# BauerLab/VARSCOT

Measured on AMD Instinct MI355X. Metric: guides/sec (candidate sites/sec alongside) at <=8 mismatches on a 3.0 Gbp reference, higher is better.
Workload: dtype u32

## Files before the change

### varscot_amd/csrc/vsc_api.cpp

```cpp
#include <algorithm>
#include <atomic>
#include <chrono>
#include <cstdlib>
#include <cmath>
#include <cstdio>
#include <cstring>
#include <memory>
#include <new>
#include <string>
#include <vector>

#include "vsc_enum.h"
#include "vsc_internal.h"
#include "vsc_objects.h"
#include "vsc_varmap.h"

using namespace vsc;

namespace {

struct HostTimer {
    bool on = vsc::host_timing_on();
    std::chrono::steady_clock::time_point t0 = std::chrono::steady_clock::now();
    void lap(const char *what)
    {
        if (!on) return;
        auto t1 = std::chrono::steady_clock::now();
        std::fprintf(stderr, "[vsc timing] %-28s %9.3f ms\n", what, std::chrono::duration<double, std::milli>(t1 - t0).count());
        t0 = t1;
    }
};

}

namespace vsc {
static std::atomic<int> g_host_timing{0};
bool host_timing_on() { return g_host_timing.load(std::memory_order_relaxed) != 0; }
}

namespace {

int fail(vsc_ctx *ctx, int code, const char *what, hipError_t e = hipSuccess)
{
    if (ctx) {
        char buf[512];
        if (e != hipSuccess)
            std::snprintf(buf, sizeof buf, "%s: %s", what, hipGetErrorString(e));
        else
            std::snprintf(buf, sizeof buf, "%s", what);
        ctx->err = buf;
    }
    return code;
}

int fail_in(vsc_ctx *ctx, int code, const char *who, const char *what) { return fail(ctx, code, (std::string(who) + ": " + what).c_str()); }

#define VSC_HIP(ctx, call)                                                 \
    do {                                                                   \
        hipError_t e_ = (call);                                            \
        if (e_ != hipSuccess) return fail((ctx), e_ == hipErrorOutOfMemory ? VSC_ERR_NOMEM : VSC_ERR_DEVICE, #call, e_); \
    } while (0)

hipError_t ensure_hl(vsc_ctx *ctx, const vsc_genome *genome)
{
    vsc_genome *g = const_cast<vsc_genome *>(genome);
    if (g->d_hl) return hipSuccess;
    hipError_t e = hipMalloc((void **)&g->d_hl, g->dev_words * sizeof(uint2));
    if (e != hipSuccess) return e;
    g->device_bytes += g->dev_words * sizeof(uint2);
    return launch_interleave(g->d_hi, g->d_lo, g->dev_words, g->d_hl, ctx->stream);
}

hipError_t take_records(vsc_ctx *ctx, vsc_hits *hits, uint64_t n)
{
    const size_t bytes = n * sizeof(vsc_hit);
    int best = -1;
    for (size_t i = 0; i < ctx->spare_records.size(); ++i)
        if (ctx->spare_records[i].cap >= bytes && (best < 0 || ctx->spare_records[i].cap < ctx->spare_records[best].cap))
            best = (int)i;
    if (best >= 0) {
        hits->storage = ctx->spare_records[best];
        ctx->spare_records.erase(ctx->spare_records.begin() + best);
    } else {
        for (auto &b : ctx->spare_records) b.release();
        ctx->spare_records.clear();
        hipError_t e = hits->storage.ensure(bytes);
        if (e != hipSuccess) return e;
    }
    hits->d_records = (vsc_hit *)hits->storage.p;
    return hipSuccess;
}

double hit_probability(unsigned m)
{
    double p = 0, c = 1;
    for (unsigned j = 0; j <= m && j <= 21; ++j) {
        if (j > 0) c = c * (21 - (j - 1)) / j;
        p += c * std::pow(0.75, (double)j) * std::pow(0.25, (double)(21 - j));
    }
    return p;
}

PamMasks pam_masks(int a, int b)
{
    PamMasks m;
    m.ah = (a & 2) ? 0xFFFFFFFFu : 0u;
    m.al = (a & 1) ? 0xFFFFFFFFu : 0u;
    m.bh = (b & 2) ? 0xFFFFFFFFu : 0u;
    m.bl = (b & 1) ? 0xFFFFFFFFu : 0u;
    return m;
}

int base_code(char c)
{
    switch (c) {
    case 'A': case 'a': return 0;
    case 'C': case 'c': return 1;
    case 'G': case 'g': return 2;
    case 'T': case 't': return 3;
    default: return 4;
    }
}

void guide_planes(uint64_t g, uint32_t *h, uint32_t *l)
{
    uint32_t hh = 0, ll = 0;
    for (int i = 0; i < VSC_READ_LEN; ++i) {
        const unsigned c = (unsigned)(g >> (2 * i)) & 3u;
        hh |= (c >> 1) << i;
        ll |= (c & 1u) << i;
    }
    *h = hh;
    *l = ll;
}

}

template <class F> int guarded(vsc_ctx *ctx, F &&body) noexcept
{
    try {
        return body();
    } catch (const std::bad_alloc &) {
        try {
            if (ctx) ctx->err = "out of host memory";
        } catch (...) {
        }
        return VSC_ERR_NOMEM;
    } catch (...) {
        try {
            if (ctx) ctx->err = "unexpected C++ exception";
        } catch (...) {
        }
        return VSC_ERR_DEVICE;
    }
}


extern "C" {

int vsc_abi_version(void) { return VSC_ABI_VERSION; }

int vsc_device_count(void)
{
    int n = 0;
    if (hipGetDeviceCount(&n) != hipSuccess) return 0;
    return n;
}

int vsc_ctx_create(int device_id, vsc_ctx **out) { return vsc_ctx_create_masked(device_id, nullptr, 0, out); }

int vsc_ctx_create_masked(int device_id, const uint32_t *cu_mask, uint32_t n_mask_words, vsc_ctx **out)
{
    if (!out) return VSC_ERR_INVALID;
    *out = nullptr;
    int n = 0;
    if (hipGetDeviceCount(&n) != hipSuccess || n <= 0) return VSC_ERR_NODEVICE;
    if (device_id < 0 || device_id >= n) return VSC_ERR_INVALID;
    vsc_ctx *ctx = new (std::nothrow) vsc_ctx();
    if (!ctx) return VSC_ERR_NOMEM;
    ctx->device = device_id;
    hipDeviceProp_t prop;
    if (hipSetDevice(device_id) != hipSuccess || hipGetDeviceProperties(&prop, device_id) != hipSuccess ||
        (cu_mask && n_mask_words ? hipExtStreamCreateWithCUMask(&ctx->stream, n_mask_words, cu_mask) : hipStreamCreate(&ctx->stream)) != hipSuccess) {
        delete ctx;
        return VSC_ERR_DEVICE;
    }
    ctx->own_stream = true;
    ctx->n_cus = prop.multiProcessorCount;
    for (auto &e : ctx->ev)
        if (hipEventCreate(&e) != hipSuccess) {
            vsc_ctx_destroy(ctx);
            return VSC_ERR_DEVICE;
        }
    *out = ctx;
    return VSC_OK;
}

int vsc_ctx_release_scratch(vsc_ctx *ctx)
{
    if (!ctx) return VSC_ERR_INVALID;
    (void)hipSetDevice(ctx->device);
    (void)hipStreamSynchronize(ctx->stream);
    for (DeviceBuf *b : {&ctx->counters, &ctx->guides, &ctx->score_guides, &ctx->keys_a, &ctx->keys_b, &ctx->vals_a, &ctx->vals_b, &ctx->votes_rows,
                         &ctx->score_mit, &ctx->score_flags, &ctx->score_feat, &ctx->score_sched, &ctx->sort_segs, &ctx->sort_tabs,
                         &ctx->sort_over, &ctx->seed_off,
                         &ctx->seed_poff, &ctx->seed_lrest, &ctx->sum_rows, &ctx->sum_excl, &ctx->sel_hist, &ctx->sel_tabs, &ctx->sel_keys,
                         &ctx->sel_masks, &ctx->sum_rows_in, &ctx->regions_buf, &ctx->enum_tabs, &ctx->locate_buf, &ctx->locate_out,
                         &ctx->varmap_buf, &ctx->var_state, &ctx->var_excl, &ctx->var_labels})
        b->release();
    ctx->regions_serial = 0;
    ctx->locate_serial = 0;
    ctx->varmap_serial = 0;
    for (auto &b : ctx->spare_records) b.release();
    ctx->spare_records.clear();
    ctx->forest.nodes.release();
    ctx->forest.ranks.release();
    ctx->forest.fingerprint = 0;
    return VSC_OK;
}

int vsc_ctx_destroy(vsc_ctx *ctx)
{
    if (!ctx) return VSC_OK;
    (void)vsc_ctx_release_scratch(ctx);
    for (auto &e : ctx->ev)
        if (e) (void)hipEventDestroy(e);
    if (ctx->own_stream && ctx->stream) (void)hipStreamDestroy(ctx->stream);
    delete ctx;
    return VSC_OK;
}

int vsc_ctx_set_stream(vsc_ctx *ctx, void *hip_stream)
{
    if (!ctx) return VSC_ERR_INVALID;
    if (ctx->own_stream && ctx->stream) {
        (void)hipStreamSynchronize(ctx->stream);
        (void)hipStreamDestroy(ctx->stream);
    }
    ctx->stream = (hipStream_t)hip_stream;
    ctx->own_stream = false;
    return VSC_OK;
}

const char *vsc_last_error(const vsc_ctx *ctx) { return ctx ? ctx->err.c_str() : "null context"; }

int vsc_ctx_set_debug_params(vsc_ctx *ctx, const vsc_debug_params *params)
{
    if (!ctx) return VSC_ERR_INVALID;
    ctx->dbg = params ? *params : default_debug_params();
    return VSC_OK;
}

int vsc_ctx_get_debug_params(const vsc_ctx *ctx, vsc_debug_params *out)
{
    if (!ctx || !out) return VSC_ERR_INVALID;
    *out = ctx->dbg;
    return VSC_OK;
}

void vsc_debug_set_host_timing(int on) { vsc::g_host_timing.store(on ? 1 : 0, std::memory_order_relaxed); }

int vsc_ctx_timing(const vsc_ctx *ctx, vsc_timing *out)
{
    if (!ctx || !out) return VSC_ERR_INVALID;
    *out = ctx->timing;
    return VSC_OK;
}

int vsc_genome_load(vsc_ctx *ctx, const uint32_t *hi, const uint32_t *lo, const uint32_t *nmask, uint64_t first_word,
                    uint64_t n_words, uint64_t own_words, const vsc_contig *contigs, uint32_t n_contigs,
                    vsc_genome **out)
{
    return guarded(ctx, [&]() -> int {
    if (!ctx || !out) return VSC_ERR_INVALID;
    *out = nullptr;
    ctx->err.clear();
    if (!hi || !lo || !nmask || !contigs || n_contigs == 0 || n_words == 0 || own_words == 0 || own_words > n_words)
        return fail(ctx, VSC_ERR_INVALID, "vsc_genome_load: null or empty argument");
    if (own_words < n_words && own_words % kTileWords != 0)
        return fail(ctx, VSC_ERR_INVALID, "vsc_genome_load: a shard followed by halo words must own a multiple of 64 words");
    const uint64_t n_tiles = (own_words + kTileWords - 1) / kTileWords;
    const uint64_t dev_words = std::max<uint64_t>(n_tiles * kTileWords, n_words) + kPadWords;
    if ((first_word + dev_words) * 32 >= (1ull << 32) - 4096)
        return fail(ctx, VSC_ERR_RANGE, "vsc_genome_load: genome exceeds the 32-bit position space (4 Gbases)");
    std::vector<uint32_t> off(n_contigs), end(n_contigs);
    for (uint32_t c = 0; c < n_contigs; ++c) {
        const uint64_t e = contigs[c].offset + contigs[c].length;
        if (e >= (1ull << 32) - 4096) return fail(ctx, VSC_ERR_RANGE, "vsc_genome_load: contig table exceeds 4 Gbases");
        if (c > 0 && contigs[c].offset < contigs[c - 1].offset + contigs[c - 1].length + 1)
            return fail(ctx, VSC_ERR_INVALID, "vsc_genome_load: contigs must be ascending and separated by >= 1 N position");
        off[c] = (uint32_t)contigs[c].offset;
        end[c] = (uint32_t)e;
    }
    VSC_HIP(ctx, hipSetDevice(ctx->device));
    vsc_genome *g = new (std::nothrow) vsc_genome();
    if (!g) return fail(ctx, VSC_ERR_NOMEM, "vsc_genome_load: out of host memory");
    g->ctx = ctx;
    g->first_word = first_word;
    g->own_words = own_words;
    g->dev_words = dev_words;
    g->n_tiles = (uint32_t)n_tiles;
    g->n_contigs = n_contigs;
    g->h_contig_off = off;
    g->h_contig_end = end;
    const size_t pb = dev_words * sizeof(uint32_t), cb = (size_t)n_contigs * sizeof(uint32_t);
    hipError_t e = hipSuccess;
    auto step = [&](hipError_t r) {
        if (e == hipSuccess) e = r;
    };
    step(hipMalloc((void **)&g->d_hi, pb));
    step(hipMalloc((void **)&g->d_lo, pb));
    step(hipMalloc((void **)&g->d_nm, pb));
    step(hipMalloc((void **)&g->d_contig_off, cb));
    step(hipMalloc((void **)&g->d_contig_end, cb));
    if (e == hipSuccess) {
        step(hipMemsetAsync(g->d_hi, 0, pb, ctx->stream));
        step(hipMemsetAsync(g->d_lo, 0, pb, ctx->stream));
        step(hipMemsetAsync(g->d_nm, 0xFF, pb, ctx->stream));
        step(hipMemcpyAsync(g->d_hi, hi, n_words * sizeof(uint32_t), hipMemcpyHostToDevice, ctx->stream));
        step(hipMemcpyAsync(g->d_lo, lo, n_words * sizeof(uint32_t), hipMemcpyHostToDevice, ctx->stream));
        step(hipMemcpyAsync(g->d_nm, nmask, n_words * sizeof(uint32_t), hipMemcpyHostToDevice, ctx->stream));
        step(hipMemcpyAsync(g->d_contig_off, off.data(), cb, hipMemcpyHostToDevice, ctx->stream));
        step(hipMemcpyAsync(g->d_contig_end, end.data(), cb, hipMemcpyHostToDevice, ctx->stream));
        step(hipStreamSynchronize(ctx->stream));
    }
    if (e != hipSuccess) {
        vsc_genome_free(g);
        return fail(ctx, e == hipErrorOutOfMemory ? VSC_ERR_NOMEM : VSC_ERR_DEVICE, "vsc_genome_load", e);
    }
    g->device_bytes = 3 * pb + 2 * cb;
    *out = g;
    return VSC_OK;
    });
}

}

int vsc::genome_table_only(vsc_ctx *ctx, const vsc_contig *contigs, uint32_t n_contigs, vsc_genome **out)
{
    if (!ctx || !out || !contigs || n_contigs == 0) return VSC_ERR_INVALID;
    *out = nullptr;
    std::vector<uint32_t> off(n_contigs), end(n_contigs);
    for (uint32_t c = 0; c < n_contigs; ++c) {
        off[c] = (uint32_t)contigs[c].offset;
        end[c] = (uint32_t)(contigs[c].offset + contigs[c].length);
    }
    VSC_HIP(ctx, hipSetDevice(ctx->device));
    vsc_genome *g = new (std::nothrow) vsc_genome();
    if (!g) return fail(ctx, VSC_ERR_NOMEM, "out of host memory");
    g->ctx = ctx;
    g->n_contigs = n_contigs;
    g->h_contig_off = off;
    g->h_contig_end = end;
    const size_t cb = (size_t)n_contigs * sizeof(uint32_t);
    hipError_t e = hipMalloc((void **)&g->d_contig_off, cb);
    if (e == hipSuccess) e = hipMalloc((void **)&g->d_contig_end, cb);
    if (e == hipSuccess) e = hipMemcpy(g->d_contig_off, off.data(), cb, hipMemcpyHostToDevice);
    if (e == hipSuccess) e = hipMemcpy(g->d_contig_end, end.data(), cb, hipMemcpyHostToDevice);
    if (e != hipSuccess) {
        vsc_genome_free(g);
        return fail(ctx, e == hipErrorOutOfMemory ? VSC_ERR_NOMEM : VSC_ERR_DEVICE, "contig table upload", e);
    }
    g->device_bytes = 2 * cb;
    *out = g;
    return VSC_OK;
}

extern "C" {

int vsc_genome_free(vsc_genome *g)
{
    if (!g) return VSC_OK;
    if (g->ctx) (void)hipSetDevice(g->ctx->device);
    for (void *p : {(void *)g->d_hi, (void *)g->d_lo, (void *)g->d_nm, (void *)g->d_contig_off, (void *)g->d_contig_end, (void *)g->d_hl,
                    (void *)g->d_ix_chunk_tab, (void *)g->d_ix_vert, (void *)g->d_ix_sites, (void *)g->d_ix_edge})
        if (p) (void)hipFree(p);
    delete g;
    return VSC_OK;
}

uint64_t vsc_genome_device_bytes(const vsc_genome *g) { return g ? g->device_bytes + g->index_bytes : 0; }

namespace {

#define VSC_TRY(call)                        \
    do {                                     \
        hipError_t e_ = (call);              \
        if (e_ != hipSuccess) return e_;     \
    } while (0)

void fill_pam(ScanArgs &a, const vsc_search_params *params)
{
    a.n_pam = 2;
    a.pam[0] = pam_masks(2, 2);
    a.pam[1] = pam_masks(2, 0);
    if (params && params->has_extra_pam) {
        const int p0 = base_code(params->extra_pam[0]), p1 = base_code(params->extra_pam[1]);
        if (p0 < 4 && p1 < 4) a.pam[a.n_pam++] = pam_masks(p0, p1);
    }
}

uint32_t pam_code_set(const ScanArgs &a)
{
    uint32_t codes = 0;
    for (uint32_t c = 0; c < a.n_pam; ++c)
        codes |= ((((a.pam[c].ah & 2u) | (a.pam[c].al & 1u)) << 2) | (a.pam[c].bh & 2u) | (a.pam[c].bl & 1u)) << (4 * c);
    return codes;
}

void fill_genome(ScanArgs &a, const vsc_ctx *ctx, const vsc_genome *genome)
{
    a.hi = genome->d_hi;
    a.lo = genome->d_lo;
    a.nm = genome->d_nm;
    a.first_pos = (uint32_t)(genome->first_word * 32);
    a.n_tiles = genome->n_tiles;
    a.contig_end = genome->d_contig_end;
    a.n_contigs = genome->n_contigs;
    a.counters = (unsigned long long *)ctx->counters.p;
}

int scan_groups(const vsc_ctx *ctx, uint32_t n_tiles)
{
    const uint32_t n_waves_max = (uint32_t)ctx->n_cus * 4 * kWavesPerGroup;
    const uint32_t n_chunks = (n_tiles + kChunkTiles - 1) / kChunkTiles;
    const uint32_t n_waves = std::max<uint32_t>(1, std::min<uint32_t>(n_waves_max, n_chunks));
    return (int)((n_waves + kWavesPerGroup - 1) / kWavesPerGroup);
}

bool index_matches(const vsc_genome *g, const vsc_search_params *p)
{
    if (!g->has_index) return false;
    const bool want = p && p->has_extra_pam && base_code(p->extra_pam[0]) < 4 && base_code(p->extra_pam[1]) < 4;
    if (want != (g->index_has_extra_pam != 0)) return false;
    return !want || (base_code(p->extra_pam[0]) == base_code(g->index_extra_pam[0]) &&
                     base_code(p->extra_pam[1]) == base_code(g->index_extra_pam[1]));
}

void free_index(vsc_genome *g)
{
    for (void **p : {(void **)&g->d_ix_chunk_tab, (void **)&g->d_ix_vert, (void **)&g->d_ix_sites, (void **)&g->d_ix_edge}) {
        if (*p) (void)hipFree(*p);
        *p = nullptr;
    }
    g->has_index = false;
    g->index_bytes = 0;
    g->ix_chunks = 0;
}

void class_counts(vsc_genome *g, const std::vector<uint32_t> &ctab);

hipError_t build_index(vsc_ctx *ctx, vsc_genome *g, const vsc_search_params *params, std::string *why)
{
    free_index(g);
    hipStream_t st = ctx->stream;
    ScanArgs a{};
    fill_pam(a, params);
    fill_genome(a, ctx, g);
    const int n_groups = scan_groups(ctx, a.n_tiles);
    VSC_TRY(ctx->counters.ensure(kCounterWords * sizeof(unsigned long long)));
    a.counters = (unsigned long long *)ctx->counters.p;
    unsigned long long cnt[kCntSlots];
    VSC_TRY(hipEventRecord(ctx->ev[kEvIndexStart], st));
    VSC_TRY(hipMemsetAsync(ctx->counters.p, 0, sizeof cnt, st));
    VSC_TRY(launch_scan(a, n_groups, true, st));
    VSC_TRY(hipMemcpyAsync(cnt, ctx->counters.p, sizeof cnt, hipMemcpyDeviceToHost, st));
    VSC_TRY(hipStreamSynchronize(st));
    const uint64_t S = cnt[kCntHits];
    if (3 * S >= (1ull << 32) - (1u << 20)) {
        *why = "too many PAM-valid sites for 32-bit table indices";
        return hipErrorInvalidValue;
    }
    DeviceBuf sx, sl, sp, full, rec16;
    auto release = [&]() {
        for (DeviceBuf *b : {&sx, &sl, &sp, &full, &rec16}) b->release();
    };
    hipError_t e = hipSuccess;
    auto step = [&](hipError_t r) {
        if (e == hipSuccess) e = r;
    };
    HostTimer ht;
    constexpr uint32_t kKeys = 8 * kBuckets;
    const uint32_t pam_codes = pam_code_set(a);
    const size_t n4 = std::max<uint64_t>(S, 1) * sizeof(uint32_t);
    for (DeviceBuf *b : {&sx, &sl, &sp}) step(b->ensure(n4));
    step(rec16.ensure(std::max<uint64_t>(S, 1) * sizeof(uint4)));
    const size_t edge_words = (size_t)((3 * S + 31) / 32 + 1);
    ht.lap("index: count pass + buffers");
    if (e == hipSuccess && S > 0) {
        a.site_x = (uint32_t *)sx.p;
        a.site_l = (uint32_t *)sl.p;
        a.site_pos = (uint32_t *)sp.p;
        a.hit_cap = S;
        step(hipMemsetAsync(ctx->counters.p, 0, sizeof cnt, st));
        step(launch_scan(a, n_groups, true, st));
        step(launch_seed_pack16((const uint32_t *)sx.p, (const uint32_t *)sl.p, (const uint32_t *)sp.p, S, (uint4 *)rec16.p, st));
        step(hipStreamSynchronize(st));
    }
    for (DeviceBuf *b : {&sx, &sl, &sp}) b->release();
    ht.lap("index: emit pass");
    constexpr unsigned kKeyBits = 2 * kSegBases + 3, kBits1 = 8, kBits2 = kKeyBits - kBits1;
    constexpr uint32_t kBins1 = 1u << kBits1, kBins2 = 1u << kBits2;
    step(ctx->keys_a.ensure(std::max<uint64_t>(S, 1) * sizeof(uint64_t)));
    step(ctx->keys_b.ensure(std::max<uint64_t>(S, 1) * sizeof(uint64_t)));
    step(full.ensure(std::max<uint64_t>(3 * S, 1) * sizeof(uint4)));
    step(ctx->sort_tabs.ensure(3 * (size_t)(kBins1 * kBins2) * sizeof(uint32_t)));
    const size_t seg_bytes = (kBins1 * sizeof(SortSeg) + 255) / 256 * 256;
    step(ctx->sort_segs.ensure(seg_bytes + (kBins1 + 1) * sizeof(uint32_t)));
// ... 154 lines not shown
    uint64_t sites;
    uint64_t own_words, vert_bytes, edge_words, fingerprint;
    uint32_t chunks, n_contigs;
    uint8_t has_extra_pam;
    char extra_pam[2];
    uint8_t layout;
    uint8_t pad[4];
};
static_assert(sizeof(IndexFileHeader) == 80, "index file header layout");
constexpr char kIndexMagic[8] = {'V', 'S', 'C', 'S', 'E', 'E', 'D', 0};
constexpr size_t kIndexIoChunk = 64u << 20;

hipError_t genome_fingerprint(vsc_ctx *ctx, const vsc_genome *g, uint64_t *out)
{
    VSC_TRY(ctx->counters.ensure(kCounterWords * sizeof(unsigned long long)));
    unsigned long long *d_sum = (unsigned long long *)ctx->counters.p;
    VSC_TRY(hipMemsetAsync(d_sum, 0, sizeof *d_sum, ctx->stream));
    const uint64_t words = std::min<uint64_t>(g->own_words + 1, g->dev_words);
    VSC_TRY(launch_plane_hash(g->d_hi, g->d_lo, g->d_nm, words, d_sum, ctx->stream));
    unsigned long long sum = 0;
    VSC_TRY(hipMemcpyAsync(&sum, d_sum, sizeof sum, hipMemcpyDeviceToHost, ctx->stream));
    std::vector<uint32_t> tab(2 * (size_t)g->n_contigs);
    if (g->n_contigs) {
        VSC_TRY(hipMemcpyAsync(tab.data(), g->d_contig_off, (size_t)g->n_contigs * sizeof(uint32_t), hipMemcpyDeviceToHost, ctx->stream));
        VSC_TRY(hipMemcpyAsync(tab.data() + g->n_contigs, g->d_contig_end, (size_t)g->n_contigs * sizeof(uint32_t), hipMemcpyDeviceToHost, ctx->stream));
    }
    VSC_TRY(hipStreamSynchronize(ctx->stream));
    uint64_t h = 0xcbf29ce484222325ull;
    auto eat = [&](uint64_t v) {
        for (int i = 0; i < 8; ++i) h = (h ^ ((v >> (8 * i)) & 0xFF)) * 0x100000001b3ull;
    };
    eat(sum);
    eat(g->own_words);
    eat(g->first_word);
    for (uint32_t w : tab) eat(w);
    *out = h;
    return hipSuccess;
}

bool chunk_table_ok(const std::vector<uint32_t> &ctab, uint64_t S, uint64_t vert_bytes, std::string *why)
{
    const uint64_t n_blocks = vert_bytes / (kVertWords * sizeof(uint32_t));
    uint64_t expect_site = 0, expect_block = 0;
    uint32_t last_group = 0;
    for (size_t c = 0; c * 4 < ctab.size(); ++c) {
        const uint64_t first = ctab[4 * c], count = ctab[4 * c + 1], vfirst = ctab[4 * c + 3];
        const uint32_t z = ctab[4 * c + 2], bucket = z & kChunkBucketMask, minus_from = (z >> kChunkMinusShift) & 0xFFFu;
        const uint32_t cls = z >> kChunkClassShift;
        const uint64_t blocks = (count + kSlicedSites - 1) / kSlicedSites;
        const char *bad = nullptr;
        if (count == 0 || count > (uint64_t)kSlicedChunk) bad = "site count";
        else if (first != expect_site || first + count > 3 * S) bad = "first site";
        else if (vfirst != expect_block || vfirst + blocks > n_blocks) bad = "first block";
        else if (bucket >= (uint32_t)kBuckets || cls >= (uint32_t)kSeedClasses || (bucket << 2 | cls) < last_group) bad = "bucket";
        else if (minus_from > count) bad = "strand boundary";
        if (bad) {
            *why = "chunk " + std::to_string(c) + ": bad " + bad;
            return false;
        }
        expect_site = first + count;
        expect_block = vfirst + blocks;
        last_group = bucket << 2 | cls;
    }
    if (expect_site != 3 * S) {
        *why = "the chunks do not cover the site table";
        return false;
    }
    return true;
}

void class_counts(vsc_genome *g, const std::vector<uint32_t> &ctab)
{
    for (int c = 0; c < 4; ++c) g->ix_class_sites[c] = g->ix_class_chunks[c] = 0;
    for (size_t c = 0; c * 4 < ctab.size(); ++c) {
        const uint32_t cls = ctab[4 * c + 2] >> kChunkClassShift;
        g->ix_class_sites[cls] += ctab[4 * c + 1];
        g->ix_class_chunks[cls] += 1;
    }
    for (int c = 0; c < 4; ++c) g->ix_class_sites[c] /= kSegments;
}

struct FileCloser {
    std::FILE *f;
    ~FileCloser() { if (f) std::fclose(f); }
};

hipError_t index_io(std::FILE *f, void *dev, uint64_t bytes, bool to_file, std::vector<char> &host, bool *io_ok)
{
    for (uint64_t off = 0; off < bytes; off += kIndexIoChunk) {
        const size_t n = (size_t)std::min<uint64_t>(kIndexIoChunk, bytes - off);
        if (to_file) {
            VSC_TRY(hipMemcpy(host.data(), (const char *)dev + off, n, hipMemcpyDeviceToHost));
            if (std::fwrite(host.data(), 1, n, f) != n) { *io_ok = false; return hipSuccess; }
        } else {
            if (std::fread(host.data(), 1, n, f) != n) { *io_ok = false; return hipSuccess; }
            VSC_TRY(hipMemcpy((char *)dev + off, host.data(), n, hipMemcpyHostToDevice));
        }
    }
    return hipSuccess;
}

}

int vsc_genome_build_index(vsc_ctx *ctx, vsc_genome *genome, const vsc_search_params *params)
{
    return guarded(ctx, [&]() -> int {
    if (!ctx || !genome || genome->ctx != ctx) return VSC_ERR_INVALID;
    ctx->err.clear();
    if (index_matches(genome, params)) return VSC_OK;
    VSC_HIP(ctx, hipSetDevice(ctx->device));
    std::string why;
    hipError_t e = build_index(ctx, genome, params, &why);
    if (e != hipSuccess) {
        if (!why.empty()) return fail(ctx, VSC_ERR_RANGE, ("vsc_genome_build_index: " + why).c_str());
        return fail(ctx, e == hipErrorOutOfMemory ? VSC_ERR_NOMEM : VSC_ERR_DEVICE, "vsc_genome_build_index", e);
    }
    ctx->timing.index_ms = genome->index_ms;
    return VSC_OK;
    });
}

int vsc_genome_index_save(vsc_ctx *ctx, const vsc_genome *genome, const char *path)
{
    return guarded(ctx, [&]() -> int {
    if (!ctx || !genome || genome->ctx != ctx || !path) return VSC_ERR_INVALID;
    ctx->err.clear();
    if (!genome->has_index) return fail(ctx, VSC_ERR_INVALID, "vsc_genome_index_save: the genome has no seed index (vsc_genome_build_index)");
    VSC_HIP(ctx, hipSetDevice(ctx->device));
    IndexFileHeader h{};
    std::memcpy(h.magic, kIndexMagic, sizeof h.magic);
    h.abi = VSC_ABI_VERSION;
    h.seg_bases = kSegBases;
    h.sliced_chunk = kSlicedChunk;
    h.sliced_sites = kSlicedSites;
    h.layout = (uint8_t)kIndexLayout;
    h.sites = genome->index_sites;
    h.own_words = genome->own_words;
    h.vert_bytes = genome->ix_vert_bytes;
    h.edge_words = genome->ix_edge_words;
    h.chunks = genome->ix_chunks;
    h.n_contigs = genome->n_contigs;
    h.has_extra_pam = genome->index_has_extra_pam;
    h.extra_pam[0] = genome->index_extra_pam[0];
    h.extra_pam[1] = genome->index_extra_pam[1];
    VSC_HIP(ctx, genome_fingerprint(ctx, genome, &h.fingerprint));
    FileCloser fc{std::fopen(path, "wb")};
    if (!fc.f) return fail(ctx, VSC_ERR_INVALID, (std::string("vsc_genome_index_save: cannot write ") + path).c_str());
    bool ok = std::fwrite(&h, sizeof h, 1, fc.f) == 1;
    std::vector<char> host(kIndexIoChunk);
    const uint64_t S = genome->index_sites;
    if (ok) VSC_HIP(ctx, index_io(fc.f, genome->d_ix_sites, 3 * S * sizeof(uint2), true, host, &ok));
    if (ok) VSC_HIP(ctx, index_io(fc.f, genome->d_ix_edge, h.edge_words * sizeof(uint32_t), true, host, &ok));
    if (ok) VSC_HIP(ctx, index_io(fc.f, genome->d_ix_chunk_tab, (uint64_t)h.chunks * sizeof(uint4), true, host, &ok));
    if (ok) VSC_HIP(ctx, index_io(fc.f, genome->d_ix_vert, h.vert_bytes, true, host, &ok));
    if (ok) ok = std::fflush(fc.f) == 0;
    if (!ok) return fail(ctx, VSC_ERR_DEVICE, (std::string("vsc_genome_index_save: write to ") + path + " failed").c_str());
    return VSC_OK;
    });
}

int vsc_genome_index_load(vsc_ctx *ctx, vsc_genome *genome, const char *path)
{
    return guarded(ctx, [&]() -> int {
    if (!ctx || !genome || genome->ctx != ctx || !path) return VSC_ERR_INVALID;
    ctx->err.clear();
    VSC_HIP(ctx, hipSetDevice(ctx->device));
    const auto t0 = std::chrono::steady_clock::now();
    FileCloser fc{std::fopen(path, "rb")};
    if (!fc.f) return fail(ctx, VSC_ERR_INVALID, (std::string("vsc_genome_index_load: cannot read ") + path).c_str());
    IndexFileHeader h{};
    if (std::fread(&h, sizeof h, 1, fc.f) != 1 || std::memcmp(h.magic, kIndexMagic, sizeof h.magic) != 0)
        return fail(ctx, VSC_ERR_INVALID, (std::string("vsc_genome_index_load: ") + path + " is not a seed index file").c_str());
    if (h.abi != VSC_ABI_VERSION || h.seg_bases != (uint32_t)kSegBases || h.sliced_chunk != (uint32_t)kSlicedChunk ||
        h.sliced_sites != (uint32_t)kSlicedSites || h.layout != (uint8_t)kIndexLayout)
        return fail(ctx, VSC_ERR_INVALID, "vsc_genome_index_load: the file was written by another version of the library");
    uint64_t fp = 0;
    VSC_HIP(ctx, genome_fingerprint(ctx, genome, &fp));
    if (h.own_words != genome->own_words || h.n_contigs != genome->n_contigs || h.fingerprint != fp)
        return fail(ctx, VSC_ERR_INVALID, "vsc_genome_index_load: the file belongs to another genome");
    const uint64_t S = h.sites;
    if (3 * S >= (1ull << 32) || h.edge_words != (3 * S + 31) / 32 + 1 || h.vert_bytes % (kVertWords * sizeof(uint32_t)) != 0)
        return fail(ctx, VSC_ERR_INVALID, "vsc_genome_index_load: inconsistent header");
    {
        const long at = std::ftell(fc.f);
        const uint64_t want = (uint64_t)sizeof h + 3 * S * sizeof(uint2) + h.edge_words * sizeof(uint32_t) +
                              (uint64_t)h.chunks * sizeof(uint4) + h.vert_bytes;
        if (at < 0 || std::fseek(fc.f, 0, SEEK_END) != 0) return fail(ctx, VSC_ERR_INVALID, "vsc_genome_index_load: cannot seek in the file");
        const long size = std::ftell(fc.f);
        if (size < 0 || (uint64_t)size != want || std::fseek(fc.f, at, SEEK_SET) != 0)
            return fail(ctx, VSC_ERR_INVALID, (std::string("vsc_genome_index_load: ") + path + " is truncated or does not match its header").c_str());
    }
    free_index(genome);
    hipError_t e = hipSuccess;
    auto step = [&](hipError_t r) {
        if (e == hipSuccess) e = r;
    };
    const uint64_t sb = std::max<uint64_t>(3 * S, 1) * sizeof(uint2), eb = h.edge_words * sizeof(uint32_t);
    const uint64_t cb = std::max<uint64_t>(h.chunks, 1) * sizeof(uint4), vb = std::max<uint64_t>(h.vert_bytes, kVertWords * sizeof(uint32_t));
    step(hipMalloc((void **)&genome->d_ix_sites, sb));
    step(hipMalloc((void **)&genome->d_ix_edge, eb));
    step(hipMalloc((void **)&genome->d_ix_chunk_tab, cb));
    step(hipMalloc((void **)&genome->d_ix_vert, vb));
    bool ok = true;
    std::vector<char> host(kIndexIoChunk);
    if (e == hipSuccess) step(index_io(fc.f, genome->d_ix_sites, 3 * S * sizeof(uint2), false, host, &ok));
    if (e == hipSuccess && ok) step(index_io(fc.f, genome->d_ix_edge, eb, false, host, &ok));
    if (e == hipSuccess && ok) step(index_io(fc.f, genome->d_ix_chunk_tab, (uint64_t)h.chunks * sizeof(uint4), false, host, &ok));
    if (e == hipSuccess && ok) step(index_io(fc.f, genome->d_ix_vert, h.vert_bytes, false, host, &ok));
    if (e != hipSuccess || !ok) {
        free_index(genome);
        if (e != hipSuccess) return fail(ctx, e == hipErrorOutOfMemory ? VSC_ERR_NOMEM : VSC_ERR_DEVICE, "vsc_genome_index_load", e);
        return fail(ctx, VSC_ERR_INVALID, (std::string("vsc_genome_index_load: ") + path + " is truncated").c_str());
    }
    {
        std::vector<uint32_t> ctab((size_t)h.chunks * 4);
        if (h.chunks) VSC_HIP(ctx, hipMemcpy(ctab.data(), genome->d_ix_chunk_tab, ctab.size() * sizeof(uint32_t), hipMemcpyDeviceToHost));
        std::string why;
        if (!chunk_table_ok(ctab, S, h.vert_bytes, &why)) {
            free_index(genome);
            return fail(ctx, VSC_ERR_INVALID, (std::string("vsc_genome_index_load: ") + path + " is damaged (" + why + ")").c_str());
        }
        class_counts(genome, ctab);
    }
    genome->ix_chunks = h.chunks;
    genome->ix_vert_bytes = vb;
    genome->ix_edge_words = h.edge_words;
    genome->index_sites = S;
    genome->sites = S;
    genome->has_index = true;
    genome->index_has_extra_pam = h.has_extra_pam;
    genome->index_extra_pam[0] = h.extra_pam[0];
    genome->index_extra_pam[1] = h.extra_pam[1];
    genome->index_bytes = sb + eb + cb + vb;
    genome->index_ms = std::chrono::duration<double, std::milli>(std::chrono::steady_clock::now() - t0).count();
    ctx->timing.index_ms = genome->index_ms;
    return VSC_OK;
    });
}

}

namespace {

unsigned ceil_log2(uint64_t x)
{
    unsigned b = 0;
    while (b < 63 && (1ull << b) < x) ++b;
    return b;
}

struct SortRows {
    uint32_t *side_src = nullptr;
    DeviceBuf *side_other = nullptr;
    const uint2 *guides = nullptr;
    uint32_t guide_first = 0;
    uint4 *rows = nullptr;
    uint64_t rows_first = 0;
};

struct SortInfo {
    unsigned levels = 0;
    unsigned bin_bits = 0;
    uint64_t bytes = 0;
    unsigned slot_fallbacks = 0;
};

hipError_t bin_sort(vsc_ctx *ctx, const vsc_genome *genome, std::vector<SortSeg> segs, uint64_t *src, uint64_t *other,
                    unsigned key_bits, unsigned pos_pad, uint32_t pos_base, vsc_hit *out, hipEvent_t ev_sorted, SortInfo *info,
                    DeviceBuf *other_buf = nullptr, bool *slots = nullptr, const SortRows *rows = nullptr)
{
    uint32_t *side_src = rows ? rows->side_src : nullptr, *side_other = nullptr;
    hipStream_t st = ctx->stream;
    unsigned rem = key_bits;
    bool sorted_marked = false;
    const vsc_debug_params &dbg = ctx->dbg;
    uint64_t sort_cap = kSortCap;
    unsigned max_bits = kSortMaxBinBits;
    if (dbg.sort_cap) sort_cap = std::min<uint64_t>(kSortCap, std::max<uint32_t>(16, dbg.sort_cap));
    if (dbg.sort_max_bits) max_bits = std::min<unsigned>(kSortMaxBinBits, std::max<uint32_t>(1, dbg.sort_max_bits));
    uint64_t slot_cap = dbg.sort_slot_cap ? dbg.sort_slot_cap : (sort_cap + sort_cap / 4 + 15) / 16 * 16;
    slot_cap = std::max<uint64_t>(slot_cap, 16);
    for (unsigned level = 1; !segs.empty(); ++level) {
        if (level > 48) return hipErrorUnknown;
        uint64_t n_max = 0, n_all = 0;
        for (const SortSeg &s : segs) {
            n_max = std::max<uint64_t>(n_max, s.n_in);
            n_all += s.n_in;
        }
        unsigned bits = 0;
        if (n_max > sort_cap) {
            if (rem == 0) return hipErrorUnknown;
            const uint64_t want = std::max<uint64_t>(1, sort_cap * 7 / 10);
            bits = std::min<unsigned>({std::max(1u, ceil_log2((n_max + want - 1) / want)), max_bits, rem});
            while (bits > 1 && ((uint64_t)segs.size() << bits) > (1ull << 22)) --bits;
        }
        const size_t n_segs = segs.size();
        const size_t n_bins = n_segs << bits;
        bool use_slots = level == 1 && bits && slots && other_buf && (dbg.sort_optimistic == 1 || (dbg.sort_optimistic != 0 && *slots));
        if (level == 1 && bits && other_buf) {
            uint64_t span = 1;
            for (const SortSeg &sg : segs) span = std::max<uint64_t>(span, sg.out_off + sg.n_in);
            const uint64_t slot_records = (uint64_t)n_bins * slot_cap;
            if (use_slots && dbg.sort_optimistic != 1) {
                size_t free_b = 0, total_b = 0;
                if (hipMemGetInfo(&free_b, &total_b) != hipSuccess) free_b = 0;
                const uint64_t room = (uint64_t)free_b + other_buf->cap;
                const uint64_t slot_bytes = slot_records * (sizeof(uint64_t) + (rows ? sizeof(uint32_t) : 0));
                if (slot_records > 4 * n_all + (1ull << 20) || slot_bytes + (1ull << 30) > room + (rows ? rows->side_other->cap : 0)) {
                    use_slots = false;
                    *slots = false;
                }
            }
            hipError_t ge = other_buf->ensure((size_t)(use_slots ? std::max(slot_records, span) : span) * sizeof(uint64_t));
            if (ge == hipErrorOutOfMemory && use_slots) {
                (void)hipGetLastError();
                use_slots = false;
                *slots = false;
                ge = other_buf->ensure((size_t)span * sizeof(uint64_t));
            }
            if (ge != hipSuccess) return ge;
            other = (uint64_t *)other_buf->p;
            if (rows) {
                VSC_TRY(rows->side_other->ensure(other_buf->cap / sizeof(uint64_t) * sizeof(uint32_t)));
                side_other = (uint32_t *)rows->side_other->p;
            }
        }
        std::vector<uint32_t> &tile0 = ctx->host_tile0;
        tile0.assign(n_segs + 1, 0);
        uint64_t tiles = 0;
        for (size_t i = 0; i < n_segs; ++i) {
            tile0[i] = (uint32_t)tiles;
            tiles += (segs[i].n_in + kSortTile - 1) / kSortTile;
        }
        if (tiles >= (1ull << 31)) return hipErrorInvalidValue;
        tile0[n_segs] = (uint32_t)tiles;
        const size_t seg_bytes = (n_segs * sizeof(SortSeg) + 255) / 256 * 256;
        VSC_TRY(ctx->sort_segs.ensure(seg_bytes + tile0.size() * sizeof(uint32_t)));
        SortSeg *d_segs = (SortSeg *)ctx->sort_segs.p;
        uint32_t *d_tile0 = (uint32_t *)((char *)ctx->sort_segs.p + seg_bytes);
        ctx->host_segs = segs;
        VSC_TRY(hipMemcpyAsync(d_segs, ctx->host_segs.data(), n_segs * sizeof(SortSeg), hipMemcpyHostToDevice, st));
        VSC_TRY(hipMemcpyAsync(d_tile0, tile0.data(), tile0.size() * sizeof(uint32_t), hipMemcpyHostToDevice, st));
        VSC_TRY(ctx->sort_over.ensure(256 + n_bins * sizeof(SortSeg)));
        uint32_t *d_n_over = (uint32_t *)ctx->sort_over.p;
        if (bits) VSC_TRY(ctx->sort_tabs.ensure(3 * n_bins * sizeof(uint32_t)));
        uint32_t flags[3] = {0, 0, 0};
        for (;;) {
            if (dbg.sort_debug)
                std::fprintf(stderr, "[vsc sort] level %u: %zu segments, %llu records, largest %llu, %u bits (of %u left), cap %llu%s\n", level,
                             n_segs, (unsigned long long)n_all, (unsigned long long)n_max, bits, rem, (unsigned long long)sort_cap,
                             use_slots ? ", slot mode" : "");
            VSC_TRY(hipMemsetAsync(d_n_over, 0, 3 * sizeof(uint32_t), st));
            FinArgs f{};
            f.segs = d_segs;
            f.n_segs = (uint32_t)n_segs;
            f.src = src;
            f.side_src = side_src;
            if (rows) {
                f.guides = rows->guides;
                f.guide_first = rows->guide_first;
                f.rows = rows->rows;
                f.rows_first = rows->rows_first;
            }
            if (bits) {
                SortArgs a{};
                a.segs = d_segs;
                a.seg_tile0 = d_tile0;
                a.n_segs = (uint32_t)n_segs;
                a.n_tiles = (uint32_t)tiles;
                a.in = src;
                a.out = other;
                a.side_in = rows ? side_src : nullptr;
                a.side_out = rows ? side_other : nullptr;
                a.hist = (uint32_t *)ctx->sort_tabs.p;
                a.cursor = a.hist + n_bins;
                a.bin_start = a.cursor + n_bins;
                a.bin_bits = bits;
                a.bin_shift = kRecPosShift + pos_pad + rem - bits;
                if (dbg.sort_xcd != 0 && tiles >= 64) a.xcd_tiles = (uint32_t)((tiles + 7) / 8);
                if (use_slots) {
                    a.hist = a.cursor;
                    a.slot_cap = (uint32_t)slot_cap;
                    a.overflow = d_n_over + 2;
                    VSC_TRY(hipMemsetAsync(a.cursor, 0, n_bins * sizeof(uint32_t), st));
                    VSC_TRY(launch_bin_partition(a, st));
                    VSC_TRY(launch_bin_scan(a, st));
                } else {
                    VSC_TRY(hipMemsetAsync(a.hist, 0, n_bins * sizeof(uint32_t), st));
                    VSC_TRY(launch_bin_hist(a, st));
                    VSC_TRY(launch_bin_scan(a, st));
                    if (dbg.sort_debug >= 2) {
                        std::vector<uint32_t> h(n_bins);
                        VSC_TRY(hipMemcpyAsync(h.data(), a.hist, n_bins * sizeof(uint32_t), hipMemcpyDeviceToHost, st));
                        VSC_TRY(hipStreamSynchronize(st));
                        for (size_t i = 0; i < n_segs; ++i) {
                            std::vector<uint64_t> recs(segs[i].n_in);
                            VSC_TRY(hipMemcpy(recs.data(), src + segs[i].in_off, recs.size() * sizeof(uint64_t), hipMemcpyDeviceToHost));
                            std::vector<uint32_t> want((size_t)1 << bits, 0);
                            for (uint64_t r : recs) {
                                if (r >> 63) continue;
                                want[(r >> a.bin_shift) & (((uint64_t)1 << bits) - 1)]++;
                            }
                            for (size_t b = 0; b < want.size(); ++b)
                                if (want[b] != h[(i << bits) + b])
                                    std::fprintf(stderr, "[vsc sort]   seg %zu (in_off %llu n %u) bin %zu: device %u host %u\n", i,
                                                 (unsigned long long)segs[i].in_off, segs[i].n_in, b, h[(i << bits) + b], want[b]);
                        }
                    }
                    VSC_TRY(launch_bin_partition(a, st));
                }
                f.src = other;
                f.side_src = side_other;
                f.hist = a.hist;
                f.bin_start = a.bin_start;
                f.bin_bits = bits;
                f.slot_cap = a.slot_cap;
                f.overflow = a.overflow;
            }
            if (!sorted_marked && ev_sorted) {
                VSC_TRY(hipEventRecord(ev_sorted, st));
                sorted_marked = true;
            }
            const unsigned rem_after = rem - bits;
            f.sub_bits = std::min<unsigned>(rows ? kSortSubBitsRows : kSortSubBits, rem_after);
            f.sub_shift = kRecPosShift + pos_pad + rem_after - f.sub_bits;
            f.pos_pad = pos_pad;
            f.pos_base = pos_base;
            f.low_bits = rem_after - f.sub_bits;
            f.over = (SortSeg *)((char *)ctx->sort_over.p + 256);
            f.over_cap = (uint32_t)std::min<size_t>(n_bins, 0xFFFFFFFFu);
            f.n_over = d_n_over;
            f.cursor = d_n_over + 1;
            f.cap = (uint32_t)sort_cap;
            f.contig_off = genome->d_contig_off;
            f.n_contigs = genome->n_contigs;
            f.out = out;
            VSC_TRY(launch_bin_finalize(f, 2 * ctx->n_cus, st));
            if (bits) {
                VSC_TRY(hipMemcpyAsync(flags, d_n_over, sizeof flags, hipMemcpyDeviceToHost, st));
                VSC_TRY(hipStreamSynchronize(st));
                if (use_slots && flags[2]) {
                    use_slots = false;
                    *slots = false;
                    if (info) {
                        info->slot_fallbacks++;
                        info->bytes += 16 * n_all;
                    }
                    continue;
                }
            }
            if (info && bits) {
                if (info->levels == 0) info->bin_bits = bits;
                info->levels++;
                info->bytes += (use_slots ? 16 : 24) * n_all;
            }
            if (info) info->bytes += 24 * n_all;
            if (info && rows) info->bytes += (bits ? 8 : 0) * n_all + (4 + 12 + 64) * n_all;
            break;
        }
        if (!bits) break;
        rem -= bits;
        const uint32_t n_over = flags[0];
        if (n_over == 0) break;
        segs.resize(n_over);
        VSC_TRY(hipMemcpyAsync(segs.data(), (char *)ctx->sort_over.p + 256, (size_t)n_over * sizeof(SortSeg), hipMemcpyDeviceToHost, st));
        VSC_TRY(hipStreamSynchronize(st));
        std::swap(src, other);
        std::swap(side_src, side_other);
        if (rows && !side_other) {
            uint64_t span = 1;
            for (const SortSeg &sg : segs) span = std::max<uint64_t>(span, sg.out_off + sg.n_in);
            VSC_TRY(rows->side_other->ensure(span * sizeof(uint32_t)));
            side_other = (uint32_t *)rows->side_other->p;
        }
    }
    return hipSuccess;
}

hipError_t result_room(vsc_ctx *ctx, vsc_hits *hits, uint64_t used, uint64_t n, uint64_t projected)
{
    const uint64_t need = used + n;
    if (hits->storage.p && hits->storage.cap >= need * sizeof(vsc_hit)) return hipSuccess;
    if (used == 0) {
        if (hits->storage.p) {
            ctx->spare_records.push_back(hits->storage);
            hits->storage = DeviceBuf{};
        }
        VSC_TRY(take_records(ctx, hits, std::max(need, projected)));
        return hipSuccess;
    }
    DeviceBuf bigger;
    VSC_TRY(bigger.ensure(std::max(need, projected) * sizeof(vsc_hit)));
    hipError_t e = hipMemcpyAsync(bigger.p, hits->storage.p, used * sizeof(vsc_hit), hipMemcpyDeviceToDevice, ctx->stream);
    if (e == hipSuccess) e = hipStreamSynchronize(ctx->stream);
    if (e != hipSuccess) {
        bigger.release();
        return e;
    }
    hits->storage.release();
    hits->storage = bigger;
    hits->d_records = (vsc_hit *)bigger.p;
    return hipSuccess;
}

struct PassFound {
    HostTimer ht;
    int algo = 0, n_parts = 0;
    uint32_t max_mm = 0, guide_base = 0;
    uint64_t cap = 0, n = 0;
    std::vector<SortSeg> segs;
    unsigned key_bits = 0, pos_pad = 0;
    uint32_t pos_base = 0;
    bool bases = false;
    bool selected = false;
    std::vector<uint64_t> sel_off;
    std::vector<SumSeg> sink_segs;
    std::vector<uint32_t> sink_tile0;
    SinkInput sink{};
    bool classified = false;
};

uint32_t neighbours(int k) { return k < 0 ? 0u : (k == 0 ? 1u : (k == 1 ? 22u : 211u)); }

SeedPlan seed_cut(const vsc_genome *genome, const uint32_t *gp, uint32_t n_guides, uint32_t m, int n_cus, const vsc_debug_params &dbg,
                  int *k2_max)
{
    SeedPlan plan{};
    plan.max_mm = m;
    ScanArgs pa{};
    vsc_search_params ip{};
    ip.has_extra_pam = genome->index_has_extra_pam;
    ip.extra_pam[0] = genome->index_extra_pam[0];
    ip.extra_pam[1] = genome->index_extra_pam[1];
    fill_pam(pa, &ip);
    plan.n_pam = pa.n_pam;
    plan.pam_codes = pam_code_set(pa);
    plan.tight = dbg.seed_tight != 0;
    if (!plan.tight) {
        plan.k0 = plan.k1 = m / kSegments;
        *k2_max = (int)plan.k0;
    } else {
        uint32_t left_reads[kSeedClasses][VSC_MAX_MISMATCHES + 1] = {};
        int left_max = -1;
        for (uint32_t i = 0; i < n_guides; ++i) {
            const uint32_t x = gp[2 * (size_t)i], l = gp[2 * (size_t)i + 1];
            const uint32_t mine = (((x >> 21) & 1u) << 3) | (((l >> 21) & 1u) << 2) | (((x >> 22) & 1u) << 1) | ((l >> 22) & 1u);
            for (uint32_t c = 0; c < plan.n_pam; ++c) {
                const uint32_t diff = mine ^ ((plan.pam_codes >> (4 * c)) & 15u);
                const uint32_t spent = ((diff & 12u) ? 1u : 0u) + ((diff & 3u) ? 1u : 0u);
                if (spent > m) continue;
                left_reads[c][m - spent]++;
                left_max = std::max(left_max, (int)(m - spent));
            }
        }
        double cost[9];
        double chunks_all = 0, sites_all = 0;
        uint64_t reads_any = 0;
        for (uint32_t c = 0; c < plan.n_pam; ++c) {
            chunks_all += (double)genome->ix_class_chunks[c] / kSegments;
            sites_all += (double)genome->ix_class_sites[c];
            uint64_t reads_c = 0;
            for (int left = 0; left <= (int)m; ++left) reads_c += left_reads[c][left];
            reads_any = std::max(reads_any, reads_c);
        }
        const double block_bytes = (double)kVertWords * 4 / kSlicedSites;
        for (int cut = 0; cut < 9; ++cut) {
            const int k0 = cut % 3, k1 = cut / 3;
            cost[cut] = -1;
            if (left_max - k0 - k1 - 2 > 2) continue;
            double bytes = 0, visits = 0;
            for (uint32_t c = 0; c < plan.n_pam; ++c) {
                double e2 = 0;
                for (int left = 0; left <= (int)m; ++left) e2 += (double)left_reads[c][left] * neighbours(left - k0 - k1 - 2);
                const double per_list = e2 / kBucketsPerSeg;
                bytes += (1.0 - std::exp(-per_list)) * (double)genome->ix_class_sites[c] * block_bytes;
                visits += per_list * (double)genome->ix_class_chunks[c] / kSegments;
            }
            for (int k : {k0, k1}) {
                const double per_list = (double)reads_any * neighbours(k) / kBucketsPerSeg;
                bytes += (1.0 - std::exp(-per_list)) * sites_all * block_bytes;
                visits += per_list * chunks_all;
            }
            cost[cut] = std::max(bytes / 4.2e12, visits * 215.0 / ((double)n_cus * 4 * 2.0e9));
        }
        int best = -1;
        for (int cut = 0; cut < 9; ++cut)
            if (cost[cut] >= 0 && (best < 0 || cost[cut] < cost[best])) best = cut;
        const int forced = dbg.seed_tight >= 1 ? dbg.seed_tight - 1 : -1;
        if (forced >= 0 && forced < 9 && cost[forced] >= 0) best = forced;
        if (best < 0) best = 4 * (int)(m ? (m - 1) / kSegments : 0u);
        plan.k0 = (uint32_t)(best % 3);
        plan.k1 = (uint32_t)(best / 3);
        *k2_max = std::min<int>(2, (int)m - (int)plan.k0 - (int)plan.k1 - 2);
    }
    plan.n_nbr = neighbours(std::max<int>(std::max<int>((int)plan.k0, (int)plan.k1), *k2_max));
    return plan;
}

hipError_t seed_plan(vsc_ctx *ctx, const vsc_genome *genome, const uint32_t *gp, uint32_t n_guides, const PassFound &f, SeedArgs &sa,
                     int *n_groups, bool *shared)
{
    int k2_max = 0;
    const SeedPlan plan = seed_cut(genome, gp, n_guides, f.max_mm, ctx->n_cus, ctx->dbg, &k2_max);
    const uint64_t n_pairs = (uint64_t)n_guides * (neighbours((int)plan.k0) + neighbours((int)plan.k1) + plan.n_pam * neighbours(k2_max));
    const uint64_t list_cap = n_pairs + (uint64_t)kLists * (kGuideUnroll - 1) + 2 * kGuideUnroll;
    VSC_TRY(ctx->seed_off.ensure((kLists + 1) * sizeof(uint32_t)));
    VSC_TRY(ctx->seed_poff.ensure((kLists + 1) * sizeof(uint32_t)));
    VSC_TRY(ctx->seed_lrest.ensure(list_cap * sizeof(uint2)));
    VSC_TRY(hipMemsetAsync(ctx->seed_lrest.p, 0xFF, list_cap * sizeof(uint2), ctx->stream));
    VSC_TRY(launch_seed_lists((const uint2 *)ctx->guides.p, n_guides, plan, (uint32_t *)ctx->seed_off.p, (uint32_t *)ctx->seed_poff.p,
                              (uint2 *)ctx->seed_lrest.p, ctx->stream));
    VSC_TRY(hipEventRecord(ctx->ev[kEvPrepEnd], ctx->stream));
    sa.chunk_tab = genome->d_ix_chunk_tab;
    sa.n_chunks = genome->ix_chunks;
    sa.vert = genome->d_ix_vert;
    sa.list_rest = (const uint2 *)ctx->seed_lrest.p;
    sa.sites = genome->d_ix_sites;
    sa.edge_bits = genome->d_ix_edge;
    sa.guides = (const uint2 *)ctx->guides.p;
    sa.poff = (const uint32_t *)ctx->seed_poff.p;
    sa.max_mm = f.max_mm;
    sa.k_half = f.max_mm / 2;
    sa.k_seg0 = plan.k0;
    sa.k_seg1 = plan.k1;
    sa.contig_end = genome->d_contig_end;
    sa.n_contigs = genome->n_contigs;
    sa.counters = (unsigned long long *)ctx->counters.p;
    sa.n_parts = (uint32_t)f.n_parts;
    uint32_t groups_per_cu = kSlicedWavesPerSimd;
    if (ctx->dbg.seed_groups_per_cu) groups_per_cu = ctx->dbg.seed_groups_per_cu;
    *shared = (uint64_t)n_guides * neighbours((int)std::max(plan.k0, plan.k1)) / kBucketsPerSeg >= 72;
    if (ctx->dbg.seed_shared >= 0) *shared = ctx->dbg.seed_shared == 1;
    const uint32_t n_grabs = (sa.n_chunks + kSlicedGrab - 1) / kSlicedGrab;
    const uint32_t n_waves_max = (uint32_t)ctx->n_cus * groups_per_cu * kWavesPerGroup;
    const uint32_t n_waves = std::max<uint32_t>(1, std::min<uint32_t>(n_waves_max, *shared ? n_grabs * kWavesPerGroup : n_grabs));
    *n_groups = (int)((n_waves + kWavesPerGroup - 1) / kWavesPerGroup);
    sa.group_out = *shared && ctx->dbg.seed_group_out != 0 ? 1u : 0u;
    const uint32_t owners = sa.group_out ? (uint32_t)*n_groups : (uint32_t)*n_groups * kWavesPerGroup;
    const uint64_t per_wave = f.cap / ((uint64_t)owners * 8 * f.n_parts);
    uint32_t want_reserve = (uint32_t)std::min<uint64_t>(f.n_parts > 8 ? (sa.group_out ? 1024 : 128) : 1024, std::max<uint64_t>(kWave, per_wave));
    if (ctx->dbg.seed_reserve) want_reserve = std::min<uint32_t>(1024, std::max<uint32_t>(kWave, ctx->dbg.seed_reserve));
    sa.reserve_log2 = 6;
    while ((2u << sa.reserve_log2) <= want_reserve) ++sa.reserve_log2;
    sa.reserve = 1u << sa.reserve_log2;
    sa.pos_pad = f.pos_pad;
    sa.pos_base = f.pos_base;
    uint64_t part_cap = f.cap / f.n_parts + f.cap / f.n_parts / 7 + 4096;
    part_cap = std::max<uint64_t>(part_cap, (uint64_t)(1.2 * genome->seen_rate[f.max_mm] * std::min<uint32_t>(n_guides, kRegionReads)) + 4096);
    sa.part_cap = part_cap + (uint64_t)owners * sa.reserve;
    return hipSuccess;
}

int find_pass(vsc_ctx *ctx, const vsc_genome *genome, const uint64_t *guides, uint32_t n_guides, uint32_t guide_base,
              const vsc_search_params *params, bool keep_bases, vsc_timing &t, PassFound &f)
{
    const int algo = (int)t.algorithm;
    const uint32_t m = params->max_mismatches;
    f.algo = algo;
    f.max_mm = m;
    f.guide_base = guide_base;
    f.bases = keep_bases;
    const uint32_t n_pad = (n_guides + kGuideUnroll - 1) / kGuideUnroll * kGuideUnroll;
    std::vector<uint32_t> gp((size_t)(n_pad + kGuideUnroll) * 2, 0xFFFFFFFFu);
    for (uint32_t i = 0; i < n_guides; ++i) guide_planes(guides[i], &gp[2 * (size_t)i], &gp[2 * (size_t)i + 1]);
    VSC_HIP(ctx, ctx->guides.ensure(gp.size() * sizeof(uint32_t)));
    VSC_HIP(ctx, ctx->counters.ensure(kCounterWords * sizeof(unsigned long long)));
    VSC_HIP(ctx, hipEventRecord(ctx->ev[kEvPassStart], ctx->stream));
    VSC_HIP(ctx, hipMemcpyAsync(ctx->guides.p, gp.data(), gp.size() * sizeof(uint32_t), hipMemcpyHostToDevice, ctx->stream));

    const double own_bases = (double)genome->n_tiles * kTileBases;
    const double sites_est = genome->sites ? (double)genome->sites : own_bases / 4;
    f.cap = (uint64_t)(1.5 * sites_est * n_guides * hit_probability(m)) + (1u << 20);
    const double seen_rate = genome->seen_rate[m];
    if (algo == VSC_ALGO_SCAN) f.cap = std::max<uint64_t>(f.cap, (uint64_t)(1.2 * seen_rate * n_guides) + 4096);
    unsigned long long cnt[kCntPart + 4 * kParts] = {};
    f.n_parts = (int)((n_guides + kRegionReads - 1) / kRegionReads);
    f.pos_base = (uint32_t)(genome->first_word * 32);
    const unsigned pos_bits = std::max(1u, ceil_log2((uint64_t)genome->dev_words * 32));
    f.pos_pad = pos_bits < 32 ? 32 - pos_bits : 0;
    f.key_bits = pos_bits + 1 + ceil_log2(std::min<uint32_t>(n_guides, kRegionReads));

    ScanArgs a{};
    SeedArgs sa{};
    int n_groups = 1;
    bool seed_shared = false;
    if (algo == VSC_ALGO_SCAN) {
        fill_pam(a, params);
        fill_genome(a, ctx, genome);
        a.guides = (const uint4 *)ctx->guides.p;
        a.n_guides_padded = n_pad;
        a.max_mm = m;
        a.k_half = m / 2;
        n_groups = scan_groups(ctx, a.n_tiles);
        t.genome_bytes += (uint64_t)genome->n_tiles * kTileWords * 3 * sizeof(uint32_t);
        VSC_HIP(ctx, hipEventRecord(ctx->ev[kEvPrepEnd], ctx->stream));
    } else {
        VSC_HIP(ctx, seed_plan(ctx, genome, gp.data(), n_guides, f, sa, &n_groups, &seed_shared));
        f.cap = sa.part_cap * f.n_parts;
    }

    f.ht.lap("prep enqueue");
    uint32_t list_total = 0;
    for (unsigned tries = 0;; ++tries) {
        if (algo == VSC_ALGO_SEED && (sa.part_cap >= (1ull << 32) - (1u << 20) || sa.part_cap >= ((uint64_t)sa.reserve << 20) - sa.reserve))
            return fail(ctx, VSC_ERR_RANGE, "vsc_search: more than 2^32 hits in a block of 64 reads");
        VSC_HIP(ctx, ctx->keys_a.ensure(f.cap * sizeof(uint64_t)));
        VSC_HIP(ctx, hipMemsetAsync(ctx->counters.p, 0, kCounterWords * sizeof(unsigned long long), ctx->stream));
        VSC_HIP(ctx, hipEventRecord(ctx->ev[kEvSearchStart], ctx->stream));
        if (algo == VSC_ALGO_SCAN) {
            VSC_HIP(ctx, ctx->vals_a.ensure(f.cap * sizeof(uint32_t)));
            a.hit_keys = (uint64_t *)ctx->keys_a.p;
            a.hit_vals = (uint32_t *)ctx->vals_a.p;
            a.hit_cap = f.cap;
            VSC_HIP(ctx, launch_scan(a, n_groups, false, ctx->stream));
        } else {
            sa.hit_recs = (uint64_t *)ctx->keys_a.p;
            if (keep_bases) {
                VSC_HIP(ctx, ctx->vals_a.ensure(f.cap * sizeof(uint32_t)));
                sa.hit_side = (uint32_t *)ctx->vals_a.p;
            }
            VSC_HIP(ctx, launch_seed_sliced(sa, n_groups, seed_shared, ctx->stream));
        }
        VSC_HIP(ctx, hipEventRecord(ctx->ev[kEvSearchEnd], ctx->stream));
        VSC_HIP(ctx, hipMemcpyAsync(cnt, ctx->counters.p, sizeof cnt, hipMemcpyDeviceToHost, ctx->stream));
        if (algo == VSC_ALGO_SEED)
            VSC_HIP(ctx, hipMemcpyAsync(&list_total, (const uint32_t *)ctx->seed_poff.p + kLists, sizeof list_total, hipMemcpyDeviceToHost, ctx->stream));
        VSC_HIP(ctx, hipStreamSynchronize(ctx->stream));
        f.ht.lap("search kernel + sync");
        t.passes++;
        if (!cnt[kCntOverflow]) break;
        if (tries >= 2) return fail(ctx, VSC_ERR_DEVICE, "vsc_search: hit buffer overflowed repeatedly");
        if (algo == VSC_ALGO_SEED) {
            uint64_t need = 0;
            for (int q = 0; q < f.n_parts; ++q) need = std::max<uint64_t>(need, cnt[kCntPart + 4 * q] + cnt[kCntPart + 4 * q + 2]);
            sa.part_cap = need + (need >> 6) + 4096 + (uint64_t)(sa.group_out ? n_groups : n_groups * kWavesPerGroup) * sa.reserve;
            f.cap = sa.part_cap * f.n_parts;
        } else {
            f.cap = cnt[kCntHits] + (cnt[kCntHits] >> 6) + 4096;
        }
    }
    float ms = 0;
    VSC_HIP(ctx, hipEventElapsedTime(&ms, ctx->ev[kEvPassStart], ctx->ev[kEvPrepEnd]));
    t.prep_ms += ms;
    VSC_HIP(ctx, hipEventElapsedTime(&ms, ctx->ev[kEvSearchStart], ctx->ev[kEvSearchEnd]));
    t.scan_ms += ms;

    if (algo == VSC_ALGO_SCAN) {
        genome->sites = cnt[kCntSites];
        t.sites = cnt[kCntSites];
        t.pairs += cnt[kCntSites] * n_guides;
        f.n = cnt[kCntHits];
        genome->seen_rate[m] = (double)f.n / n_guides;
        if (f.n >= (1ull << 32)) return fail(ctx, VSC_ERR_RANGE, "vsc_search: more than 2^32 hits in one scan pass (split the read set)");
        if (f.n > 0) f.segs.push_back(SortSeg{0, 0, 0, (uint32_t)f.n, guide_base});
    } else {
        t.list_entries = list_total;
        t.seed_cut = sa.k_seg0 | (sa.k_seg1 << 4);
        t.sites = genome->index_sites;
        t.pairs += cnt[kCntSites];
        t.genome_bytes += cnt[kCntVisited] * kVertWords * sizeof(uint32_t) / kSlicedSites;
        double fullest = 0;
        for (int q = 0; q < f.n_parts; ++q) {
            const uint64_t placed = cnt[kCntPart + 4 * q], real = placed - cnt[kCntPart + 4 * q + 1];
            fullest = std::max(fullest, (double)placed / std::min<uint32_t>(kRegionReads, n_guides - (uint32_t)q * kRegionReads));
            if (placed) f.segs.push_back(SortSeg{(uint64_t)q * sa.part_cap, (uint64_t)q * sa.part_cap, f.n, (uint32_t)placed,
                                                 guide_base + (uint32_t)q * kRegionReads});
            f.n += real;
        }
        genome->seen_rate[m] = fullest;
    }
    t.hits += f.n;
    return VSC_OK;
}

hipError_t sink_input(vsc_ctx *ctx, PassFound &f, bool excluded)
{
    if (f.sink.recs) return hipSuccess;
    f.sink_tile0.assign(1, 0);
    for (const SortSeg &sg : f.segs) {
        f.sink_segs.push_back(SumSeg{sg.in_off, sg.n_in, sg.guide_base - f.guide_base});
        f.sink_tile0.push_back(f.sink_tile0.back() + (sg.n_in + kSumTile - 1) / kSumTile);
    }
    const size_t seg_bytes = f.sink_segs.size() * sizeof(SumSeg), tile0_bytes = f.sink_tile0.size() * sizeof(uint32_t);
    const size_t tile0_at = (seg_bytes + 255) / 256 * 256;
    VSC_TRY(ctx->sort_segs.ensure(tile0_at + tile0_bytes));
    VSC_TRY(hipMemcpyAsync(ctx->sort_segs.p, f.sink_segs.data(), seg_bytes, hipMemcpyHostToDevice, ctx->stream));
    VSC_TRY(hipMemcpyAsync((char *)ctx->sort_segs.p + tile0_at, f.sink_tile0.data(), tile0_bytes, hipMemcpyHostToDevice, ctx->stream));
    SinkInput &a = f.sink;
    a.vals = f.algo == VSC_ALGO_SCAN ? (const uint32_t *)ctx->vals_a.p : nullptr;
    a.segs = (const SumSeg *)ctx->sort_segs.p;
    a.seg_tile0 = (const uint32_t *)((char *)ctx->sort_segs.p + tile0_at);
    a.n_segs = (uint32_t)f.sink_segs.size();
    a.n_tiles = f.sink_tile0.back();
    a.pos_pad = f.pos_pad;
    a.pos_base = f.pos_base;
    a.excl = excluded ? (const uint64_t *)ctx->sum_excl.p + f.guide_base : nullptr;
    a.recs = (const uint64_t *)ctx->keys_a.p;
    return hipSuccess;
}

hipError_t end_pass(vsc_ctx *ctx, PassFound &f, const char *lap, vsc_timing &t)
{
    VSC_TRY(hipEventRecord(ctx->ev[kEvSinkEnd], ctx->stream));
    VSC_TRY(hipStreamSynchronize(ctx->stream));
    f.ht.lap(lap);
    float ms = 0;
    VSC_TRY(hipEventElapsedTime(&ms, ctx->ev[kEvSinkStart], ctx->ev[kEvSinkEnd]));
    t.finalize_ms += ms;
    VSC_TRY(hipEventElapsedTime(&ms, ctx->ev[kEvPassStart], ctx->ev[kEvSinkEnd]));
    t.total_ms += ms;
    t.read_passes++;
    return hipSuccess;
}

int sort_pass(vsc_ctx *ctx, const vsc_genome *genome, PassFound &f, vsc_hits *hits, uint64_t used, uint64_t projected, vsc_timing &t)
{
    SortInfo info;
    if (f.n > 0) {
        uint64_t *src = (uint64_t *)ctx->keys_a.p, *other = nullptr;
        if (f.algo == VSC_ALGO_SCAN && !f.selected) {
            VSC_HIP(ctx, ctx->keys_b.ensure(f.cap * sizeof(uint64_t)));
            const unsigned bits0 = ceil_log2((uint64_t)f.n_parts);
            const size_t n_bins = (size_t)1 << bits0;
            VSC_HIP(ctx, ctx->sort_segs.ensure(512));
            VSC_HIP(ctx, ctx->sort_tabs.ensure(3 * n_bins * sizeof(uint32_t)));
            const uint32_t tile0[2] = {0u, (uint32_t)((f.n + kSortTile - 1) / kSortTile)};
            VSC_HIP(ctx, hipMemcpyAsync(ctx->sort_segs.p, f.segs.data(), sizeof(SortSeg), hipMemcpyHostToDevice, ctx->stream));
            VSC_HIP(ctx, hipMemcpyAsync((char *)ctx->sort_segs.p + 256, tile0, sizeof tile0, hipMemcpyHostToDevice, ctx->stream));
            SortArgs l0{};
            l0.segs = (const SortSeg *)ctx->sort_segs.p;
            l0.seg_tile0 = (const uint32_t *)((char *)ctx->sort_segs.p + 256);
            l0.n_segs = 1;
            l0.n_tiles = tile0[1];
            l0.pair_keys = (const uint64_t *)ctx->keys_a.p;
            l0.pair_vals = (const uint32_t *)ctx->vals_a.p;
            l0.out = (uint64_t *)ctx->keys_b.p;
            l0.hist = (uint32_t *)ctx->sort_tabs.p;
            l0.cursor = l0.hist + n_bins;
            l0.bin_start = l0.cursor + n_bins;
            l0.bin_bits = bits0;
            l0.bin_shift = kRecKeyBits;
            l0.pos_pad = f.pos_pad;
            l0.pos_base = f.pos_base;
            VSC_HIP(ctx, hipMemsetAsync(l0.hist, 0, n_bins * sizeof(uint32_t), ctx->stream));
            VSC_HIP(ctx, launch_bin_hist(l0, ctx->stream));
            VSC_HIP(ctx, launch_bin_scan(l0, ctx->stream));
            VSC_HIP(ctx, launch_bin_partition(l0, ctx->stream));
            std::vector<uint32_t> tabs(3 * n_bins);
            VSC_HIP(ctx, hipMemcpyAsync(tabs.data(), l0.hist, tabs.size() * sizeof(uint32_t), hipMemcpyDeviceToHost, ctx->stream));
            VSC_HIP(ctx, hipStreamSynchronize(ctx->stream));
            f.segs.clear();
            for (int q = 0; q < f.n_parts; ++q) {
                const uint32_t count = tabs[q], start = tabs[2 * n_bins + q];
                if (count) f.segs.push_back(SortSeg{start, start, start, count, f.guide_base + (uint32_t)q * kRegionReads});
            }
            src = (uint64_t *)ctx->keys_b.p;
            other = (uint64_t *)ctx->keys_a.p;
            info.bytes += 12 * f.n + 20 * f.n;
        }
        for (SortSeg &s : f.segs) s.final_off += used;
        f.ht.lap("sort buffers");
        VSC_HIP(ctx, result_room(ctx, hits, used, f.n, projected));
        f.ht.lap("record storage");
        bool *slots = f.algo == VSC_ALGO_SEED && !f.selected ? &genome->sort_slots_ok[f.max_mm] : nullptr;
        SortRows rows;
        if (f.bases) {
            if (ctx->score_feat.ensure(f.n * VSC_PACKED_FEATURE_BYTES) != hipSuccess) {
                (void)hipGetLastError();
                for (auto &b : ctx->spare_records) b.release();
                ctx->spare_records.clear();
                for (DeviceBuf *b : {&ctx->score_mit, &ctx->score_flags, &ctx->score_sched, &ctx->keys_b, &ctx->vals_b}) b->release();
                VSC_HIP(ctx, ctx->score_feat.ensure(f.n * VSC_PACKED_FEATURE_BYTES));
            }
            rows.side_src = (uint32_t *)ctx->vals_a.p;
            rows.side_other = &ctx->vals_b;
            rows.guides = (const uint2 *)ctx->guides.p;
            rows.guide_first = f.guide_base;
            rows.rows = (uint4 *)ctx->score_feat.p;
            rows.rows_first = used;
        }
        VSC_HIP(ctx, bin_sort(ctx, genome, std::move(f.segs), src, other, f.key_bits, f.pos_pad, f.pos_base, hits->d_records, ctx->ev[kEvSinkStart],
                              &info, f.algo == VSC_ALGO_SEED || f.selected ? &ctx->keys_b : nullptr, slots, f.bases ? &rows : nullptr));
    } else {
        VSC_HIP(ctx, hipEventRecord(ctx->ev[kEvSinkStart], ctx->stream));
    }
    VSC_HIP(ctx, end_pass(ctx, f, "sort + finalize + sync", t));
    float ms = 0;
    VSC_HIP(ctx, hipEventElapsedTime(&ms, ctx->ev[kEvSearchEnd], ctx->ev[kEvSinkStart]));
    t.sort_ms += ms;
    t.sort_levels = std::max(t.sort_levels, info.levels);
    t.sort_bin_bits = std::max(t.sort_bin_bits, info.bin_bits);
    t.sort_bytes += info.bytes;
    t.sort_fallbacks += info.slot_fallbacks;
    return VSC_OK;
}

int prepare_forest(vsc_ctx *ctx, const vsc_rf_model *model, const char *who);
void fill_forest(RfArgs &a, const vsc_ctx *ctx);
int resident_ranks(vsc_ctx *ctx, const double *guide_activity, uint32_t n_guides);

int classify_pass(vsc_ctx *ctx, const vsc_genome *genome, PassFound &f, uint32_t n_reads, bool excluded)
{
    if (f.segs.empty()) return VSC_OK;
    RfArgs a{};
    VSC_HIP(ctx, sink_input(ctx, f, excluded));
    fill_forest(a, ctx);
    a.in = f.sink;
    a.score.hl = genome->d_hl;
    a.score.first_pos = (uint32_t)(genome->first_word * 32);
    a.score.n_plane_words = genome->dev_words;
    a.score.guides = (const uint2 *)ctx->guides.p;
    a.act_rank = (const uint8_t *)ctx->forest.ranks.p + f.guide_base;
    a.n_reads = n_reads;
    a.n = (uint64_t)a.in.n_tiles * kSumTile;
// ... 1801 lines not shown
```

### varscot_amd/csrc/vsc_internal.h

```cpp
#pragma once

#include <hip/hip_runtime.h>
#include <stdint.h>

#include "varscot_hip.h"

namespace vsc {

constexpr int kWave = 64;
constexpr int kWavesPerGroup = 4;
constexpr int kSitesPerLane = 8;
constexpr int kBatch = kWave * kSitesPerLane;
constexpr int kQueueCap = kBatch + kWave;
constexpr int kHitCap = 128;
constexpr int kTileWords = kWave;
constexpr int kTileBases = kTileWords * 32;
constexpr int kChunkTiles = 8;
constexpr int kGuideUnroll = 4;
constexpr uint32_t kMask23 = 0x7FFFFFu;
constexpr int kSiteStrandBit = 23;
constexpr int kSiteEdgeBit = 24;
constexpr uint32_t kPadWords = 4;

constexpr int kSegments = 3;
constexpr int kSegBases = 7;
constexpr int kBucketsPerSeg = 1 << (2 * kSegBases);
constexpr int kBuckets = kSegments * kBucketsPerSeg;
constexpr int kSeedHitCap = 256;
constexpr int kSlicedSites = 32;
constexpr int kSlicedChunk = kWave * kSlicedSites;
constexpr int kRestBases = VSC_READ_LEN - kSegBases;
constexpr int kCmpBases = 2 * kSegBases;
constexpr int kVertWords = 2 * kCmpBases;
constexpr int kSeedClasses = 3;
constexpr int kLists = (kSegments - 1 + kSeedClasses) * kBucketsPerSeg;
constexpr int kListBudgetShift = 16;
constexpr uint32_t kListNoBudget = 15;
constexpr int kTokLaneShift = 26;
constexpr int kTokSlotShift = 14;
constexpr uint32_t kTokReadMask = (1u << kTokSlotShift) - 1u;
constexpr int kSlicedResolve = 3;
constexpr int kSlicedTokCap = 512;
constexpr uint32_t kChunkBucketMask = 0xFFFFu;
constexpr int kChunkMinusShift = 16;
constexpr int kChunkEdgeBit = 28;
constexpr int kChunkClassShift = 29;
constexpr uint32_t kIndexLayout = 2;
constexpr int kSlicedWavesPerSimd = 6;
constexpr int kSlicedGrab = 8;

enum { kCntHits = 0, kCntChunk = 1, kCntSites = 2, kCntOverflow = 3, kCntVisited = 4, kCntPad = 5, kCntLost = 6, kCntGroups = 7, kCntSlots = 8 };
constexpr int kRegionBits = 6;
constexpr int kRegionReads = 1 << kRegionBits;
constexpr int kParts = 256;
constexpr int kMaxPassReads = kParts * kRegionReads;
constexpr int kCntPart = 8;
constexpr int kCursors = 32;
constexpr int kCursorStride = 16;
constexpr int kCursorBase = kCntPart + 4 * kParts + 8;
constexpr int kCounterWords = kCursorBase + kCursors * kCursorStride;

constexpr int kRecPosShift = 23;
constexpr int kRecStrandShift = 55;
constexpr int kRecReadShift = 56;
constexpr int kRecKeyBits = 33 + kRegionBits;
constexpr uint64_t kRecSentinel = ~0ull;

constexpr int kSortThreads = 512;
constexpr int kSortItems = 16;
constexpr int kSortTile = kSortThreads * kSortItems;
constexpr int kFinThreads = 512;
constexpr int kFinItems = 16;
constexpr int kSortCap = kFinThreads * kFinItems - 128;
constexpr int kSortMaxBinBits = 11;
constexpr int kSortSubBits = 13;
constexpr int kSortSubBitsRows = 12;
constexpr int kHistTiles = 8;

struct PamMasks {
    uint32_t ah, al;
    uint32_t bh, bl;
};

struct ScanArgs {
    const uint32_t *hi, *lo, *nm;
    uint32_t first_pos;
    uint32_t n_tiles;
    const uint4 *guides;
    uint32_t n_guides_padded;
    uint32_t max_mm;
    uint32_t k_half;
    uint32_t n_pam;
    PamMasks pam[3];
    const uint32_t *contig_end;
    uint32_t n_contigs;
    uint64_t *hit_keys;
    uint32_t *hit_vals;
    unsigned long long hit_cap;
    unsigned long long *counters;
    uint32_t *site_x, *site_l, *site_pos;
};

struct SortSeg {
    uint64_t in_off;
    uint64_t out_off;
    uint64_t final_off;
    uint32_t n_in;
    uint32_t guide_base;
};

struct SortArgs {
    const SortSeg *segs;
    const uint32_t *seg_tile0;
    uint32_t n_segs, n_tiles;
    const uint64_t *in;
    const uint64_t *pair_keys;
    const uint32_t *pair_vals;
    uint64_t *out;
    const uint32_t *side_in;
    uint32_t *side_out;
    uint32_t *hist;
    uint32_t *cursor;
    uint32_t *bin_start;
    uint32_t bin_bits, bin_shift;
    uint32_t pos_pad;
    uint32_t pos_base;
    uint32_t xcd_tiles;
    uint32_t slot_cap;
    uint32_t *overflow;
};

struct FinArgs {
    const SortSeg *segs;
    uint32_t n_segs;
    const uint64_t *src;
    const uint32_t *hist;
    const uint32_t *bin_start;
    uint32_t bin_bits;
    uint32_t sub_shift, sub_bits;
    uint32_t low_bits;
    uint32_t pos_pad;
    uint32_t pos_base;
    SortSeg *over;
    uint32_t over_cap;
    uint32_t cap;
    uint32_t *n_over;
    uint32_t *cursor;
    const uint32_t *contig_off;
    uint32_t n_contigs;
    vsc_hit *out;
    uint32_t slot_cap;
    const uint32_t *overflow;
    const uint32_t *side_src;
    const uint2 *guides;
    uint32_t guide_first;
    uint4 *rows;
    uint64_t rows_first;
};

struct ScoreArgs {
    const vsc_hit *hits;
    uint64_t n;
    const uint2 *hl;
    uint32_t first_pos;
    uint64_t n_plane_words;
    const uint32_t *contig_off;
    const uint2 *guides;
    double *mit;
    uint8_t *mit_flags;
    uint8_t *features;
    const uint64_t *seg_prefix;
    const uint64_t *seg_start;
    uint32_t n_segs;
};

struct SeedPlan {
    uint32_t max_mm, k0, k1, tight;
    uint32_t n_nbr;
    uint32_t n_pam;
    uint32_t pam_codes;
};

struct SeedArgs {
    const uint4 *chunk_tab;
    const uint32_t *vert;
    const uint2 *list_rest;
    const uint2 *sites;
    const uint32_t *edge_bits;
    const uint2 *guides;
    uint32_t n_chunks;
    const uint32_t *poff;
    uint32_t max_mm, k_half;
    uint32_t k_seg0, k_seg1;
    const uint32_t *contig_end;
    uint32_t n_contigs;
    uint64_t *hit_recs;
    uint32_t *hit_side;
    uint32_t group_out;
    uint32_t reserve;
    uint32_t reserve_log2;
    uint32_t pos_pad;
    uint32_t pos_base;
    uint32_t n_parts;
    unsigned long long part_cap;
    unsigned long long *counters;
};

constexpr int kSumThreads = 256;
constexpr int kSumItems = 8;
constexpr int kSumTile = kSumThreads * kSumItems;
constexpr int kSumTilesPerBlock = 8;

struct SumSeg {
    uint64_t in_off;
    uint32_t n;
    uint32_t first_read;
};

struct SinkInput {
    const uint64_t *recs;
    const uint32_t *vals;
    const SumSeg *segs;
    const uint32_t *seg_tile0;
    uint32_t n_segs, n_tiles;
    uint32_t pos_pad, pos_base;
    const uint64_t *excl;
};

constexpr int kRfRows = 512;
constexpr int kRfMaxTests = 1024;
constexpr int kRfMaxNodes = 1024;
constexpr int kRfTileBytes = 26624;
constexpr int kRfPairFirstBit = 3;
constexpr int kRfPairMaxTests = 8 * (32 - kRfPairFirstBit);
constexpr int kRfPairBitsBytes = 16384;
constexpr int kRfPairTileBytes = 24512;
constexpr int kRfChains = 2;
constexpr int kRfRowWords = 20;
struct RfTest {
    uint8_t word, shift, width, thr;
    uint16_t dense_col;
    uint16_t pad;
};

struct RfArgs {
    const uint32_t *nodes;
    const uint8_t *depth;
    uint32_t n_trees, n_nodes;
    uint32_t compact;
    const RfTest *tests;
    const uint32_t *test_begin;
    uint32_t n_tests;
    const uint8_t *dense;
    const uint4 *packed;
    const uint8_t *act_rank;
    uint64_t n;
    uint32_t *votes;
    uint16_t *votes16;
    uint32_t tree_splits;
    ScoreArgs score;
    SinkInput in;
    uint32_t n_reads;
    uint32_t *slot_votes;
};

constexpr int kSumWords = 12;
constexpr int kSumCounts = 11;
constexpr int kSumCountBits = 7;

struct SummaryArgs : SinkInput {
    unsigned long long *out;
};

struct VotesSummaryArgs : SummaryArgs {
    const uint32_t *votes;
    uint32_t n_trees, n_reads;
};

constexpr int kSelBins = 128;
constexpr int kSelThreads = 256;
constexpr int kSelMaxTilesPerBlock = 128;
constexpr int kSelMinTilesPerBlock = 8;
constexpr uint32_t kSelDropped = ~0u;
constexpr int kSelKeyPosBits = 33;

struct SelectArgs : SinkInput {
    uint32_t min_score;
    uint32_t vote_trees;
    uint32_t top_k;
    uint32_t n_reads;
    uint32_t tiles_per_block;
    uint32_t *score;
    uint32_t *hist;
    uint32_t *thr;
    uint32_t *thr_region;
    uint32_t *count;
    uint32_t *cursor;
    const uint64_t *cand_off;
    const uint64_t *surv_off;
    uint64_t *cand_key;
    uint32_t *cand_mask;
    uint64_t *out;
};

constexpr uint32_t kRegOut = 0, kRegIn = 1, kRegMixed = 2;
constexpr uint32_t kRegMinBlockShift = 5;
constexpr uint32_t kRegMaxBlocks = 1u << 23;

struct RegionsView {
    const uint32_t *start;
    const uint32_t *end_max;
    const uint32_t *cls;
    uint32_t n;
    uint32_t n_blocks;
    uint32_t block_shift;
    uint32_t rule;
};

__host__ __device__ inline bool regions_search(const RegionsView &v, uint32_t pos, uint32_t len)
{
    const bool inside = v.rule == VSC_REGION_INSIDE;
    const uint32_t bound = inside ? pos + 1u : pos + len;
    uint32_t lo = 0, hi = v.n;
    while (lo < hi) {
        const uint32_t mid = (lo + hi) >> 1;
        if (v.start[mid] < bound) lo = mid + 1; else hi = mid;
    }
    if (lo == 0) return false;
    const uint32_t e = v.end_max[lo - 1];
    return inside ? e >= pos + (uint32_t)VSC_READ_LEN : e > pos;
}

__host__ __device__ inline bool regions_contains(const RegionsView &v, uint32_t pos, uint32_t len = VSC_READ_LEN)
{
    if (len != (uint32_t)VSC_READ_LEN) return len != 0 && regions_search(v, pos, len);
    const uint32_t b = pos >> v.block_shift;
    if (b >= v.n_blocks) return false;
    const uint32_t c = (v.cls[b >> 4] >> (2u * (b & 15u))) & 3u;
    return c == kRegMixed ? regions_search(v, pos, len) : c == kRegIn;
}

struct SummaryRegionArgs : SummaryArgs {
    RegionsView reg;
    unsigned long long *out_in;
};

struct SelectRegionArgs : SelectArgs {
    RegionsView reg;
    uint32_t drop;
};

hipError_t launch_scan(const ScanArgs &args, int n_groups, bool extract, hipStream_t stream);
hipError_t launch_summary(const SummaryArgs &args, hipStream_t stream);
hipError_t launch_summary_regions(const SummaryRegionArgs &args, hipStream_t stream);
hipError_t launch_votes_summary(const VotesSummaryArgs &args, hipStream_t stream);
hipError_t launch_select_score(const SelectArgs &args, hipStream_t stream);
hipError_t launch_select_score_regions(const SelectRegionArgs &args, hipStream_t stream);
hipError_t launch_select_threshold(const SelectArgs &args, hipStream_t stream);
hipError_t launch_select_compact(const SelectArgs &args, hipStream_t stream);
hipError_t launch_select_resolve(const SelectArgs &args, hipStream_t stream);
hipError_t launch_bin_hist(const SortArgs &args, hipStream_t stream);
hipError_t launch_bin_scan(const SortArgs &args, hipStream_t stream);
hipError_t launch_bin_partition(const SortArgs &args, hipStream_t stream);
hipError_t launch_bin_finalize(const FinArgs &args, int max_groups, hipStream_t stream);
hipError_t launch_rf_predict(const RfArgs &args, hipStream_t stream);
hipError_t launch_interleave(const uint32_t *hi, const uint32_t *lo, uint64_t n, uint2 *hl, hipStream_t stream);
hipError_t launch_score(const ScoreArgs &args, hipStream_t stream);
hipError_t launch_score_packed(const ScoreArgs &args, uint4 *packed, hipStream_t stream);
hipError_t launch_score_schedule(const ScoreArgs &args, uint32_t g_lo, uint32_t g_hi, uint32_t slice_shift, uint32_t n_slices,
                                 uint64_t *bounds, uint64_t *seg_start, uint64_t *seg_prefix, hipStream_t stream);
hipError_t launch_score_pairs(const uint2 *on, const uint2 *off, const uint32_t *masks, uint64_t n, double *mit,
                              uint8_t *mit_flags, uint8_t *features, hipStream_t stream);
hipError_t launch_xpack(const vsc_hit *in, uint64_t n, const uint32_t *contig_off, uint64_t *out, hipStream_t stream);
hipError_t launch_key_bounds(const vsc_hit *in, const uint64_t *range_dev, uint32_t K, uint64_t *bound, hipStream_t stream);
hipError_t launch_merge_packed(const uint64_t *seg_src, const uint64_t *seg_dst, const uint32_t *seg_n, uint32_t n_segs, uint32_t n_shards,
                               uint32_t first_key, const uint32_t *contig_off, const uint32_t *contig_end, uint32_t n_contigs, vsc_hit *out,
                               uint32_t *bad , const uint64_t *seg_side, uint16_t *side_out, hipStream_t stream);
hipError_t launch_plane_hash(const uint32_t *hi, const uint32_t *lo, const uint32_t *nm, uint64_t n_words, unsigned long long *out,
                             hipStream_t stream);
hipError_t launch_seed_keys(const uint4 *rec, uint64_t n, int seg, uint32_t pam_codes, uint32_t n_pam, uint64_t *sort_records, hipStream_t stream);
hipError_t launch_seed_lists(const uint2 *guides, uint32_t n_guides, const SeedPlan &plan, uint32_t *count, uint32_t *poff, uint2 *list_rest,
                             hipStream_t stream);
hipError_t launch_seed_pack16(const uint32_t *x, const uint32_t *l, const uint32_t *pos, uint64_t n, uint4 *rec, hipStream_t stream);
hipError_t launch_seed_gather16(const uint4 *rec, const uint64_t *sorted, uint64_t n, uint4 *out, hipStream_t stream);
hipError_t launch_seed_compact(const uint4 *sites16, uint64_t n_per_table, uint64_t n, uint2 *sites8, uint32_t *edge_bits,
                               hipStream_t stream);
hipError_t launch_seed_chunk_flags(uint4 *chunk_tab, uint32_t n_chunks, const uint32_t *edge_bits, hipStream_t stream);
hipError_t launch_seed_transpose(const uint4 *sites, const uint4 *chunk_tab, uint32_t n_chunks, uint32_t *vert,
                                 hipStream_t stream);
hipError_t launch_seed_sliced(const SeedArgs &args, int n_groups, bool shared, hipStream_t stream);
hipError_t launch_merge(const vsc_hit *in, const uint64_t *shard_off_dev, uint32_t n_shards, uint32_t K, uint64_t *bound,
                        uint64_t *key_off, vsc_hit *out, hipStream_t stream);

}
```

### varscot_amd/csrc/vsc_objects.h

```cpp
#pragma once

#include <string>
#include <vector>

#include "varscot_hip_debug.h"
#include "vsc_internal.h"

namespace vsc {

struct DeviceBuf {
    void *p = nullptr;
    size_t cap = 0;
    hipError_t ensure(size_t bytes)
    {
        if (bytes <= cap) return hipSuccess;
        if (p) (void)hipFree(p);
        p = nullptr;
        cap = 0;
        size_t want = bytes + (bytes < ((size_t)32 << 30) ? bytes / 8 : bytes / 32);
        hipError_t e = hipMalloc(&p, want);
        if (e != hipSuccess && want != bytes) {
            (void)hipGetLastError();
            want = bytes;
            e = hipMalloc(&p, want);
        }
        if (e == hipSuccess) cap = want;
        return e;
    }
    void release()
    {
        if (p) (void)hipFree(p);
        p = nullptr;
        cap = 0;
    }
};

inline vsc_debug_params default_debug_params()
{
    vsc_debug_params d{};
    d.sort_xcd = -1;
    d.sort_optimistic = -1;
    d.score_slices = -1;
    d.seed_shared = -1;
    d.seed_group_out = -1;
    d.seed_tight = -1;
    d.rf_form = -1;
    return d;
}

bool host_timing_on();

}

enum vsc_event {
    kEvPassStart = 0,
    kEvSearchStart,
    kEvSearchEnd,
    kEvSinkStart,
    kEvSinkEnd,
    kEvIndexStart,
    kEvIndexEnd,
    kEvPrepEnd,
    kEvClassStart,
    kEvClassEnd,
    kEvCount,
    kEvStageStart = kEvPassStart,
    kEvStageEnd = kEvSearchStart,
    kEvStage2Start = kEvSearchEnd,
    kEvStage2End = kEvSinkStart,
};

struct vsc_ctx {
    int device = 0;
    int n_cus = 0;
    hipStream_t stream = nullptr;
    bool own_stream = false;
    hipEvent_t ev[kEvCount] = {};
    std::string err;
    vsc_timing timing{};
    vsc_debug_params dbg = vsc::default_debug_params();
    vsc::DeviceBuf counters, guides, keys_a, keys_b, vals_a, score_mit, score_flags, score_feat;
    vsc::DeviceBuf vals_b;
    vsc::DeviceBuf score_guides;
    uint64_t score_guides_hash = 0;
    uint32_t score_guides_n = ~0u;
    vsc::DeviceBuf sort_segs, sort_tabs, sort_over, score_sched;
    std::vector<vsc::SortSeg> host_segs;
    std::vector<uint32_t> host_tile0;
    vsc::DeviceBuf seed_off, seed_poff, seed_lrest;
    vsc::DeviceBuf sum_rows, sum_excl;
    vsc::DeviceBuf sel_hist, sel_tabs, sel_keys, sel_masks;
    vsc::DeviceBuf sum_rows_in, regions_buf;
    vsc::DeviceBuf votes_rows;
    uint64_t regions_serial = 0;
    vsc::DeviceBuf locate_buf, locate_out;
    uint64_t locate_serial = 0;
    vsc::DeviceBuf varmap_buf, var_state, var_excl, var_labels;
    uint64_t varmap_serial = 0;
    vsc::DeviceBuf enum_tabs;
    struct Forest {
        vsc::DeviceBuf nodes, ranks;
        size_t depth_at = 0, tests_at = 0, begin_at = 0;
        uint32_t n_tests = 0, n_trees = 0, n_nodes = 0;
        uint32_t form = 0;
        uint32_t node_stride = 0;
        std::vector<double> thresholds;
        uint64_t fingerprint = 0;
        uint64_t ranks_key = 0;
        uint32_t ranks_n = ~0u;
    } forest;
    std::vector<vsc::DeviceBuf> spare_records;
};

struct vsc_genome {
    vsc_ctx *ctx = nullptr;
    uint32_t *d_hi = nullptr, *d_lo = nullptr, *d_nm = nullptr;
    uint32_t *d_contig_off = nullptr, *d_contig_end = nullptr;
    std::vector<uint32_t> h_contig_off, h_contig_end;
    uint2 *d_hl = nullptr;
    uint64_t first_word = 0, own_words = 0, dev_words = 0;
    uint32_t n_tiles = 0, n_contigs = 0;
    uint64_t device_bytes = 0;
    mutable uint64_t sites = 0;
    mutable double seen_rate[VSC_MAX_MISMATCHES + 1] = {};
    mutable bool sort_slots_ok[VSC_MAX_MISMATCHES + 1] = {true, true, true, true, true, true, true, true, true};
    bool has_index = false;
    uint8_t index_has_extra_pam = 0;
    char index_extra_pam[2] = {0, 0};
    uint64_t index_sites = 0;
    uint4 *d_ix_chunk_tab = nullptr;
    uint32_t *d_ix_vert = nullptr;
    uint2 *d_ix_sites = nullptr;
    uint32_t *d_ix_edge = nullptr;
    uint32_t ix_chunks = 0;
    uint64_t ix_class_sites[4] = {};
    uint64_t ix_class_chunks[4] = {};
    uint64_t ix_vert_bytes = 0, ix_edge_words = 0;
    uint64_t index_bytes = 0;
    double index_ms = 0;
};

struct vsc_regions {
    std::vector<uint32_t> start, end_max, cls;
    std::vector<uint32_t> contig_off, contig_len;
    std::vector<uint32_t> loc_end, loc_index, loc_up;
    bool has_locate = false;
    uint32_t rule = 0, block_shift = 0, n_blocks = 0;
    uint64_t serial = 0;
    vsc_regions_stats stats{};
    vsc::RegionsView view() const
    {
        return vsc::RegionsView{start.data(), end_max.data(), cls.data(), (uint32_t)start.size(), n_blocks, block_shift, rule};
    }
};

struct vsc_hits {
    vsc_ctx *ctx = nullptr;
    vsc_hit *d_records = nullptr;
    vsc::DeviceBuf storage;
    uint64_t n = 0;
    std::vector<vsc_hit> host;
    bool host_valid = false;
};

struct vsc_guides {
    vsc_ctx *ctx = nullptr;
    vsc::DeviceBuf storage;
    size_t loci_at = 0;
    uint64_t n = 0;
    std::vector<uint64_t> codes;
    std::vector<vsc_locus> loci;
    bool host_valid = false;
};

namespace vsc {
int genome_table_only(vsc_ctx *ctx, const vsc_contig *contigs, uint32_t n_contigs, vsc_genome **out);
int merge_packed_shards(vsc_ctx *ctx, const vsc_genome *genome, const void *const *shard_records, const void *const *shard_side,
                        const uint32_t *key_counts, uint32_t n_shards, uint32_t first_key, uint32_t n_keys, vsc_hits **out,
                        DeviceBuf *side_out);
}
```

### varscot_amd/csrc/vsc_seed.hip

```cpp
#include "vsc_internal.h"
#include "vsc_device.h"

#include <type_traits>

namespace vsc {

__device__ __forceinline__ uint32_t segment_key(uint32_t x, uint32_t l, int s)
{
    return (((x >> (kSegBases * s)) & 0x7Fu) << kSegBases) | ((l >> (kSegBases * s)) & 0x7Fu);
}

__device__ __forceinline__ uint32_t pam_code(uint32_t x, uint32_t l)
{
    return (((x >> 21) & 1u) << 3) | (((l >> 21) & 1u) << 2) | (((x >> 22) & 1u) << 1) | ((l >> 22) & 1u);
}

__global__ __launch_bounds__(256) void seed_key_kernel(const uint4 *rec, uint64_t n, int seg, uint32_t pam_codes, uint32_t n_pam, uint64_t *out)
{
    const uint64_t i = (uint64_t)blockIdx.x * blockDim.x + threadIdx.x;
    if (i >= n) return;
    const uint4 r = rec[i];
    const uint32_t code = pam_code(r.x, r.y);
    uint32_t cls = 0;
    for (uint32_t c = n_pam; c-- > 0;)
        if (((pam_codes >> (4 * c)) & 15u) == code) cls = c;
    const uint32_t key = (((segment_key(r.x, r.y, seg) << 2) | cls) << 1) | ((r.x >> kSiteStrandBit) & 1u);
    out[i] = ((uint64_t)key << 32) | (uint32_t)i;
}

__global__ __launch_bounds__(256) void seed_pack16_kernel(const uint32_t *x, const uint32_t *l, const uint32_t *pos, uint64_t n,
                                                          uint4 *rec)
{
    const uint64_t i = (uint64_t)blockIdx.x * blockDim.x + threadIdx.x;
    if (i < n) rec[i] = make_uint4(x[i], l[i], pos[i], 0u);
}

__global__ __launch_bounds__(256) void seed_gather16_kernel(const uint4 *rec, const uint64_t *sorted, uint64_t n, uint4 *out)
{
    const uint64_t i = (uint64_t)blockIdx.x * blockDim.x + threadIdx.x;
    if (i >= n) return;
    out[i] = rec[(uint32_t)sorted[i]];
}

hipError_t launch_seed_keys(const uint4 *rec, uint64_t n, int seg, uint32_t pam_codes, uint32_t n_pam, uint64_t *out, hipStream_t stream)
{
    if (n == 0) return hipSuccess;
    hipLaunchKernelGGL(seed_key_kernel, dim3((unsigned)((n + 255) / 256)), dim3(256), 0, stream, rec, n, seg, pam_codes, n_pam, out);
    return hipGetLastError();
}

hipError_t launch_seed_pack16(const uint32_t *x, const uint32_t *l, const uint32_t *pos, uint64_t n, uint4 *rec, hipStream_t stream)
{
    if (n == 0) return hipSuccess;
    hipLaunchKernelGGL(seed_pack16_kernel, dim3((unsigned)((n + 255) / 256)), dim3(256), 0, stream, x, l, pos, n, rec);
    return hipGetLastError();
}

hipError_t launch_seed_gather16(const uint4 *rec, const uint64_t *sorted, uint64_t n, uint4 *out, hipStream_t stream)
{
    if (n == 0) return hipSuccess;
    hipLaunchKernelGGL(seed_gather16_kernel, dim3((unsigned)((n + 255) / 256)), dim3(256), 0, stream, rec, sorted, n, out);
    return hipGetLastError();
}

__device__ __forceinline__ uint32_t rest_of(uint32_t v, uint32_t seg);

__global__ __launch_bounds__(256) void seed_compact_kernel(const uint4 *sites16, uint64_t n_per_table, uint64_t n, uint2 *sites8,
                                                           uint32_t *edge_bits)
{
    const uint64_t i = (uint64_t)blockIdx.x * blockDim.x + threadIdx.x;
    if (i >= n) return;
    const uint4 r = sites16[i];
    const uint32_t seg = (uint32_t)(i / n_per_table);
    sites8[i] = make_uint2(rest_of(r.x, seg) | (rest_of(r.y, seg) << 16), r.z);
    if ((r.x >> kSiteEdgeBit) & 1u) atomicOr(&edge_bits[i >> 5], 1u << (i & 31u));
}

__global__ __launch_bounds__(256) void seed_chunk_flags_kernel(uint4 *chunk_tab, uint32_t n_chunks, const uint32_t *edge_bits)
{
    const uint32_t c = blockIdx.x * blockDim.x + threadIdx.x;
    if (c >= n_chunks) return;
    const uint4 ct = chunk_tab[c];
    if (ct.y == 0) return;
    const uint32_t first = ct.x, last = ct.x + ct.y - 1;
    uint32_t any = 0;
    for (uint32_t w = first >> 5; w <= last >> 5; ++w) {
        uint32_t bits = edge_bits[w];
        if (w == first >> 5) bits &= 0xFFFFFFFFu << (first & 31u);
        if (w == last >> 5) bits &= 0xFFFFFFFFu >> (31u - (last & 31u));
        any |= bits;
    }
    if (any) chunk_tab[c].z = ct.z | (1u << kChunkEdgeBit);
}

hipError_t launch_seed_compact(const uint4 *sites16, uint64_t n_per_table, uint64_t n, uint2 *sites8, uint32_t *edge_bits,
                               hipStream_t stream)
{
    if (n == 0) return hipSuccess;
    hipLaunchKernelGGL(seed_compact_kernel, dim3((unsigned)((n + 255) / 256)), dim3(256), 0, stream, sites16, n_per_table, n, sites8,
                       edge_bits);
    return hipGetLastError();
}

hipError_t launch_seed_chunk_flags(uint4 *chunk_tab, uint32_t n_chunks, const uint32_t *edge_bits, hipStream_t stream)
{
    if (n_chunks == 0) return hipSuccess;
    hipLaunchKernelGGL(seed_chunk_flags_kernel, dim3((n_chunks + 255) / 256), dim3(256), 0, stream, chunk_tab, n_chunks, edge_bits);
    return hipGetLastError();
}

__constant__ uint8_t kPairP[21] = {0, 0, 0, 0, 0, 0, 1, 1, 1, 1, 1, 2, 2, 2, 2, 3, 3, 3, 4, 4, 5};
__constant__ uint8_t kPairQ[21] = {1, 2, 3, 4, 5, 6, 2, 3, 4, 5, 6, 3, 4, 5, 6, 4, 5, 6, 5, 6, 6};

__device__ __forceinline__ void substitute(uint32_t &h, uint32_t &l, uint32_t p, uint32_t alt)
{
    const uint32_t c = (((h >> p) & 1u) << 1) | ((l >> p) & 1u);
    const uint32_t d = (c + alt) & 3u;
    h = (h & ~(1u << p)) | ((d >> 1) << p);
    l = (l & ~(1u << p)) | ((d & 1u) << p);
}

__device__ __forceinline__ uint32_t seed_neighbour(const uint2 gp, uint32_t s, uint32_t n, uint32_t *dist)
{
    uint32_t h = (gp.x >> (kSegBases * s)) & 0x7Fu, l = (gp.y >> (kSegBases * s)) & 0x7Fu;
    if (n >= 22) {
        const uint32_t e = n - 22, pi = e / 9, alts = e % 9;
        substitute(h, l, kPairP[pi], alts / 3 + 1);
        substitute(h, l, kPairQ[pi], alts % 3 + 1);
    } else if (n >= 1) {
        const uint32_t e = n - 1;
        substitute(h, l, e / 3, e % 3 + 1);
    }
    *dist = n >= 22 ? 2u : (n >= 1 ? 1u : 0u);
    return s * kBucketsPerSeg + ((h << kSegBases) | l);
}

__device__ __forceinline__ uint32_t rest_of(uint32_t v, uint32_t seg)
{
    v &= kMask23;
    if (seg == 0) return v >> kSegBases;
    if (seg == 1) return (v & 0x7Fu) | ((v >> (2 * kSegBases)) << kSegBases);
    return (v & 0x3FFFu) | ((v >> (3 * kSegBases)) << (2 * kSegBases));
}

template <bool kScatter>
__global__ __launch_bounds__(256) void seed_enum_kernel(const uint2 *guides, uint32_t n_guides, const SeedPlan plan, uint32_t *count,
                                                        const uint32_t *poff, uint2 *list_rest)
{
    const uint64_t i = (uint64_t)blockIdx.x * blockDim.x + threadIdx.x;
    const uint64_t total = (uint64_t)n_guides * kSegments * plan.n_nbr;
    if (i >= total) return;
    const uint32_t n = (uint32_t)(i % plan.n_nbr);
    const uint32_t s = (uint32_t)((i / plan.n_nbr) % kSegments);
    const uint32_t g = (uint32_t)(i / ((uint64_t)plan.n_nbr * kSegments));
    const uint2 gp = guides[g];
    uint32_t d;
    const uint32_t b = seed_neighbour(gp, s, n, &d);
    const uint32_t mine = pam_code(gp.x, gp.y);
    const uint32_t rest = rest_of(gp.x, s) | (rest_of(gp.y, s) << 16);
    constexpr uint32_t kNone = (kListNoBudget << kListBudgetShift) | (kListNoBudget << (kListBudgetShift + 4)) |
                               (kListNoBudget << (kListBudgetShift + 8)) | (kListNoBudget << (kListBudgetShift + 12));
    uint32_t shared = kNone;
    for (uint32_t c = 0; c < plan.n_pam; ++c) {
        const uint32_t diff = mine ^ ((plan.pam_codes >> (4 * c)) & 15u);
        const uint32_t spent = ((diff & 12u) ? 1u : 0u) + ((diff & 3u) ? 1u : 0u);
        if (spent + d > plan.max_mm) continue;
        const uint32_t left = plan.max_mm - spent;
        const int thr = s == 0 ? (int)plan.k0 : (s == 1 ? (int)plan.k1 : (plan.tight ? (int)left - (int)plan.k0 - (int)plan.k1 - 2 : (int)plan.k0));
        if ((int)d > thr) continue;
        const uint32_t field = kListBudgetShift + 4 * c;
        if (s < 2) {
            shared = (shared & ~(15u << field)) | ((left - d) << field);
            continue;
        }
        const uint32_t list = b + c * (uint32_t)kBucketsPerSeg;
        const uint32_t at = atomicAdd(&count[list], 1u);
        if (kScatter) list_rest[poff[list] + at] = make_uint2(rest, g | ((kNone & ~(15u << field)) | ((left - d) << field)));
    }
    if (s < 2 && shared != kNone) {
        const uint32_t at = atomicAdd(&count[b], 1u);
        if (kScatter) list_rest[poff[b] + at] = make_uint2(rest, g | shared);
    }
}

__device__ __forceinline__ uint32_t wave_inclusive_scan(uint32_t x)
{
    x += (uint32_t)__builtin_amdgcn_update_dpp(0, (int)x, 0x111, 0xF, 0xF, false);
    x += (uint32_t)__builtin_amdgcn_update_dpp(0, (int)x, 0x112, 0xF, 0xF, false);
    x += (uint32_t)__builtin_amdgcn_update_dpp(0, (int)x, 0x114, 0xF, 0xF, false);
    x += (uint32_t)__builtin_amdgcn_update_dpp(0, (int)x, 0x118, 0xF, 0xF, false);
    x += (uint32_t)__builtin_amdgcn_update_dpp(0, (int)x, 0x142, 0xA, 0xF, false);
    x += (uint32_t)__builtin_amdgcn_update_dpp(0, (int)x, 0x143, 0xC, 0xF, false);
    return x;
}

__global__ __launch_bounds__(1024) void seed_pad_scan_kernel(uint32_t *count, uint32_t *poff)
{
    constexpr int kWaves = 1024 / kWave, kPerWave = kLists / kWaves, kRows = kPerWave / kWave;
    static_assert(kLists % (kWaves * kWave) == 0 && kRows % 8 == 0, "whole rows per wave, eight at a time");
    __shared__ uint32_t s_total[kWaves];
    const uint32_t lane = threadIdx.x % kWave, wave = uniform(threadIdx.x / kWave);
    uint32_t *const c = count + wave * kPerWave + lane;
    auto padded = [](uint32_t n) { return (n + (uint32_t)(kGuideUnroll - 1)) & ~(uint32_t)(kGuideUnroll - 1); };
    uint32_t column = 0;
#pragma unroll 16
    for (int i = 0; i < kRows; ++i) column += padded(c[i * kWave]);
    const uint32_t mine = (uint32_t)__builtin_amdgcn_readlane((int)wave_inclusive_scan(column), kWave - 1);
    if (lane == 0) s_total[wave] = mine;
    block_sync();
    uint32_t run = 0;
#pragma unroll
    for (int w = 0; w < kWaves; ++w) run += (uint32_t)w < wave ? s_total[w] : 0u;
    uint32_t *const p = poff + wave * kPerWave + lane;
    for (int i0 = 0; i0 < kRows; i0 += 8) {
        uint32_t v[8];
#pragma unroll
        for (int j = 0; j < 8; ++j) v[j] = padded(c[(i0 + j) * kWave]);
#pragma unroll
        for (int j = 0; j < 8; ++j) {
            const uint32_t inc = wave_inclusive_scan(v[j]);
            p[(i0 + j) * kWave] = run + inc - v[j];
            c[(i0 + j) * kWave] = 0;
            run += (uint32_t)__builtin_amdgcn_readlane((int)inc, kWave - 1);
        }
    }
    if (threadIdx.x == 1023) poff[kLists] = run;
}

hipError_t launch_seed_lists(const uint2 *guides, uint32_t n_guides, const SeedPlan &plan, uint32_t *count, uint32_t *poff, uint2 *list_rest,
                             hipStream_t stream)
{
    const uint64_t total = (uint64_t)n_guides * kSegments * plan.n_nbr;
    hipError_t e = hipMemsetAsync(count, 0, (size_t)kLists * sizeof(uint32_t), stream);
    if (e != hipSuccess) return e;
    const unsigned blocks = (unsigned)((total + 255) / 256);
    if (total) hipLaunchKernelGGL(seed_enum_kernel<false>, dim3(blocks), dim3(256), 0, stream, guides, n_guides, plan, count, (const uint32_t *)nullptr, (uint2 *)nullptr);
    hipLaunchKernelGGL(seed_pad_scan_kernel, dim3(1), dim3(1024), 0, stream, count, poff);
    if (total) hipLaunchKernelGGL(seed_enum_kernel<true>, dim3(blocks), dim3(256), 0, stream, guides, n_guides, plan, count, (const uint32_t *)poff, list_rest);
    return hipGetLastError();
}

typedef const __attribute__((address_space(4))) uint32_t *const_u32_ptr;
typedef uint32_t v8u __attribute__((ext_vector_type(8)));
typedef const __attribute__((address_space(4))) v8u *const_v8u_ptr;

struct SeedWave {
    uint2 *tok;
    uint32_t ntok, lane;
    uint32_t thead;
    uint32_t *parts;
    uint32_t *first;
    uint32_t *info;
};

__device__ __forceinline__ uint32_t rest_position(uint32_t q, uint32_t seg)
{
    if (seg == 0) return q + kSegBases;
    if (seg == 1) return q < (uint32_t)kSegBases ? q : q + kSegBases;
    return q;
}

__global__ __launch_bounds__(kWave *kWavesPerGroup) void seed_transpose_kernel(const uint4 *sites, const uint4 *chunk_tab,
                                                                              uint32_t n_chunks, uint32_t *vert)
{
    const uint32_t c = blockIdx.x * kWavesPerGroup + threadIdx.x / kWave;
    if (c >= n_chunks) return;
    const uint32_t lane = threadIdx.x % kWave;
    const uint4 ct = chunk_tab[c];
    const uint32_t seg = (ct.z & kChunkBucketMask) / (uint32_t)kBucketsPerSeg;
    for (uint32_t k = 0; k * kWave < ct.y; ++k) {
        const uint32_t i = k * kWave + lane;
        uint4 v = make_uint4(0u, 0u, 0u, 0u);
        if (i < ct.y) v = sites[ct.x + i];
        uint32_t mine = 0;
        for (uint32_t q = 0; q < (uint32_t)kCmpBases; ++q) {
            const uint32_t p = rest_position(q, seg);
            const uint64_t bh = __ballot((v.x >> p) & 1u), bl = __ballot((v.y >> p) & 1u);
            const uint32_t wh = lane < 32 ? (uint32_t)bh : (uint32_t)(bh >> 32);
            const uint32_t wl = lane < 32 ? (uint32_t)bl : (uint32_t)(bl >> 32);
            if ((lane & 31u) == q) mine = wh;
            if ((lane & 31u) == q + kCmpBases) mine = wl;
        }
        const uint32_t block = 2 * k + (lane >> 5), j = lane & 31u;
        const uint32_t nb = (ct.y + kSlicedSites - 1) / kSlicedSites;
        if (block < nb && j < (uint32_t)kVertWords) vert[(size_t)ct.w * kVertWords + ((size_t)(j >> 2) * nb + block) * 4 + (j & 3u)] = mine;
    }
}

hipError_t launch_seed_transpose(const uint4 *sites, const uint4 *chunk_tab, uint32_t n_chunks, uint32_t *vert,
                                 hipStream_t stream)
{
    if (n_chunks == 0) return hipSuccess;
    hipLaunchKernelGGL(seed_transpose_kernel, dim3((n_chunks + kWavesPerGroup - 1) / kWavesPerGroup),
                       dim3(kWave * kWavesPerGroup), 0, stream, sites, chunk_tab, n_chunks, vert);
    return hipGetLastError();
}

template <int kTable> __device__ __forceinline__ uint32_t bitop3(uint32_t a, uint32_t b, uint32_t c)
{
    return __builtin_amdgcn_bitop3_b32(a, b, c, kTable);
}

__device__ __forceinline__ void full_add(uint32_t a, uint32_t b, uint32_t c, uint32_t &sum, uint32_t &carry)
{
    sum = bitop3<0x96>(a, b, c);
    carry = bitop3<0xE8>(a, b, c);
}

__device__ __forceinline__ void half_add(uint32_t a, uint32_t b, uint32_t &sum, uint32_t &carry)
{
    sum = a ^ b;
    carry = a & b;
}

__device__ __forceinline__ uint32_t spread(uint32_t word, int bit)
{
    return (uint32_t)((int32_t)(word << (31 - bit)) >> 31);
}

__device__ __forceinline__ void count7(const uint32_t *m, uint32_t &b0, uint32_t &b1, uint32_t &b2)
{
    uint32_t s1, c1, s2, c2, c3;
    full_add(m[0], m[1], m[2], s1, c1);
    full_add(m[3], m[4], m[5], s2, c2);
    full_add(s1, s2, m[6], b0, c3);
    full_add(c1, c2, c3, b1, b2);
}

template <uint32_t kSeg>
__device__ __forceinline__ uint32_t sliced_within(const uint32_t (&v)[kVertWords], uint32_t rx, uint32_t budget, uint32_t valid,
                                                  const uint32_t (&kv)[4])
{
    uint32_t mm[kCmpBases];
#pragma unroll
    for (int q = 0; q < kCmpBases; ++q)
        mm[q] = bitop3<0xF6>(v[q] ^ spread(rx, q), v[kCmpBases + q], spread(rx, kRestBases + q));
    uint32_t a0, a1, a2, b0, b1, b2;
    count7(mm, a0, a1, a2);
    count7(mm + kSegBases, b0, b1, b2);
    uint32_t t0, t1, t2, k0, k1, k2;
    half_add(a0, b0, t0, k0);
    full_add(a1, b1, k0, t1, k1);
    full_add(a2, b2, k1, t2, k2);
    uint32_t le = ~t0 | spread(budget, 0);
    le = bitop3<0x8E>(t1, spread(budget, 1), le);
    le = bitop3<0x8E>(t2, spread(budget, 2), le);
    le = bitop3<0x8E>(k2, spread(budget, 3), le);
    uint32_t ok = le & valid;
    if (kSeg >= 1) ok = bitop3<0xD0>(ok, a2, bitop3<0x8E>(a1, kv[1], ~a0 | kv[0]));
    if (kSeg >= 2) ok = bitop3<0xD0>(ok, b2, bitop3<0x8E>(b1, kv[3], ~b0 | kv[2]));
    return ok;
}

struct SlicedFetch {
    uint32_t word, hi, site0;
    uint2 gp;
    uint2 rec;
};

constexpr uint32_t kPartUsedBits = 11;
constexpr uint32_t kPartUsedMask = (1u << kPartUsedBits) - 1u;
constexpr uint32_t kPartBusy = 1u << kPartUsedBits;
constexpr uint32_t kPartBlockShift = kPartUsedBits + 1;
constexpr uint32_t kPartDeadBlock = 0xFFFFFu;

__device__ __forceinline__ bool sliced_reserve(const SeedArgs &a, const SeedWave &w, uint32_t p, uint32_t losing, uint32_t &base)
{
    unsigned long long *const cursor = &a.counters[kCntPart + 4 * p];
    unsigned long long rel = 0;
    if (w.lane == 0) rel = atomicAdd(cursor, (unsigned long long)a.reserve);
    rel = ((unsigned long long)uniform((uint32_t)(rel >> 32)) << 32) | uniform((uint32_t)rel);
    if (rel + a.reserve > a.part_cap) {
        if (w.lane == 0) {
            atomicAdd(cursor, 0ull - (unsigned long long)a.reserve);
            atomicAdd(cursor + 2, (unsigned long long)losing);
            atomicMax(&a.counters[kCntOverflow], 1ull);
        }
        return false;
    }
    base = (uint32_t)rel;
    return true;
}

__device__ __forceinline__ void put_record(const SeedArgs &a, unsigned long long at, uint64_t rec, uint32_t side)
{
    a.hit_recs[at] = rec;
    if (a.hit_side) a.hit_side[at] = side;
}

__device__ __forceinline__ void sliced_store_group_slow(const SeedArgs &a, SeedWave &w, uint32_t p, bool mine, uint64_t rec, uint32_t side)
{
    volatile uint32_t *const word = &w.parts[p];
    for (uint32_t spins = 0;;) {
        uint32_t s = 0;
        if (w.lane == 0) s = *word;
        s = uniform(s);
        const uint32_t used = s & kPartUsedMask;
        if ((s >> kPartBlockShift) == kPartDeadBlock) {
            const uint64_t b = __ballot(mine);
            if (w.lane == 0) {
                atomicAdd(&a.counters[kCntPart + 4 * p + 2], (unsigned long long)__popcll(b));
                *word = (kPartDeadBlock << kPartBlockShift) | a.reserve;
            }
            return;
        }
        if (!(s & kPartBusy) && used < a.reserve) {
            uint32_t st = kPartUsedMask;
            if (mine) st = atomicAdd(&w.parts[p], 1u);
            const bool ok = mine && (st & kPartUsedMask) < a.reserve;
            if (ok) put_record(a, (unsigned long long)p * (uint32_t)a.part_cap + (((st >> kPartBlockShift) << a.reserve_log2) + (st & kPartUsedMask)), rec, side);
            mine = mine && !ok;
            if (__ballot(mine) == 0) return;
            continue;
        }
        if (s & kPartBusy) {
            if (++spins > (1u << 20)) {
                const uint64_t b = __ballot(mine);
                if (w.lane == 0) {
                    atomicAdd(&a.counters[kCntPart + 4 * p + 2], (unsigned long long)__popcll(b));
                    atomicMax(&a.counters[kCntOverflow], 1ull);
                }
                return;
            }
            __builtin_amdgcn_s_sleep(2);
            continue;
        }
        uint32_t won = 0;
        if (w.lane == 0) won = atomicCAS(&w.parts[p], s, s | kPartBusy) == s ? 1u : 0u;
        if (!uniform(won)) continue;
        const uint64_t b = __ballot(mine);
        const uint32_t n = (uint32_t)__popcll(b);
        uint32_t next = 0;
        const bool ok = sliced_reserve(a, w, p, n, next);
        if (mine && ok) put_record(a, (unsigned long long)p * a.part_cap + next + lanes_below(b), rec, side);
        if (w.lane == 0) *word = ok ? ((next >> a.reserve_log2) << kPartBlockShift) | n : (kPartDeadBlock << kPartBlockShift) | a.reserve;
        return;
    }
}

__device__ __forceinline__ void sliced_store(const SeedArgs &a, SeedWave &w, bool hit, uint32_t region, uint64_t rec, uint32_t side)
{
    uint32_t state = kPartUsedMask;
    if (hit) state = atomicAdd(&w.parts[region], 1u);
    const uint32_t slot = state & kPartUsedMask;
    const bool placed = hit && slot < a.reserve;
    if (placed) put_record(a, (unsigned long long)region * (uint32_t)a.part_cap + (((state >> kPartBlockShift) << a.reserve_log2) + slot), rec, side);
    uint64_t todo = __ballot(hit && !placed);
    while (todo != 0) {
        const uint32_t p = (uint32_t)__builtin_amdgcn_readlane((int)region, (int)__builtin_ctzll(todo));
        const bool mine = hit && !placed && region == p;
        const uint64_t b = __ballot(mine);
        if (a.group_out) {
            sliced_store_group_slow(a, w, p, mine, rec, side);
        } else {
            const uint32_t n = (uint32_t)__popcll(b);
            uint32_t next = 0;
            const bool ok = sliced_reserve(a, w, p, n, next);
            if (mine && ok) put_record(a, (unsigned long long)p * a.part_cap + next + lanes_below(b), rec, side);
            if (w.lane == 0) w.parts[p] = ok ? ((next >> a.reserve_log2) << kPartBlockShift) | n : a.reserve;
        }
        wave_sync();
        todo &= ~b;
    }
}

__device__ __forceinline__ void sliced_finish_hits(const SeedArgs &a, SeedWave &w, uint32_t first, uint32_t step)
{
    wave_sync();
    for (uint32_t q = first; q < a.n_parts; q += step) {
        const uint32_t state = uniform(w.parts[q]);
        if ((state >> kPartBlockShift) == kPartDeadBlock) continue;
        const uint32_t base = (state >> kPartBlockShift) << a.reserve_log2, used = state & kPartUsedMask;
        const uint32_t left = used < a.reserve ? a.reserve - used : 0u;
        for (uint32_t i = w.lane; i < left; i += kWave) a.hit_recs[(unsigned long long)q * a.part_cap + base + used + i] = kRecSentinel;
        if (w.lane == 0 && left) atomicAdd(&a.counters[kCntPart + 4 * q + 1], (unsigned long long)left);
    }
}

__device__ __forceinline__ uint32_t ring_slot(uint32_t p)
{
    return p & (uint32_t)(kSlicedTokCap - 1);
}

template <bool kFull>
__device__ __forceinline__ SlicedFetch sliced_fetch(const SeedArgs &a, const SeedWave &w, uint32_t head, uint32_t n)
{
    SlicedFetch f;
    if (!kFull) {
        f.word = 0;
        f.hi = 0;
        f.site0 = 0;
        f.gp = make_uint2(0u, 0u);
        f.rec = make_uint2(0u, 0u);
    }
    if (kFull || w.lane < n) {
        const uint2 tk = w.tok[ring_slot(head + w.lane)];
        f.word = tk.x;
        f.hi = tk.y;
        f.gp = a.guides[tk.y & kTokReadMask];
        f.site0 = w.first[(tk.y >> kTokSlotShift) & (uint32_t)(kSlicedGrab - 1)] + (tk.y >> kTokLaneShift) * kSlicedSites;
        f.rec = a.sites[f.site0 + (uint32_t)__builtin_ctz(tk.x)];
    }
    return f;
}

__device__ __forceinline__ uint32_t ring_tail(const SeedWave &w) { return ring_slot(w.thead + w.ntok); }

template <bool kFull>
__device__ __forceinline__ void sliced_consume(const SeedArgs &a, SeedWave &w, const SlicedFetch &f)
{
    bool hit = kFull || f.word != 0;
    const uint32_t rest = f.word & (f.word - 1);
    const uint64_t again = __ballot(rest != 0);
    if (again != 0) {
        if (rest != 0) w.tok[ring_slot(lanes_below(again, ring_tail(w)))] = make_uint2(rest, f.hi);
        w.ntok += (uint32_t)__popcll(again);
    }
    const uint32_t gid_of = f.hi & kTokReadMask;
    const uint32_t info = w.info[(f.hi >> kTokSlotShift) & (uint32_t)(kSlicedGrab - 1)];
    const uint32_t bucket = info & kChunkBucketMask;
    const uint32_t sh = (uint32_t)kSegBases * (bucket >> (2 * kSegBases));
    const uint32_t low = (1u << sh) - 1u;
    const uint32_t rest_hi = f.rec.x & 0xFFFFu, rest_lo = f.rec.x >> 16;
    const uint32_t site_hi = (rest_hi & low) | (((bucket >> kSegBases) & 0x7Fu) << sh) | ((rest_hi >> sh) << (sh + kSegBases));
    const uint32_t site_lo = (rest_lo & low) | ((bucket & 0x7Fu) << sh) | ((rest_lo >> sh) << (sh + kSegBases));
    const uint32_t t = ((site_hi ^ f.gp.x) | (site_lo ^ f.gp.y)) & kMask23;
    const uint32_t rank_in_chunk = (f.hi >> kTokLaneShift) * kSlicedSites + (uint32_t)__builtin_ctz(f.word | 0x80000000u);
    const uint32_t strand = rank_in_chunk >= ((info >> kChunkMinusShift) & 0xFFFu) ? 1u : 0u;
    const uint32_t pos = f.rec.y;
    const uint32_t mask = strand ? reverse23(t) : t;
    const bool maybe_edge = hit && ((info >> kChunkEdgeBit) & 1u) && (uint32_t)__popc(mask >> (VSC_READ_LEN / 2)) > a.k_half;
    if (__ballot(maybe_edge) != 0) {
        if (maybe_edge) {
            const uint32_t site = f.site0 + (uint32_t)__builtin_ctz(f.word);
            if (((a.edge_bits[site >> 5] >> (site & 31u)) & 1u) && is_contig_end(a.contig_end, a.n_contigs, pos + VSC_READ_LEN)) hit = false;
        }
    }
    const uint32_t low23 = a.hit_side ? (site_hi & kMask23) : mask;
    const uint64_t rec = ((uint64_t)(gid_of & (uint32_t)(kRegionReads - 1)) << kRecReadShift) | ((uint64_t)strand << kRecStrandShift) |
                         ((uint64_t)((pos - a.pos_base) << a.pos_pad) << kRecPosShift) | low23;
    sliced_store(a, w, hit, gid_of >> kRegionBits, rec, site_lo & kMask23);
// ... 242 lines not shown
```

### varscot_amd/csrc/vsc_sort.hip

```cpp
#include "vsc_internal.h"
#include "vsc_device.h"

namespace vsc {

namespace {

constexpr int kLaneRun = 2;
__device__ __forceinline__ uint32_t tile_record(int k, uint32_t t)
{
    return (uint32_t)(k / kLaneRun) * (uint32_t)(kLaneRun * kSortThreads) + t * (uint32_t)kLaneRun + (uint32_t)(k % kLaneRun);
}

template <int kThreads>
__device__ __forceinline__ uint32_t block_exclusive_scan(uint32_t *s, uint32_t n, uint32_t *s_wave)
{
    const uint32_t t = threadIdx.x, lane = t % kWave, wave = t / kWave;
    const uint32_t per = n > (uint32_t)kThreads ? n / kThreads : 1u;
    const bool mine = t * per < n;
    uint32_t v[4] = {0u, 0u, 0u, 0u};
    uint32_t sum = 0;
    if (mine)
        for (uint32_t i = 0; i < per; ++i) {
            v[i] = s[t * per + i];
            sum += v[i];
        }
    uint32_t inc = sum;
#pragma unroll
    for (int d = 1; d < kWave; d <<= 1) {
        const uint32_t o = __shfl_up(inc, d, kWave);
        if (lane >= (uint32_t)d) inc += o;
    }
    if (lane == kWave - 1) s_wave[wave] = inc;
    block_sync();
    uint32_t before = 0, total = 0;
#pragma unroll
    for (int w = 0; w < kThreads / kWave; ++w) {
        const uint32_t x = s_wave[w];
        before += (uint32_t)w < wave ? x : 0u;
        total += x;
    }
    uint32_t run = before + inc - sum;
    if (mine)
        for (uint32_t i = 0; i < per; ++i) {
            s[t * per + i] = run;
            run += v[i];
        }
    block_sync();
    return total;
}

__device__ __forceinline__ uint64_t pack_pair(uint64_t key, uint32_t val, uint32_t pos_pad, uint32_t pos_base)
{
    const uint64_t high = (key >> 32) & ((1ull << (kRecKeyBits - 32)) - 1ull);
    return (((high << 32) | (uint32_t)(((uint32_t)key - pos_base) << pos_pad)) << kRecPosShift) | (val & kMask23);
}

}

template <bool kPairs>
__global__ __launch_bounds__(kSortThreads) void bin_hist_kernel(const SortArgs a)
{
    __shared__ uint32_t s_hist[1 << kSortMaxBinBits];
    const uint32_t t = threadIdx.x;
    const uint32_t nbins = 1u << a.bin_bits;
    for (uint32_t b = t; b < nbins; b += kSortThreads) s_hist[b] = 0;
    block_sync();
    const uint32_t tile_begin = blockIdx.x * kHistTiles, tile_end = min(tile_begin + (uint32_t)kHistTiles, a.n_tiles);
    uint32_t seg = segment_of_tile(a.seg_tile0, a.n_segs, tile_begin);
    for (uint32_t tile = tile_begin; tile < tile_end; ++tile) {
        if (tile >= a.seg_tile0[seg + 1]) {
            block_sync();
            for (uint32_t b = t; b < nbins; b += kSortThreads) {
                const uint32_t c = s_hist[b];
                if (c) atomicAdd(&a.hist[((size_t)seg << a.bin_bits) + b], c);
                s_hist[b] = 0;
            }
            block_sync();
            seg = segment_of_tile(a.seg_tile0, a.n_segs, tile);
        }
        const SortSeg sg = a.segs[seg];
        const uint32_t first = (tile - a.seg_tile0[seg]) * (uint32_t)kSortTile;
        const uint32_t n = min(sg.n_in - first, (uint32_t)kSortTile);
        uint64_t r[kSortItems];
#pragma unroll
        for (int k = 0; k < kSortItems; ++k) {
            const uint32_t i = tile_record(k, t);
            const uint64_t at = sg.in_off + first + (i < n ? i : 0u);
            const uint64_t v = kPairs ? a.pair_keys[at] : a.in[at];
            r[k] = i < n ? v : kRecSentinel;
        }
#pragma unroll
        for (int k = 0; k < kSortItems; ++k) {
            if (kPairs) {
                if (tile_record(k, t) < n) atomicAdd(&s_hist[(uint32_t)(r[k] >> a.bin_shift)], 1u);
            } else {
                if (!(r[k] >> 63)) atomicAdd(&s_hist[(uint32_t)(r[k] >> a.bin_shift) & (nbins - 1u)], 1u);
            }
        }
    }
    block_sync();
    for (uint32_t b = t; b < nbins; b += kSortThreads) {
        const uint32_t c = s_hist[b];
        if (c) atomicAdd(&a.hist[((size_t)seg << a.bin_bits) + b], c);
    }
}

hipError_t launch_bin_hist(const SortArgs &args, hipStream_t stream)
{
    if (args.n_tiles == 0) return hipSuccess;
    const unsigned blocks = (args.n_tiles + kHistTiles - 1) / kHistTiles;
    if (args.pair_keys)
        hipLaunchKernelGGL(bin_hist_kernel<true>, dim3(blocks), dim3(kSortThreads), 0, stream, args);
    else
        hipLaunchKernelGGL(bin_hist_kernel<false>, dim3(blocks), dim3(kSortThreads), 0, stream, args);
    return hipGetLastError();
}

__global__ __launch_bounds__(512) void bin_scan_kernel(const SortArgs a)
{
    __shared__ uint32_t s_cnt[1 << kSortMaxBinBits];
    __shared__ uint32_t s_wave[512 / kWave];
    const uint32_t nbins = 1u << a.bin_bits;
    const size_t base = (size_t)blockIdx.x << a.bin_bits;
    for (uint32_t b = threadIdx.x; b < nbins; b += 512) s_cnt[b] = a.hist[base + b];
    block_sync();
    block_exclusive_scan<512>(s_cnt, nbins, s_wave);
    for (uint32_t b = threadIdx.x; b < nbins; b += 512) {
        a.bin_start[base + b] = s_cnt[b];
        if (!a.slot_cap) a.cursor[base + b] = s_cnt[b];
    }
}

hipError_t launch_bin_scan(const SortArgs &args, hipStream_t stream)
{
    if (args.n_segs == 0) return hipSuccess;
    hipLaunchKernelGGL(bin_scan_kernel, dim3(args.n_segs), dim3(512), 0, stream, args);
    return hipGetLastError();
}

template <bool kPairs, bool kSide = false>
__global__ __launch_bounds__(kSortThreads) void bin_partition_kernel(const SortArgs a)
{
    __shared__ uint64_t s_rec[kSortTile];
    __shared__ uint32_t s_cnt[(1 << kSortMaxBinBits) + kWave];
    __shared__ uint32_t s_gbase[kPairs ? (1 << kSortMaxBinBits) : 1];
    __shared__ uint32_t s_over[(1 << kSortMaxBinBits) / 32 + 1];
    __shared__ uint32_t s_wave[kSortThreads / kWave];
    const uint32_t t = threadIdx.x;
    const uint32_t nbins = 1u << a.bin_bits;
    uint32_t tile = blockIdx.x;
    if (a.xcd_tiles) {
        tile = (blockIdx.x & 7u) * a.xcd_tiles + (blockIdx.x >> 3);
        if ((blockIdx.x >> 3) >= a.xcd_tiles || tile >= a.n_tiles) return;
    }
    const uint32_t seg = segment_of_tile(a.seg_tile0, a.n_segs, tile);
    const SortSeg sg = a.segs[seg];
    const uint32_t first = (tile - a.seg_tile0[seg]) * (uint32_t)kSortTile;
    const uint32_t n = min(sg.n_in - first, (uint32_t)kSortTile);
    for (uint32_t b = t; b < nbins + kWave; b += kSortThreads) s_cnt[b] = 0;
    for (uint32_t b = t; b < (1u << kSortMaxBinBits) / 32u + 1u; b += kSortThreads) s_over[b] = 0;
    block_sync();
    uint64_t r[kSortItems];
    uint32_t bin[kSortItems];
    uint32_t side[kSide ? kSortItems : 1];
#pragma unroll
    for (int k = 0; k < kSortItems; ++k) {
        const uint32_t i = tile_record(k, t);
        const bool in_tile = i < n;
        const uint64_t at = sg.in_off + first + (in_tile ? i : 0u);
        if (kSide) side[k] = a.side_in[at];
        if (kPairs) {
            const uint64_t key = a.pair_keys[at];
            r[k] = in_tile ? pack_pair(key, a.pair_vals[at], a.pos_pad, a.pos_base) : kRecSentinel;
            bin[k] = in_tile ? (uint32_t)(key >> a.bin_shift) : 0u;
        } else {
            const uint64_t v = a.in[at];
            r[k] = in_tile ? v : kRecSentinel;
            bin[k] = (uint32_t)(r[k] >> a.bin_shift) & (nbins - 1u);
        }
    }
    const uint32_t spare = nbins + (t % kWave);
#pragma unroll
    for (int k = 0; k < kSortItems; ++k) {
        const bool real = !(r[k] >> 63);
        const uint32_t rank = atomicAdd(&s_cnt[real ? bin[k] : spare], real ? 1u : 0u);
        bin[k] |= rank << 16;
    }
    block_sync();
    constexpr int kOwnBins = (1 << kSortMaxBinBits) / kSortThreads;
    uint32_t own_at[kOwnBins];
#pragma unroll
    for (int j = 0; j < kOwnBins; ++j) {
        const uint32_t b = t + (uint32_t)j * kSortThreads;
        const uint32_t c = b < nbins ? s_cnt[b] : 0u;
        uint32_t at = c ? atomicAdd(&a.cursor[((size_t)seg << a.bin_bits) + b], c) : 0u;
        if (a.slot_cap && c && at + c > a.slot_cap) {
            atomicOr(a.overflow, 1u);
            atomicOr(&s_over[b >> 5], 1u << (b & 31u));
            s_over[(1u << kSortMaxBinBits) / 32u] = 1u;
        }
        own_at[j] = at;
        if (kPairs && b < nbins) s_gbase[b] = at;
    }
    const uint32_t total = block_exclusive_scan<kSortThreads>(s_cnt, nbins, s_wave);
#pragma unroll
    for (int k = 0; k < kSortItems; ++k) {
        const uint32_t slot = s_cnt[bin[k] & 0xFFFFu] + (bin[k] >> 16);
        if (!(r[k] >> 63)) s_rec[slot] = r[k];
        if (kSide) bin[k] = slot;
    }
    block_sync();
    if (!kPairs) {
#pragma unroll
        for (int j = 0; j < kOwnBins; ++j) {
            const uint32_t b = t + (uint32_t)j * kSortThreads;
            if (b < nbins) s_cnt[b] = own_at[j] - s_cnt[b];
        }
        block_sync();
    }
    const bool any_over = s_over[(1u << kSortMaxBinBits) / 32u] != 0u;
    uint32_t slot_bin[kSide ? kSortItems / 2 : 1];
    if (kSide) {
#pragma unroll
        for (int j = 0; j < kSortItems / 2; ++j) slot_bin[j] = 0;
    }
    for (uint32_t i = t; i < total; i += kSortThreads) {
        const uint64_t x = s_rec[i];
        uint32_t b;
        if (kPairs) {
            uint32_t lo = 0, hi = nbins;
            while (hi - lo > 1) {
                const uint32_t mid = (lo + hi) >> 1;
                if (s_cnt[mid] <= i) lo = mid; else hi = mid;
            }
            b = lo;
        } else {
            b = (uint32_t)(x >> a.bin_shift) & (nbins - 1u);
        }
        const uint32_t in_bin = kPairs ? s_gbase[b] + (i - s_cnt[b]) : s_cnt[b] + i;
        const bool skip = any_over && ((s_over[b >> 5] >> (b & 31u)) & 1u);
        if (a.slot_cap) {
            if (!skip) a.out[(((uint64_t)seg << a.bin_bits) + b) * a.slot_cap + in_bin] = x;
        } else {
            a.out[sg.out_off + in_bin] = x;
        }
        if (kSide) {
            const uint32_t j = i / kSortThreads;
#pragma unroll
            for (int q = 0; q < kSortItems / 2; ++q)
                if ((uint32_t)q == (j >> 1)) slot_bin[q] |= b << ((j & 1u) * 16u);
        }
    }
    if (kSide) {
        block_sync();
        uint32_t *const s_side = (uint32_t *)s_rec;
#pragma unroll
        for (int k = 0; k < kSortItems; ++k)
            if (!(r[k] >> 63)) s_side[bin[k]] = side[k];
        block_sync();
#pragma unroll
        for (int j = 0; j < kSortItems; ++j) {
            const uint32_t i = t + (uint32_t)j * kSortThreads;
            if (i < total) {
                const uint32_t b = (slot_bin[j >> 1] >> ((j & 1) * 16)) & 0xFFFFu;
                const uint32_t in_bin = s_cnt[b] + i;
                const bool skip = any_over && ((s_over[b >> 5] >> (b & 31u)) & 1u);
                if (a.slot_cap) {
                    if (!skip) a.side_out[(((uint64_t)seg << a.bin_bits) + b) * a.slot_cap + in_bin] = s_side[i];
                } else {
                    a.side_out[sg.out_off + in_bin] = s_side[i];
                }
            }
        }
    }
}

hipError_t launch_bin_partition(const SortArgs &args, hipStream_t stream)
{
    if (args.n_tiles == 0) return hipSuccess;
    const unsigned blocks = args.xcd_tiles ? 8u * args.xcd_tiles : args.n_tiles;
    if (args.pair_keys)
        hipLaunchKernelGGL(bin_partition_kernel<true>, dim3(blocks), dim3(kSortThreads), 0, stream, args);
    else if (args.side_in)
        hipLaunchKernelGGL((bin_partition_kernel<false, true>), dim3(blocks), dim3(kSortThreads), 0, stream, args);
    else
        hipLaunchKernelGGL(bin_partition_kernel<false>, dim3(blocks), dim3(kSortThreads), 0, stream, args);
    return hipGetLastError();
}

__device__ __forceinline__ uint32_t sub_slot(const uint32_t *s_sub, uint32_t sb)
{
    return (s_sub[sb >> 1] >> ((sb & 1u) * 16u)) & 0xFFFFu;
}

constexpr int kFinalizeAhead = 4;
constexpr int kFinalizeNear = 4;
constexpr int kFinalizeRange = 64;

template <bool kRows>
__device__ __forceinline__ void finalize_bin(const FinArgs &a, const uint32_t which)
{
    __shared__ uint64_t s_rec[kSortCap];
    __shared__ uint32_t s_sub[(1 << (kRows ? kSortSubBitsRows : kSortSubBits)) / 2 + 1 + kWave];
    __shared__ uint4 s_stage[kRows ? (kFinThreads / kWave) * 64 : 1];
    __shared__ uint32_t s_wave[kFinThreads / kWave];
    __shared__ uint32_t s_range[2 + kFinalizeRange];
    __shared__ uint32_t s_edge[4];
    uint32_t t_ = threadIdx.x;
    asm volatile("" : "+v"(t_));
    const uint32_t t = t_;
    const uint32_t seg = which >> a.bin_bits, bin = which & ((1u << a.bin_bits) - 1u);
    const SortSeg sg = a.segs[seg];
    uint64_t src = sg.in_off, dst = sg.final_off;
    uint64_t compact = sg.in_off;
    uint32_t n_src = sg.n_in;
    if (a.hist) {
        const size_t idx = ((size_t)seg << a.bin_bits) + bin;
        n_src = a.hist[idx];
        const uint32_t st = a.bin_start[idx];
        src = a.slot_cap ? (uint64_t)idx * a.slot_cap : sg.out_off + st;
        dst = sg.final_off + st;
        compact = sg.in_off + st;
    }
    if (n_src == 0) return;
    if (n_src > a.cap) {
        if (t == 0) {
            const uint32_t slot = atomicAdd(a.n_over, 1u);
            if (slot < a.over_cap) {
                SortSeg o;
                o.in_off = src;
                o.out_off = a.slot_cap ? compact : src;
                o.final_off = dst;
                o.n_in = n_src;
                o.guide_base = sg.guide_base;
                a.over[slot] = o;
            }
        }
        return;
    }
    const uint32_t nsub = 1u << a.sub_bits;
    const uint32_t nwords = nsub > 1u ? nsub / 2u : 1u;
    for (uint32_t i = t; i <= nwords + kWave; i += kFinThreads) s_sub[i] = 0;
    if (t < 4) s_edge[t] = 0;
    const bool few_contigs = a.n_contigs <= (uint32_t)kFinThreads;
    const uint32_t my_contig = (few_contigs && t < a.n_contigs) ? a.contig_off[t] : 0xFFFFFFFFu;
    block_sync();
    const uint64_t *const in = a.src + src;
    uint64_t r[kFinItems];
    uint32_t rk[kFinItems];
#pragma unroll
    for (int k = 0; k < kFinItems; ++k) {
        const uint32_t i = k * kFinThreads + t;
        const uint64_t v = in[i < n_src ? i : 0u];
        r[k] = i < n_src ? v : kRecSentinel;
    }
    if (t == 0) {
        const uint32_t free_bits = a.sub_bits + a.low_bits;
        const uint32_t any = (uint32_t)(r[0] >> kRecPosShift) >> a.pos_pad;
        const uint32_t p_lo = free_bits >= 32u ? 0u : (any >> free_bits) << free_bits;
        const uint64_t p_hi = free_bits >= 32u ? 0xFFFFFFFFull : (uint64_t)(p_lo | ((1u << free_bits) - 1u)) + a.pos_base;
        s_edge[0] = free_bits >= 32u ? 0u : (uint32_t)min((uint64_t)p_lo + a.pos_base, (uint64_t)0xFFFFFFFFull);
        s_edge[1] = (uint32_t)min(p_hi, (uint64_t)0xFFFFFFFFull);
    }
#pragma unroll
    for (int k = 0; k < kFinItems; ++k) {
        const bool real = !(r[k] >> 63);
        const uint32_t sb = (uint32_t)(r[k] >> a.sub_shift) & (nsub - 1u);
        const uint32_t sh = (sb & 1u) * 16u;
        rk[k] = (atomicAdd(&s_sub[real ? sb >> 1 : nwords + 1u + (t % kWave)], real ? 1u << sh : 0u) >> sh) & 0xFFFFu;
    }
    block_sync();
    if (few_contigs) {
        const uint32_t p_lo = s_edge[0], p_hi = s_edge[1];
        const bool mine = t < a.n_contigs;
        const uint64_t le_lo = __ballot(mine && my_contig <= p_lo), le_hi = __ballot(mine && my_contig <= p_hi);
        if (t % kWave == 0) {
            if (le_lo) atomicAdd(&s_edge[2], (uint32_t)__popcll(le_lo));
            if (le_hi) atomicAdd(&s_edge[3], (uint32_t)__popcll(le_hi));
        }
    }
    uint32_t n;
    {
        const uint32_t per = nwords > (uint32_t)kFinThreads ? nwords / kFinThreads : 1u;
        static_assert((1 << kSortSubBits) / 2 <= 8 * kFinThreads, "a thread scans at most 8 words of the sub-bin table");
        const bool mine = t * per < nwords;
        uint32_t w[8];
        uint32_t sum = 0;
#pragma unroll
        for (int i = 0; i < 8; ++i) {
            w[i] = (mine && (uint32_t)i < per) ? s_sub[t * per + i] : 0u;
            sum += (w[i] & 0xFFFFu) + (w[i] >> 16);
        }
        const uint32_t lane = t % kWave, wave = t / kWave;
        uint32_t inc = sum;
#pragma unroll
        for (int d = 1; d < kWave; d <<= 1) {
            const uint32_t o = __shfl_up(inc, d, kWave);
            if (lane >= (uint32_t)d) inc += o;
        }
        if (lane == kWave - 1) s_wave[wave] = inc;
        block_sync();
        uint32_t before = 0, total = 0;
#pragma unroll
        for (int q = 0; q < kFinThreads / kWave; ++q) {
            const uint32_t x = s_wave[q];
            before += (uint32_t)q < wave ? x : 0u;
            total += x;
        }
        n = total;
        uint32_t run = before + inc - sum;
#pragma unroll
        for (int i = 0; i < 8; ++i) {
            const uint32_t lo = run;
            run += w[i] & 0xFFFFu;
            const uint32_t hi = run;
            run += w[i] >> 16;
            if (mine && (uint32_t)i < per) s_sub[t * per + i] = lo | (hi << 16);
        }
        if (t == 0 && nsub > 1u) s_sub[nwords] = n;
        if (few_contigs) {
            const uint32_t c_lo = max(s_edge[2], 1u) - 1u, c_hi = max(s_edge[3], 1u) - 1u;
            if (t == 0) {
                s_range[0] = c_lo;
                s_range[1] = c_hi - c_lo + 1u;
            }
            if (t >= c_lo && t < c_lo + (uint32_t)kFinalizeRange && t < a.n_contigs) s_range[2 + t - c_lo] = my_contig;
            if (t < (uint32_t)kFinalizeRange && a.n_contigs - c_lo + t < (uint32_t)kFinalizeRange) s_range[2 + a.n_contigs - c_lo + t] = 0xFFFFFFFFu;
        } else if (t == 0) {
            const uint32_t p_lo = s_edge[0], p_hi = s_edge[1];
            uint32_t lo = 0, hi = a.n_contigs;
            while (hi - lo > 1) {
                const uint32_t mid = (lo + hi) >> 1;
                if (a.contig_off[mid] <= p_lo) lo = mid; else hi = mid;
            }
            const uint32_t c_lo = lo;
            hi = a.n_contigs;
            while (hi - lo > 1) {
                const uint32_t mid = (lo + hi) >> 1;
                if (a.contig_off[mid] <= p_hi) lo = mid; else hi = mid;
            }
            s_range[0] = c_lo;
            s_range[1] = lo - c_lo + 1u;
        }
        block_sync();
        if (!few_contigs && t < (uint32_t)kFinalizeRange) s_range[2 + t] = t < s_range[1] ? a.contig_off[s_range[0] + t] : 0xFFFFFFFFu;
    }
#pragma unroll
    for (int k = 0; k < kFinItems; ++k)
        if (!(r[k] >> 63))
            s_rec[sub_slot(s_sub, (uint32_t)(r[k] >> a.sub_shift) & (nsub - 1u)) + rk[k]] =
                kRows ? (r[k] & ~(uint64_t)kMask23) | (uint32_t)(k * kFinThreads + t) : r[k];
    block_sync();
    const uint32_t c_lo = s_range[0], c_n = s_range[1];
    const uint32_t st0 = s_range[2], st1 = s_range[3], st2 = s_range[4], st3 = s_range[5];
    if (!kRows) {
        for (uint32_t base = 0; base < n; base += 2 * kFinThreads) {
            uint32_t s[2], e[2], smaller[2] = {0u, 0u};
            uint64_t x[2];
            bool live[2];
    #pragma unroll
            for (int u = 0; u < 2; ++u) {
                const uint32_t idx = base + u * kFinThreads + t;
                live[u] = idx < n;
                const uint64_t v = s_rec[live[u] ? idx : 0u];
                x[u] = live[u] ? v : 0ull;
            }
    #pragma unroll
            for (int u = 0; u < 2; ++u) {
                const uint32_t sb = (uint32_t)(x[u] >> a.sub_shift) & (nsub - 1u);
                const uint32_t first = sub_slot(s_sub, sb), next = sub_slot(s_sub, sb + 1u);
                s[u] = first;
                e[u] = live[u] ? next : first;
            }
            if (a.low_bits) {
                uint64_t y[2][kFinalizeAhead];
    #pragma unroll
                for (int u = 0; u < 2; ++u)
    #pragma unroll
                    for (int j = 0; j < kFinalizeAhead; ++j) y[u][j] = s_rec[min(s[u] + (uint32_t)j, (uint32_t)kSortCap - 1u)];
    #pragma unroll
                for (int u = 0; u < 2; ++u)
    #pragma unroll
                    for (int j = 0; j < kFinalizeAhead; ++j) smaller[u] += (uint32_t)(s[u] + (uint32_t)j < e[u] && y[u][j] < x[u]);
                for (uint32_t d = kFinalizeAhead;; ++d) {
                    const bool act0 = s[0] + d < e[0], act1 = s[1] + d < e[1];
                    if (__ballot(act0 || act1) == 0) break;
                    const uint64_t y0 = s_rec[act0 ? s[0] + d : 0u], y1 = s_rec[act1 ? s[1] + d : 0u];
                    smaller[0] += (uint32_t)(act0 && y0 < x[0]);
                    smaller[1] += (uint32_t)(act1 && y1 < x[1]);
                }
            }
    #pragma unroll
            for (int u = 0; u < 2; ++u) {
                if (!live[u]) continue;
                const uint32_t pos = ((uint32_t)(x[u] >> kRecPosShift) >> a.pos_pad) + a.pos_base;
                uint32_t c, start;
                if (c_n <= (uint32_t)kFinalizeNear) {
                    const uint32_t k = (uint32_t)(pos >= st1) + (uint32_t)(pos >= st2) + (uint32_t)(pos >= st3);
                    c = c_lo + k;
                    start = k == 0 ? st0 : (k == 1 ? st1 : (k == 2 ? st2 : st3));
                } else if (c_n <= (uint32_t)kFinalizeRange) {
                    uint32_t lo = 0, hi = c_n;
                    while (hi - lo > 1) {
                        const uint32_t mid = (lo + hi) >> 1;
                        if (s_range[2 + mid] <= pos) lo = mid; else hi = mid;
                    }
                    c = c_lo + lo;
                    start = s_range[2 + lo];
                } else {
                    uint32_t lo = c_lo, hi = c_lo + c_n;
                    while (hi - lo > 1) {
                        const uint32_t mid = (lo + hi) >> 1;
                        if (a.contig_off[mid] <= pos) lo = mid; else hi = mid;
                    }
                    c = lo;
                    start = a.contig_off[c];
                }
                const uint32_t mask = (uint32_t)x[u] & kMask23;
                uint4 h;
                h.x = sg.guide_base + ((uint32_t)(x[u] >> kRecReadShift) & (uint32_t)(kRegionReads - 1));
                h.y = c;
                h.z = pos - start;
                h.w = ((uint32_t)(x[u] >> kRecStrandShift) & 1u) << 31 | (uint32_t)__popc(mask) << 23 | mask;
                v4u hv;
                hv.x = h.x;
                hv.y = h.y;
                hv.z = h.z;
                hv.w = h.w;
                __builtin_nontemporal_store(hv, (v4u *)a.out + (dst + s[u] + smaller[u]));
            }
        }
    } else {
        const uint32_t *const side_in = a.side_src + src;
        const uint64_t kmask = ~(uint64_t)kMask23;
        for (uint32_t base = 0; base < n; base += 2 * kFinThreads) {
            uint32_t s[2], e[2], smaller[2] = {0u, 0u};
            uint64_t x[2], full[2];
            uint32_t lo_plane[2];
            bool live[2];
#pragma unroll
            for (int u = 0; u < 2; ++u) {
                const uint32_t idx = base + u * kFinThreads + t;
                live[u] = idx < n;
                const uint64_t v = s_rec[live[u] ? idx : 0u];
                x[u] = live[u] ? v : 0ull;
            }
#pragma unroll
            for (int u = 0; u < 2; ++u) {
                const uint32_t slot = (uint32_t)x[u] & 0x1FFFu;
                full[u] = in[slot];
                lo_plane[u] = side_in[slot];
            }
#pragma unroll
            for (int u = 0; u < 2; ++u) {
                const uint32_t sb = (uint32_t)(x[u] >> a.sub_shift) & (nsub - 1u);
                const uint32_t first = sub_slot(s_sub, sb), next = sub_slot(s_sub, sb + 1u);
                s[u] = first;
                e[u] = live[u] ? next : first;
            }
            if (a.low_bits) {
                uint64_t y[2][kFinalizeAhead];
#pragma unroll
                for (int u = 0; u < 2; ++u)
#pragma unroll
                    for (int j = 0; j < kFinalizeAhead; ++j) y[u][j] = s_rec[min(s[u] + (uint32_t)j, (uint32_t)kSortCap - 1u)];
#pragma unroll
                for (int u = 0; u < 2; ++u)
#pragma unroll
                    for (int j = 0; j < kFinalizeAhead; ++j) smaller[u] += (uint32_t)(s[u] + (uint32_t)j < e[u] && (y[u][j] & kmask) < (x[u] & kmask));
                for (uint32_t d = kFinalizeAhead;; ++d) {
                    const bool act0 = s[0] + d < e[0], act1 = s[1] + d < e[1];
                    if (__ballot(act0 || act1) == 0) break;
                    const uint64_t y0 = s_rec[act0 ? s[0] + d : 0u], y1 = s_rec[act1 ? s[1] + d : 0u];
                    smaller[0] += (uint32_t)(act0 && (y0 & kmask) < (x[0] & kmask));
                    smaller[1] += (uint32_t)(act1 && (y1 & kmask) < (x[1] & kmask));
                }
            }
            uint32_t w[2][16];
            uint64_t row_at[2] = {~0ull, ~0ull};
#pragma unroll
            for (int u = 0; u < 2; ++u) {
                if (!live[u]) continue;
                const uint32_t pos = ((uint32_t)(x[u] >> kRecPosShift) >> a.pos_pad) + a.pos_base;
                uint32_t c, start;
                if (c_n <= (uint32_t)kFinalizeNear) {
                    const uint32_t k = (uint32_t)(pos >= st1) + (uint32_t)(pos >= st2) + (uint32_t)(pos >= st3);
                    c = c_lo + k;
                    start = k == 0 ? st0 : (k == 1 ? st1 : (k == 2 ? st2 : st3));
                } else if (c_n <= (uint32_t)kFinalizeRange) {
                    uint32_t lo = 0, hi = c_n;
                    while (hi - lo > 1) {
                        const uint32_t mid = (lo + hi) >> 1;
                        if (s_range[2 + mid] <= pos) lo = mid; else hi = mid;
                    }
                    c = c_lo + lo;
                    start = s_range[2 + lo];
                } else {
                    uint32_t lo = c_lo, hi = c_lo + c_n;
                    while (hi - lo > 1) {
                        const uint32_t mid = (lo + hi) >> 1;
                        if (a.contig_off[mid] <= pos) lo = mid; else hi = mid;
                    }
                    c = lo;
                    start = a.contig_off[c];
                }
                const uint32_t strand = (uint32_t)(x[u] >> kRecStrandShift) & 1u;
                const uint32_t guide = sg.guide_base + ((uint32_t)(x[u] >> kRecReadShift) & (uint32_t)(kRegionReads - 1));
                const uint2 gp = a.guides[guide - a.guide_first];
                const uint32_t hi_pl = (uint32_t)full[u] & kMask23, lo_pl = lo_plane[u] & kMask23;
                const uint32_t tm = ((hi_pl ^ gp.x) | (lo_pl ^ gp.y)) & kMask23;
                const uint32_t mask = strand ? reverse23(tm) : tm;
                v4u hv;
                hv.x = guide;
                hv.y = c;
                hv.z = pos - start;
                hv.w = strand << 31 | (uint32_t)__popc(mask) << 23 | mask;
                const uint64_t at = dst + s[u] + smaller[u];
                __builtin_nontemporal_store(hv, (v4u *)a.out + at);
                row_at[u] = at - a.rows_first;
                feature_row_packed(gp.x, gp.y, hi_pl, lo_pl, w[u]);
            }
            uint4 *const stage = s_stage + (t / kWave) * 64;
            const uint32_t lane = t % kWave;
#pragma unroll
            for (int u = 0; u < 2; ++u) {
                if (__ballot(row_at[u] != ~0ull) == 0) continue;
#pragma unroll
                for (int j = 0; j < 4; ++j) {
                    if ((lane >> 4) == (uint32_t)j) {
#pragma unroll
                        for (int q = 0; q < 4; ++q)
                            stage[4 * (lane & 15u) + ((uint32_t)q ^ (lane & 3u))] = make_uint4(w[u][4 * q], w[u][4 * q + 1], w[u][4 * q + 2], w[u][4 * q + 3]);
                    }
                    wave_sync();
                    const uint32_t r = lane >> 2, q = lane & 3u;
                    const uint32_t owner = 16u * (uint32_t)j + r;
                    const uint32_t at_lo = __shfl((uint32_t)row_at[u], (int)owner, kWave), at_hi = __shfl((uint32_t)(row_at[u] >> 32), (int)owner, kWave);
                    const uint4 piece = stage[4 * r + (q ^ (r & 3u))];
                    if ((at_lo & at_hi) != 0xFFFFFFFFu) {
                        v4u rv;
                        rv.x = piece.x;
                        rv.y = piece.y;
                        rv.z = piece.z;
                        rv.w = piece.w;
                        __builtin_nontemporal_store(rv, (v4u *)a.rows + ((((uint64_t)at_hi << 32) | at_lo) * 4 + q));
                    }
                    wave_sync();
                }
            }
        }
    }
}

template <bool kRows>
__global__ __launch_bounds__(kFinThreads) __attribute__((amdgpu_waves_per_eu(4, 4))) void bin_finalize_kernel(const FinArgs a)
{
    __shared__ uint32_t s_next[2];
    if (a.overflow && *a.overflow) return;
    const uint32_t total = a.n_segs << a.bin_bits;
    uint32_t which = blockIdx.x, parity = 0;
    while (which < total) {
        if (threadIdx.x == 0) s_next[parity] = atomicAdd(a.cursor, 1u) + gridDim.x;
        finalize_bin<kRows>(a, which);
        block_sync();
        which = s_next[parity];
        parity ^= 1u;
    }
}

hipError_t launch_bin_finalize(const FinArgs &args, int max_groups, hipStream_t stream)
{
    if (args.n_segs == 0) return hipSuccess;
    const uint64_t bins = (uint64_t)args.n_segs << args.bin_bits;
    if (bins >= (1ull << 31) || args.sub_bits > (uint32_t)(args.rows ? kSortSubBitsRows : kSortSubBits) || args.bin_bits > (uint32_t)kSortMaxBinBits ||
        args.cap > (uint32_t)kSortCap || max_groups < 1)
        return hipErrorInvalidValue;
    const dim3 grid((unsigned)std::min<uint64_t>(bins, (uint64_t)max_groups));
    if (args.rows)
        hipLaunchKernelGGL(bin_finalize_kernel<true>, grid, dim3(kFinThreads), 0, stream, args);
    else
        hipLaunchKernelGGL(bin_finalize_kernel<false>, grid, dim3(kFinThreads), 0, stream, args);
    return hipGetLastError();
}

}
```

Measured before the change: 287,000.

## Index seeds by sort-join, compact live sort bins, prefetch bin descriptors

Seed list construction is replaced: a new kernel ranks each guide's segment key to build a sorted per-segment index, and a join kernel walks the neighbour buckets against that index instead of enumerating every guide×segment×neighbour with atomics. Per-segment neighbour counts are now separate for segments 0, 1 and the rest. The sort's histogram/scan pass emits a compacted list of non-empty bins, so the finalize kernel iterates only over live bins and fetches the next descriptor ahead of time. Smaller host-side changes merge two H2D copies into one and skip hipMemGetInfo when buffers are already large enough. These add complexity and an O(n^2/tile) ranking pass in the seed index.

```diff
diff --git a/varscot_amd/csrc/vsc_api.cpp b/varscot_amd/csrc/vsc_api.cpp
--- a/varscot_amd/csrc/vsc_api.cpp
+++ b/varscot_amd/csrc/vsc_api.cpp
@@ -203,7 +203,7 @@
     (void)hipStreamSynchronize(ctx->stream);
     for (DeviceBuf *b : {&ctx->counters, &ctx->guides, &ctx->score_guides, &ctx->keys_a, &ctx->keys_b, &ctx->vals_a, &ctx->vals_b, &ctx->votes_rows,
                          &ctx->score_mit, &ctx->score_flags, &ctx->score_feat, &ctx->score_sched, &ctx->sort_segs, &ctx->sort_tabs,
-                         &ctx->sort_over, &ctx->seed_off,
+                         &ctx->sort_over, &ctx->seed_off, &ctx->seed_index,
                          &ctx->seed_poff, &ctx->seed_lrest, &ctx->sum_rows, &ctx->sum_excl, &ctx->sel_hist, &ctx->sel_tabs, &ctx->sel_keys,
                          &ctx->sel_masks, &ctx->sum_rows_in, &ctx->regions_buf, &ctx->enum_tabs, &ctx->locate_buf, &ctx->locate_out,
                          &ctx->varmap_buf, &ctx->var_state, &ctx->var_excl, &ctx->var_labels})
@@ -964,11 +964,12 @@
             for (const SortSeg &sg : segs) span = std::max<uint64_t>(span, sg.out_off + sg.n_in);
             const uint64_t slot_records = (uint64_t)n_bins * slot_cap;
             if (use_slots && dbg.sort_optimistic != 1) {
+                const uint64_t slot_bytes = slot_records * (sizeof(uint64_t) + (rows ? sizeof(uint32_t) : 0));
+                const bool held = other_buf->cap >= slot_records * sizeof(uint64_t) && (!rows || rows->side_other->cap >= slot_records * sizeof(uint32_t));
                 size_t free_b = 0, total_b = 0;
-                if (hipMemGetInfo(&free_b, &total_b) != hipSuccess) free_b = 0;
+                if (!held && hipMemGetInfo(&free_b, &total_b) != hipSuccess) free_b = 0;
                 const uint64_t room = (uint64_t)free_b + other_buf->cap;
-                const uint64_t slot_bytes = slot_records * (sizeof(uint64_t) + (rows ? sizeof(uint32_t) : 0));
-                if (slot_records > 4 * n_all + (1ull << 20) || slot_bytes + (1ull << 30) > room + (rows ? rows->side_other->cap : 0)) {
+                if (slot_records > 4 * n_all + (1ull << 20) || (!held && slot_bytes + (1ull << 30) > room + (rows ? rows->side_other->cap : 0))) {
                     use_slots = false;
                     *slots = false;
                 }
@@ -1000,19 +1001,22 @@
         VSC_TRY(ctx->sort_segs.ensure(seg_bytes + tile0.size() * sizeof(uint32_t)));
         SortSeg *d_segs = (SortSeg *)ctx->sort_segs.p;
         uint32_t *d_tile0 = (uint32_t *)((char *)ctx->sort_segs.p + seg_bytes);
-        ctx->host_segs = segs;
-        VSC_TRY(hipMemcpyAsync(d_segs, ctx->host_segs.data(), n_segs * sizeof(SortSeg), hipMemcpyHostToDevice, st));
-        VSC_TRY(hipMemcpyAsync(d_tile0, tile0.data(), tile0.size() * sizeof(uint32_t), hipMemcpyHostToDevice, st));
+        std::vector<char> &up = ctx->host_sort_tables;
+        up.resize(seg_bytes + tile0.size() * sizeof(uint32_t));
+        std::memcpy(up.data(), segs.data(), n_segs * sizeof(SortSeg));
+        std::memcpy(up.data() + seg_bytes, tile0.data(), tile0.size() * sizeof(uint32_t));
+        VSC_TRY(hipMemcpyAsync(d_segs, up.data(), up.size(), hipMemcpyHostToDevice, st));
         VSC_TRY(ctx->sort_over.ensure(256 + n_bins * sizeof(SortSeg)));
         uint32_t *d_n_over = (uint32_t *)ctx->sort_over.p;
-        if (bits) VSC_TRY(ctx->sort_tabs.ensure(3 * n_bins * sizeof(uint32_t)));
+        const size_t tab_bytes = (3 * n_bins * sizeof(uint32_t) + 15) / 16 * 16;
+        if (bits) VSC_TRY(ctx->sort_tabs.ensure(tab_bytes + n_bins * sizeof(BinDesc)));
         uint32_t flags[3] = {0, 0, 0};
         for (;;) {
             if (dbg.sort_debug)
                 std::fprintf(stderr, "[vsc sort] level %u: %zu segments, %llu records, largest %llu, %u bits (of %u left), cap %llu%s\n", level,
                              n_segs, (unsigned long long)n_all, (unsigned long long)n_max, bits, rem, (unsigned long long)sort_cap,
                              use_slots ? ", slot mode" : "");
-            VSC_TRY(hipMemsetAsync(d_n_over, 0, 3 * sizeof(uint32_t), st));
+            VSC_TRY(hipMemsetAsync(d_n_over, 0, 4 * sizeof(uint32_t), st));
             FinArgs f{};
             f.segs = d_segs;
             f.n_segs = (uint32_t)n_segs;
@@ -1037,6 +1041,8 @@
                 a.hist = (uint32_t *)ctx->sort_tabs.p;
                 a.cursor = a.hist + n_bins;
                 a.bin_start = a.cursor + n_bins;
+                a.live = (BinDesc *)((char *)ctx->sort_tabs.p + tab_bytes);
+                a.n_live = d_n_over + 3;
                 a.bin_bits = bits;
                 a.bin_shift = kRecPosShift + pos_pad + rem - bits;
                 if (dbg.sort_xcd != 0 && tiles >= 64) a.xcd_tiles = (uint32_t)((tiles + 7) / 8);
@@ -1073,8 +1079,8 @@
                 }
                 f.src = other;
                 f.side_src = side_other;
-                f.hist = a.hist;
-                f.bin_start = a.bin_start;
+                f.live = a.live;
+                f.n_live = a.n_live;
                 f.bin_bits = bits;
                 f.slot_cap = a.slot_cap;
                 f.overflow = a.overflow;
@@ -1255,7 +1261,9 @@
         plan.k1 = (uint32_t)(best / 3);
         *k2_max = std::min<int>(2, (int)m - (int)plan.k0 - (int)plan.k1 - 2);
     }
-    plan.n_nbr = neighbours(std::max<int>(std::max<int>((int)plan.k0, (int)plan.k1), *k2_max));
+    plan.n_nbr0 = neighbours((int)plan.k0);
+    plan.n_nbr1 = neighbours((int)plan.k1);
+    plan.n_nbr = neighbours(*k2_max);
     return plan;
 }
 
@@ -1269,9 +1277,10 @@
     VSC_TRY(ctx->seed_off.ensure((kLists + 1) * sizeof(uint32_t)));
     VSC_TRY(ctx->seed_poff.ensure((kLists + 1) * sizeof(uint32_t)));
     VSC_TRY(ctx->seed_lrest.ensure(list_cap * sizeof(uint2)));
-    VSC_TRY(hipMemsetAsync(ctx->seed_lrest.p, 0xFF, list_cap * sizeof(uint2), ctx->stream));
+    const size_t index_entries = ((size_t)kSegments * n_guides * sizeof(uint2) + 15) / 16 * 16;
+    VSC_TRY(ctx->seed_index.ensure(index_entries + kBuckets * sizeof(uint32_t)));
     VSC_TRY(launch_seed_lists((const uint2 *)ctx->guides.p, n_guides, plan, (uint32_t *)ctx->seed_off.p, (uint32_t *)ctx->seed_poff.p,
-                              (uint2 *)ctx->seed_lrest.p, ctx->stream));
+                              (uint2 *)ctx->seed_lrest.p, (uint2 *)ctx->seed_index.p, (uint32_t *)((char *)ctx->seed_index.p + index_entries), ctx->stream));
     VSC_TRY(hipEventRecord(ctx->ev[kEvPrepEnd], ctx->stream));
     sa.chunk_tab = genome->d_ix_chunk_tab;
     sa.n_chunks = genome->ix_chunks;
diff --git a/varscot_amd/csrc/vsc_internal.h b/varscot_amd/csrc/vsc_internal.h
--- a/varscot_amd/csrc/vsc_internal.h
+++ b/varscot_amd/csrc/vsc_internal.h
@@ -109,6 +109,14 @@
     uint32_t guide_base;
 };
 
+struct alignas(16) BinDesc {
+    uint64_t src;
+    uint64_t dst;
+    uint64_t compact;
+    uint32_t n;
+    uint32_t guide_base;
+};
+
 struct SortArgs {
     const SortSeg *segs;
     const uint32_t *seg_tile0;
@@ -128,14 +136,16 @@
     uint32_t xcd_tiles;
     uint32_t slot_cap;
     uint32_t *overflow;
+    BinDesc *live;
+    uint32_t *n_live;
 };
 
 struct FinArgs {
     const SortSeg *segs;
     uint32_t n_segs;
     const uint64_t *src;
-    const uint32_t *hist;
-    const uint32_t *bin_start;
+    const BinDesc *live;
+    const uint32_t *n_live;
     uint32_t bin_bits;
     uint32_t sub_shift, sub_bits;
     uint32_t low_bits;
@@ -177,6 +187,7 @@
 struct SeedPlan {
     uint32_t max_mm, k0, k1, tight;
     uint32_t n_nbr;
+    uint32_t n_nbr0, n_nbr1;
     uint32_t n_pam;
     uint32_t pam_codes;
 };
@@ -380,6 +391,7 @@
                              hipStream_t stream);
 hipError_t launch_seed_keys(const uint4 *rec, uint64_t n, int seg, uint32_t pam_codes, uint32_t n_pam, uint64_t *sort_records, hipStream_t stream);
 hipError_t launch_seed_lists(const uint2 *guides, uint32_t n_guides, const SeedPlan &plan, uint32_t *count, uint32_t *poff, uint2 *list_rest,
+                             uint2 *entries, uint32_t *first,
                              hipStream_t stream);
 hipError_t launch_seed_pack16(const uint32_t *x, const uint32_t *l, const uint32_t *pos, uint64_t n, uint4 *rec, hipStream_t stream);
 hipError_t launch_seed_gather16(const uint4 *rec, const uint64_t *sorted, uint64_t n, uint4 *out, hipStream_t stream);
diff --git a/varscot_amd/csrc/vsc_objects.h b/varscot_amd/csrc/vsc_objects.h
--- a/varscot_amd/csrc/vsc_objects.h
+++ b/varscot_amd/csrc/vsc_objects.h
@@ -87,7 +87,9 @@
     vsc::DeviceBuf sort_segs, sort_tabs, sort_over, score_sched;
     std::vector<vsc::SortSeg> host_segs;
     std::vector<uint32_t> host_tile0;
+    std::vector<char> host_sort_tables;
     vsc::DeviceBuf seed_off, seed_poff, seed_lrest;
+    vsc::DeviceBuf seed_index;
     vsc::DeviceBuf sum_rows, sum_excl;
     vsc::DeviceBuf sel_hist, sel_tabs, sel_keys, sel_masks;
     vsc::DeviceBuf sum_rows_in, regions_buf;
diff --git a/varscot_amd/csrc/vsc_seed.hip b/varscot_amd/csrc/vsc_seed.hip
--- a/varscot_amd/csrc/vsc_seed.hip
+++ b/varscot_amd/csrc/vsc_seed.hip
@@ -112,27 +112,23 @@
 __constant__ uint8_t kPairP[21] = {0, 0, 0, 0, 0, 0, 1, 1, 1, 1, 1, 2, 2, 2, 2, 3, 3, 3, 4, 4, 5};
 __constant__ uint8_t kPairQ[21] = {1, 2, 3, 4, 5, 6, 2, 3, 4, 5, 6, 3, 4, 5, 6, 4, 5, 6, 5, 6, 6};
 
-__device__ __forceinline__ void substitute(uint32_t &h, uint32_t &l, uint32_t p, uint32_t alt)
-{
-    const uint32_t c = (((h >> p) & 1u) << 1) | ((l >> p) & 1u);
-    const uint32_t d = (c + alt) & 3u;
-    h = (h & ~(1u << p)) | ((d >> 1) << p);
-    l = (l & ~(1u << p)) | ((d & 1u) << p);
-}
-
-__device__ __forceinline__ uint32_t seed_neighbour(const uint2 gp, uint32_t s, uint32_t n, uint32_t *dist)
-{
-    uint32_t h = (gp.x >> (kSegBases * s)) & 0x7Fu, l = (gp.y >> (kSegBases * s)) & 0x7Fu;
+__device__ __forceinline__ uint32_t seed_neighbour_mask(uint32_t n, uint32_t *dist)
+{
+    uint32_t h = 0, l = 0;
+    auto substitute = [&](uint32_t p, uint32_t alt) {
+        h |= (alt >> 1) << p;
+        l |= (alt & 1u) << p;
+    };
     if (n >= 22) {
         const uint32_t e = n - 22, pi = e / 9, alts = e % 9;
-        substitute(h, l, kPairP[pi], alts / 3 + 1);
-        substitute(h, l, kPairQ[pi], alts % 3 + 1);
+        substitute(kPairP[pi], alts / 3 + 1);
+        substitute(kPairQ[pi], alts % 3 + 1);
     } else if (n >= 1) {
         const uint32_t e = n - 1;
-        substitute(h, l, e / 3, e % 3 + 1);
+        substitute(e / 3, e % 3 + 1);
     }
     *dist = n >= 22 ? 2u : (n >= 1 ? 1u : 0u);
-    return s * kBucketsPerSeg + ((h << kSegBases) | l);
+    return (h << kSegBases) | l;
 }
 
 __device__ __forceinline__ uint32_t rest_of(uint32_t v, uint32_t seg)
@@ -143,25 +139,54 @@
     return (v & 0x3FFFu) | ((v >> (3 * kSegBases)) << (2 * kSegBases));
 }
 
-template <bool kScatter>
-__global__ __launch_bounds__(256) void seed_enum_kernel(const uint2 *guides, uint32_t n_guides, const SeedPlan plan, uint32_t *count,
-                                                        const uint32_t *poff, uint2 *list_rest)
-{
-    const uint64_t i = (uint64_t)blockIdx.x * blockDim.x + threadIdx.x;
-    const uint64_t total = (uint64_t)n_guides * kSegments * plan.n_nbr;
-    if (i >= total) return;
-    const uint32_t n = (uint32_t)(i % plan.n_nbr);
-    const uint32_t s = (uint32_t)((i / plan.n_nbr) % kSegments);
-    const uint32_t g = (uint32_t)(i / ((uint64_t)plan.n_nbr * kSegments));
-    const uint2 gp = guides[g];
-    uint32_t d;
-    const uint32_t b = seed_neighbour(gp, s, n, &d);
-    const uint32_t mine = pam_code(gp.x, gp.y);
-    const uint32_t rest = rest_of(gp.x, s) | (rest_of(gp.y, s) << 16);
+constexpr int kIndexTile = 4096;
+constexpr int kIndexReads = kWave, kIndexSlices = 4;
+constexpr int kIndexReadBits = kTokSlotShift;
+constexpr int kIndexCodeShift = kIndexReadBits + 4;
+static_assert(kMaxPassReads <= (1 << kIndexReadBits) && 2 * kSegBases + kIndexCodeShift == 32 && kIndexTile % (4 * 256) == 0, "index key");
+
+__global__ __launch_bounds__(kIndexReads *kIndexSlices) void seed_index_kernel(const uint2 *guides, uint32_t n_guides, uint2 *entries, uint32_t *first)
+{
+    __shared__ uint4 s_keys[kIndexTile / 4];
+    __shared__ uint32_t s_part[kIndexReads * kIndexSlices];
+    const uint32_t s = blockIdx.y, g = blockIdx.x * kIndexReads + threadIdx.x % kIndexReads, slice = uniform(threadIdx.x / kIndexReads);
+    auto key_of = [&](uint32_t r, uint2 gp) { return (segment_key(gp.x, gp.y, (int)s) << kIndexCodeShift) | (r << 4) | pam_code(gp.x, gp.y); };
+    const uint2 my_gp = guides[min(g, n_guides - 1)];
+    const uint32_t mine = g < n_guides ? key_of(g, my_gp) : 0u;
+    uint32_t place = 0;
+    for (uint32_t t0 = 0; t0 < n_guides; t0 += kIndexTile) {
+        block_sync();
+        uint2 gp[kIndexTile / (kIndexReads * kIndexSlices)];
+#pragma unroll
+        for (int k = 0; k < kIndexTile / (kIndexReads * kIndexSlices); ++k) gp[k] = guides[min(t0 + k * blockDim.x + threadIdx.x, n_guides - 1)];
+#pragma unroll
+        for (int k = 0; k < kIndexTile / (kIndexReads * kIndexSlices); ++k) {
+            const uint32_t r = t0 + k * blockDim.x + threadIdx.x;
+            ((uint32_t *)s_keys)[r - t0] = r < n_guides ? key_of(r, gp[k]) : 0xFFFFFFFFu;
+        }
+        block_sync();
+        const uint32_t quads = (min(n_guides - t0, (uint32_t)kIndexTile) + 3) / 4, per = (quads + kIndexSlices - 1) / kIndexSlices;
+        const uint32_t q1 = min((slice + 1) * per, quads);
+#pragma unroll 8
+        for (uint32_t q = slice * per; q < q1; ++q) {
+            const uint4 k = s_keys[q];
+            place += (k.x < mine ? 1u : 0u) + (k.y < mine ? 1u : 0u) + (k.z < mine ? 1u : 0u) + (k.w < mine ? 1u : 0u);
+        }
+    }
+    s_part[threadIdx.x] = place;
+    block_sync();
+    if (slice != 0 || g >= n_guides) return;
+    for (int i = 1; i < kIndexSlices; ++i) place += s_part[i * kIndexReads + threadIdx.x];
+    entries[s * n_guides + place] = make_uint2(mine, rest_of(my_gp.x, s) | (rest_of(my_gp.y, s) << 16));
+    atomicMin(&first[s * (uint32_t)kBucketsPerSeg + (mine >> kIndexCodeShift)], place);
+}
+
+__device__ __forceinline__ bool seed_entry(const SeedPlan &plan, uint32_t s, uint32_t cls, uint32_t d, uint32_t mine, uint32_t g, uint32_t *y)
+{
     constexpr uint32_t kNone = (kListNoBudget << kListBudgetShift) | (kListNoBudget << (kListBudgetShift + 4)) |
                                (kListNoBudget << (kListBudgetShift + 8)) | (kListNoBudget << (kListBudgetShift + 12));
-    uint32_t shared = kNone;
-    for (uint32_t c = 0; c < plan.n_pam; ++c) {
+    uint32_t budgets = kNone;
+    for (uint32_t c = s < 2 ? 0u : cls; c < (s < 2 ? plan.n_pam : cls + 1); ++c) {
         const uint32_t diff = mine ^ ((plan.pam_codes >> (4 * c)) & 15u);
         const uint32_t spent = ((diff & 12u) ? 1u : 0u) + ((diff & 3u) ? 1u : 0u);
         if (spent + d > plan.max_mm) continue;
@@ -169,18 +194,10 @@
         const int thr = s == 0 ? (int)plan.k0 : (s == 1 ? (int)plan.k1 : (plan.tight ? (int)left - (int)plan.k0 - (int)plan.k1 - 2 : (int)plan.k0));
         if ((int)d > thr) continue;
         const uint32_t field = kListBudgetShift + 4 * c;
-        if (s < 2) {
-            shared = (shared & ~(15u << field)) | ((left - d) << field);
-            continue;
-        }
-        const uint32_t list = b + c * (uint32_t)kBucketsPerSeg;
-        const uint32_t at = atomicAdd(&count[list], 1u);
-        if (kScatter) list_rest[poff[list] + at] = make_uint2(rest, g | ((kNone & ~(15u << field)) | ((left - d) << field)));
-    }
-    if (s < 2 && shared != kNone) {
-        const uint32_t at = atomicAdd(&count[b], 1u);
-        if (kScatter) list_rest[poff[b] + at] = make_uint2(rest, g | shared);
-    }
+        budgets = (budgets & ~(15u << field)) | ((left - d) << field);
+    }
+    *y = g | budgets;
+    return budgets != kNone;
 }
 
 __device__ __forceinline__ uint32_t wave_inclusive_scan(uint32_t x)
@@ -194,13 +211,114 @@
     return x;
 }
 
-__global__ __launch_bounds__(1024) void seed_pad_scan_kernel(uint32_t *count, uint32_t *poff)
+constexpr uint32_t kJoinNoRun = 0xFFFFu;
+
+template <bool kWrite>
+__device__ __forceinline__ void join_run(const SeedPlan &plan, uint32_t s, uint32_t cls, uint32_t d, uint32_t at, uint2 e0, uint2 e1, const uint2 *ent,
+                                         uint32_t n_guides, uint32_t &acc, uint2 *list_rest)
+{
+    if (at == kJoinNoRun) return;
+    const uint32_t nb = e0.x >> kIndexCodeShift;
+    uint2 e = e0;
+    for (uint32_t j = at;;) {
+        uint32_t y;
+        if (seed_entry(plan, s, cls, d, e.x & 15u, (e.x >> 4) & ((1u << kIndexReadBits) - 1u), &y)) {
+            if (kWrite) list_rest[acc] = make_uint2(e.y, y);
+            ++acc;
+        }
+        if (++j >= n_guides) break;
+        e = j == at + 1 ? e1 : ent[j];
+        if ((e.x >> kIndexCodeShift) != nb) break;
+    }
+}
+
+constexpr int kJoinThreads = 1024, kJoinLists = 128, kJoinPerLane = 4;
+static_assert(kBucketsPerSeg % (4 * kJoinThreads) == 0 && kBucketsPerSeg % kJoinLists == 0 && kJoinLists % (kJoinThreads / kWave) == 0 && kJoinPerLane * kWave >= 211 && kMaxPassReads < (int)kJoinNoRun,
+              "whole workgroups per segment, whole rounds of waves, a lane per four neighbours, 16-bit places");
+
+template <bool kFill>
+__global__ __launch_bounds__(kJoinThreads) void seed_join_kernel(uint32_t n_guides, const SeedPlan plan, const uint2 *entries, const uint32_t *first,
+                                                                 uint32_t *count, const uint32_t *poff, uint2 *list_rest)
+{
+    __shared__ __attribute__((aligned(8))) uint16_t s_first[kBucketsPerSeg];
+    const uint32_t list0 = blockIdx.x * (uint32_t)kJoinLists, lane = threadIdx.x % kWave, wave = uniform(threadIdx.x / kWave);
+    const uint32_t s = min(list0 / (uint32_t)kBucketsPerSeg, 2u), cls = list0 / (uint32_t)kBucketsPerSeg - s;
+    const uint32_t n_nbr = s == 0 ? plan.n_nbr0 : (s == 1 ? plan.n_nbr1 : (cls < plan.n_pam ? plan.n_nbr : 0u));
+    if (n_nbr) {
+        constexpr int kQuads = kBucketsPerSeg / 4 / kJoinThreads;
+        const uint4 *const f4 = (const uint4 *)(first + s * (uint32_t)kBucketsPerSeg);
+        uint4 v[kQuads];
+#pragma unroll
+        for (int k = 0; k < kQuads; ++k) v[k] = f4[k * kJoinThreads + threadIdx.x];
+#pragma unroll
+        for (int k = 0; k < kQuads; ++k)
+            ((uint2 *)s_first)[k * kJoinThreads + threadIdx.x] =
+                make_uint2(min(v[k].x, kJoinNoRun) | (min(v[k].y, kJoinNoRun) << 16), min(v[k].z, kJoinNoRun) | (min(v[k].w, kJoinNoRun) << 16));
+    }
+    uint32_t mask[kJoinPerLane], d[kJoinPerLane];
+#pragma unroll
+    for (int u = 0; u < kJoinPerLane; ++u) mask[u] = seed_neighbour_mask(min(lane * kJoinPerLane + u, 210u), &d[u]);
+    block_sync();
+    const uint2 *const ent = entries + s * n_guides;
+    constexpr int kPerWave = kJoinLists / (kJoinThreads / kWave);
+    const uint32_t wave_list0 = list0 + wave * (uint32_t)kPerWave;
+    uint32_t start[kPerWave + 1] = {};
+    if (kFill) {
+#pragma unroll
+        for (int i = 0; i <= kPerWave; ++i) start[i] = poff[wave_list0 + i];
+    }
+#pragma unroll
+    for (int i = 0; i < kPerWave; ++i) {
+        const uint32_t list = wave_list0 + i;
+        const uint32_t code = list % (uint32_t)kBucketsPerSeg;
+        uint32_t at[kJoinPerLane];
+        bool any = false;
+#pragma unroll
+        for (int u = 0; u < kJoinPerLane; ++u) {
+            at[u] = lane * kJoinPerLane + u < n_nbr ? s_first[code ^ mask[u]] : kJoinNoRun;
+            any = any || at[u] != kJoinNoRun;
+        }
+        uint32_t total = 0, mine = 0;
+        const uint32_t base = start[i];
+        if (__ballot(any) != 0) {
+            uint2 e0[kJoinPerLane], e1[kJoinPerLane];
+#pragma unroll
+            for (int u = 0; u < kJoinPerLane; ++u) {
+                e0[u] = e1[u] = make_uint2(0xFFFFFFFFu, 0xFFFFFFFFu);
+                if (at[u] != kJoinNoRun) e0[u] = ent[at[u]];
+                if (at[u] != kJoinNoRun && at[u] + 1 < n_guides) e1[u] = ent[at[u] + 1];
+            }
+#define VSC_JOIN_RUNS(kWrite, acc)                                                                                          \
+    join_run<kWrite>(plan, s, cls, d[0], at[0], e0[0], e1[0], ent, n_guides, acc, list_rest);                               \
+    join_run<kWrite>(plan, s, cls, d[1], at[1], e0[1], e1[1], ent, n_guides, acc, list_rest);                               \
+    join_run<kWrite>(plan, s, cls, d[2], at[2], e0[2], e1[2], ent, n_guides, acc, list_rest);                               \
+    join_run<kWrite>(plan, s, cls, d[3], at[3], e0[3], e1[3], ent, n_guides, acc, list_rest)
+            static_assert(kJoinPerLane == 4, "VSC_JOIN_RUNS");
+            VSC_JOIN_RUNS(false, mine);
+            const uint32_t upto = wave_inclusive_scan(mine);
+            total = (uint32_t)__builtin_amdgcn_readlane((int)upto, kWave - 1);
+            if (kFill && mine) {
+                uint32_t to = base + upto - mine;
+                VSC_JOIN_RUNS(true, to);
+            }
+#undef VSC_JOIN_RUNS
+        }
+        if (!kFill) {
+            if (lane == 0) count[list] = total;
+            continue;
+        }
+        const uint32_t end = start[i + 1];
+        if (base + total + lane < end) list_rest[base + total + lane] = make_uint2(0xFFFFFFFFu, 0xFFFFFFFFu);
+    }
+}
+
+__global__ __launch_bounds__(1024) void seed_pad_scan_kernel(const uint32_t *count, uint32_t *poff)
 {
     constexpr int kWaves = 1024 / kWave, kPerWave = kLists / kWaves, kRows = kPerWave / kWave;
     static_assert(kLists % (kWaves * kWave) == 0 && kRows % 8 == 0, "whole rows per wave, eight at a time");
     __shared__ uint32_t s_total[kWaves];
     const uint32_t lane = threadIdx.x % kWave, wave = uniform(threadIdx.x / kWave);
-    uint32_t *const c = count + wave * kPerWave + lane;
+    const uint32_t *const c = count + wave * kPerWave + lane;
     auto padded = [](uint32_t n) { return (n + (uint32_t)(kGuideUnroll - 1)) & ~(uint32_t)(kGuideUnroll - 1); };
     uint32_t column = 0;
 #pragma unroll 16
@@ -220,7 +338,6 @@
         for (int j = 0; j < 8; ++j) {
             const uint32_t inc = wave_inclusive_scan(v[j]);
             p[(i0 + j) * kWave] = run + inc - v[j];
-            c[(i0 + j) * kWave] = 0;
             run += (uint32_t)__builtin_amdgcn_readlane((int)inc, kWave - 1);
         }
     }
@@ -228,15 +345,20 @@
 }
 
 hipError_t launch_seed_lists(const uint2 *guides, uint32_t n_guides, const SeedPlan &plan, uint32_t *count, uint32_t *poff, uint2 *list_rest,
-                             hipStream_t stream)
-{
-    const uint64_t total = (uint64_t)n_guides * kSegments * plan.n_nbr;
-    hipError_t e = hipMemsetAsync(count, 0, (size_t)kLists * sizeof(uint32_t), stream);
+                             uint2 *entries, uint32_t *first, hipStream_t stream)
+{
+    if (n_guides > (uint32_t)kMaxPassReads) return hipErrorInvalidValue;
+    hipError_t e = hipMemsetAsync(first, 0xFF, (size_t)kBuckets * sizeof(uint32_t), stream);
     if (e != hipSuccess) return e;
-    const unsigned blocks = (unsigned)((total + 255) / 256);
-    if (total) hipLaunchKernelGGL(seed_enum_kernel<false>, dim3(blocks), dim3(256), 0, stream, guides, n_guides, plan, count, (const uint32_t *)nullptr, (uint2 *)nullptr);
+    if (n_guides)
+        hipLaunchKernelGGL(seed_index_kernel, dim3((n_guides + kIndexReads - 1) / kIndexReads, kSegments), dim3(kIndexReads * kIndexSlices), 0, stream, guides,
+                           n_guides, entries, first);
+    const dim3 grid(kLists / kJoinLists), block(kJoinThreads);
+    hipLaunchKernelGGL(seed_join_kernel<false>, grid, block, 0, stream, n_guides, plan, (const uint2 *)entries, (const uint32_t *)first, count,
+                       (const uint32_t *)nullptr, (uint2 *)nullptr);
     hipLaunchKernelGGL(seed_pad_scan_kernel, dim3(1), dim3(1024), 0, stream, count, poff);
-    if (total) hipLaunchKernelGGL(seed_enum_kernel<true>, dim3(blocks), dim3(256), 0, stream, guides, n_guides, plan, count, (const uint32_t *)poff, list_rest);
+    hipLaunchKernelGGL(seed_join_kernel<true>, grid, block, 0, stream, n_guides, plan, (const uint2 *)entries, (const uint32_t *)first, count,
+                       (const uint32_t *)poff, list_rest);
     return hipGetLastError();
 }
 
diff --git a/varscot_amd/csrc/vsc_sort.hip b/varscot_amd/csrc/vsc_sort.hip
--- a/varscot_amd/csrc/vsc_sort.hip
+++ b/varscot_amd/csrc/vsc_sort.hip
@@ -124,10 +124,36 @@
     const size_t base = (size_t)blockIdx.x << a.bin_bits;
     for (uint32_t b = threadIdx.x; b < nbins; b += 512) s_cnt[b] = a.hist[base + b];
     block_sync();
+    uint32_t at = 0;
+    if (a.live) {
+        uint32_t mine = 0;
+        for (uint32_t b = threadIdx.x; b < nbins; b += 512) mine += s_cnt[b] ? 1u : 0u;
+        if (threadIdx.x == 0) s_wave[0] = 0;
+        block_sync();
+        at = mine ? atomicAdd(&s_wave[0], mine) : 0u;
+        block_sync();
+        if (threadIdx.x == 0) s_wave[1] = s_wave[0] ? atomicAdd(a.n_live, s_wave[0]) : 0u;
+        block_sync();
+        at += s_wave[1];
+        block_sync();
+    }
     block_exclusive_scan<512>(s_cnt, nbins, s_wave);
+    SortSeg sg{};
+    if (a.live) sg = a.segs[blockIdx.x];
     for (uint32_t b = threadIdx.x; b < nbins; b += 512) {
-        a.bin_start[base + b] = s_cnt[b];
-        if (!a.slot_cap) a.cursor[base + b] = s_cnt[b];
+        const uint32_t st = s_cnt[b];
+        a.bin_start[base + b] = st;
+        if (!a.slot_cap) a.cursor[base + b] = st;
+        const uint32_t n = a.live ? a.hist[base + b] : 0u;
+        if (n) {
+            BinDesc d;
+            d.src = a.slot_cap ? (uint64_t)(base + b) * a.slot_cap : sg.out_off + st;
+            d.dst = sg.final_off + st;
+            d.compact = sg.in_off + st;
+            d.n = n;
+            d.guide_base = sg.guide_base;
+            a.live[at++] = d;
+        }
     }
 }
 
@@ -297,8 +323,33 @@
 constexpr int kFinalizeNear = 4;
 constexpr int kFinalizeRange = 64;
 
+constexpr uint32_t kBinDescEnd = 0xFFFFFFFFu;
+
+__device__ __forceinline__ BinDesc bin_desc(const FinArgs &a, uint32_t turn, uint32_t total)
+{
+    BinDesc d{};
+    d.n = kBinDescEnd;
+    if (turn >= total) return d;
+    if (a.live) return a.live[turn];
+    const SortSeg sg = a.segs[turn];
+    d.src = sg.in_off;
+    d.dst = sg.final_off;
+    d.compact = sg.in_off;
+    d.n = sg.n_in;
+    d.guide_base = sg.guide_base;
+    return d;
+}
+
+__device__ __forceinline__ void fetch_ahead(const FinArgs &a, uint32_t parity, uint32_t total, BinDesc *s_desc, uint32_t *s_turn)
+{
+    const uint32_t after_next = atomicAdd(a.cursor, 1u) + 2u * gridDim.x;
+    const BinDesc next = bin_desc(a, s_turn[parity], total);
+    s_turn[parity ^ 1u] = after_next;
+    s_desc[parity ^ 1u] = next;
+}
+
 template <bool kRows>
-__device__ __forceinline__ void finalize_bin(const FinArgs &a, const uint32_t which)
+__device__ __forceinline__ void finalize_bin(const FinArgs &a, const uint32_t parity, const uint32_t total, BinDesc *s_desc, uint32_t *s_turn)
 {
     __shared__ uint64_t s_rec[kSortCap];
     __shared__ uint32_t s_sub[(1 << (kRows ? kSortSubBitsRows : kSortSubBits)) / 2 + 1 + kWave];
@@ -309,31 +360,24 @@
     uint32_t t_ = threadIdx.x;
     asm volatile("" : "+v"(t_));
     const uint32_t t = t_;
-    const uint32_t seg = which >> a.bin_bits, bin = which & ((1u << a.bin_bits) - 1u);
-    const SortSeg sg = a.segs[seg];
-    uint64_t src = sg.in_off, dst = sg.final_off;
-    uint64_t compact = sg.in_off;
-    uint32_t n_src = sg.n_in;
-    if (a.hist) {
-        const size_t idx = ((size_t)seg << a.bin_bits) + bin;
-        n_src = a.hist[idx];
-        const uint32_t st = a.bin_start[idx];
-        src = a.slot_cap ? (uint64_t)idx * a.slot_cap : sg.out_off + st;
-        dst = sg.final_off + st;
-        compact = sg.in_off + st;
-    }
-    if (n_src == 0) return;
-    if (n_src > a.cap) {
+    const BinDesc bd = s_desc[parity];
+    const uint64_t src = ((uint64_t)uniform((uint32_t)(bd.src >> 32)) << 32) | uniform((uint32_t)bd.src);
+    const uint64_t dst = ((uint64_t)uniform((uint32_t)(bd.dst >> 32)) << 32) | uniform((uint32_t)bd.dst);
+    const uint32_t n_src = uniform(bd.n), guide_base = uniform(bd.guide_base);
+    if (n_src == 0 || n_src > a.cap) {
         if (t == 0) {
-            const uint32_t slot = atomicAdd(a.n_over, 1u);
-            if (slot < a.over_cap) {
-                SortSeg o;
-                o.in_off = src;
-                o.out_off = a.slot_cap ? compact : src;
-                o.final_off = dst;
-                o.n_in = n_src;
-                o.guide_base = sg.guide_base;
-                a.over[slot] = o;
+            fetch_ahead(a, parity, total, s_desc, s_turn);
+            if (n_src) {
+                const uint32_t slot = atomicAdd(a.n_over, 1u);
+                if (slot < a.over_cap) {
+                    SortSeg o;
+                    o.in_off = src;
+                    o.out_off = a.slot_cap ? bd.compact : src;
+                    o.final_off = dst;
+                    o.n_in = n_src;
+                    o.guide_base = guide_base;
+                    a.over[slot] = o;
+                }
             }
         }
         return;
@@ -354,6 +398,7 @@
         const uint64_t v = in[i < n_src ? i : 0u];
         r[k] = i < n_src ? v : kRecSentinel;
     }
+    if (t == 0) fetch_ahead(a, parity, total, s_desc, s_turn);
     if (t == 0) {
         const uint32_t free_bits = a.sub_bits + a.low_bits;
         const uint32_t any = (uint32_t)(r[0] >> kRecPosShift) >> a.pos_pad;
@@ -518,7 +563,7 @@
                 }
                 const uint32_t mask = (uint32_t)x[u] & kMask23;
                 uint4 h;
-                h.x = sg.guide_base + ((uint32_t)(x[u] >> kRecReadShift) & (uint32_t)(kRegionReads - 1));
+                h.x = guide_base + ((uint32_t)(x[u] >> kRecReadShift) & (uint32_t)(kRegionReads - 1));
                 h.y = c;
                 h.z = pos - start;
                 h.w = ((uint32_t)(x[u] >> kRecStrandShift) & 1u) << 31 | (uint32_t)__popc(mask) << 23 | mask;
@@ -605,7 +650,7 @@
                     start = a.contig_off[c];
                 }
                 const uint32_t strand = (uint32_t)(x[u] >> kRecStrandShift) & 1u;
-                const uint32_t guide = sg.guide_base + ((uint32_t)(x[u] >> kRecReadShift) & (uint32_t)(kRegionReads - 1));
+                const uint32_t guide = guide_base + ((uint32_t)(x[u] >> kRecReadShift) & (uint32_t)(kRegionReads - 1));
                 const uint2 gp = a.guides[guide - a.guide_first];
                 const uint32_t hi_pl = (uint32_t)full[u] & kMask23, lo_pl = lo_plane[u] & kMask23;
                 const uint32_t tm = ((hi_pl ^ gp.x) | (lo_pl ^ gp.y)) & kMask23;
@@ -655,16 +700,19 @@
 template <bool kRows>
 __global__ __launch_bounds__(kFinThreads) __attribute__((amdgpu_waves_per_eu(4, 4))) void bin_finalize_kernel(const FinArgs a)
 {
-    __shared__ uint32_t s_next[2];
+    __shared__ BinDesc s_desc[2];
+    __shared__ uint32_t s_turn[2];
     if (a.overflow && *a.overflow) return;
-    const uint32_t total = a.n_segs << a.bin_bits;
-    uint32_t which = blockIdx.x, parity = 0;
-    while (which < total) {
-        if (threadIdx.x == 0) s_next[parity] = atomicAdd(a.cursor, 1u) + gridDim.x;
-        finalize_bin<kRows>(a, which);
-        block_sync();
-        which = s_next[parity];
-        parity ^= 1u;
+    const uint32_t total = a.live ? *a.n_live : a.n_segs;
+    if (blockIdx.x >= total) return;
+    if (threadIdx.x == 0) {
+        s_desc[0] = bin_desc(a, blockIdx.x, total);
+        s_turn[0] = blockIdx.x + gridDim.x;
+    }
+    block_sync();
+    for (uint32_t parity = 0; uniform(s_desc[parity].n) != kBinDescEnd; parity ^= 1u) {
+        finalize_bin<kRows>(a, parity, total, s_desc, s_turn);
+        block_sync();
     }
 }
 
@@ -672,7 +720,7 @@
 {
     if (args.n_segs == 0) return hipSuccess;
     const uint64_t bins = (uint64_t)args.n_segs << args.bin_bits;
-    if (bins >= (1ull << 31) || args.sub_bits > (uint32_t)(args.rows ? kSortSubBitsRows : kSortSubBits) || args.bin_bits > (uint32_t)kSortMaxBinBits ||
+    if (bins >= (1ull << 31) || (args.bin_bits != 0 && !args.live) || args.sub_bits > (uint32_t)(args.rows ? kSortSubBitsRows : kSortSubBits) || args.bin_bits > (uint32_t)kSortMaxBinBits ||
         args.cap > (uint32_t)kSortCap || max_groups < 1)
         return hipErrorInvalidValue;
     const dim3 grid((unsigned)std::min<uint64_t>(bins, (uint64_t)max_groups));
```

Result: slower. 283,900 (-1.1%).
